# OrangeEarth15/3dgrut

Measured on AMD Instinct MI355X. Metric: train-step images/sec + render ms/frame, MipNeRF360 bicycle @1/2/4/8 GPU, higher is better.
Workload: dtype f32; 1 GPU; bicycle_like_6M_1237x822; num_gaussians=6000000, sh_degree=3, parallelism=per-view dp1, exchanged_records_last_step=0, loss=0.8*L1+0.2*(1-SSIM) (HIP fused SSIM), optimizer=HIP fused SH-gradient+Adam, all 59 params/Gaussian, trainer=native, optimizer_state=synthetic mid-training state: non-zero Adam moments on every row, storage_order=morton, optimizer_overlap=True, lazy_moment_decay=True, densification_statistics=False, warmup_extended_by=6

## Files before the change

3dgrut_amd/_capi.py:

```python
import ctypes as C
import os

HERE = os.path.dirname(os.path.abspath(__file__))
LIB_PATH = os.environ.get("GUT_HIP_LIB", os.path.join(HERE, "libgut_hip.so"))

GUT_ABI_VERSION = 6
GUT_NUM_KERNEL_TIMERS = 11
BWD_RAW_PARAMETER_GRADS = 1
BWD_COMPACT_RADIANCE_GRADS = 2
BWD_SKIP_EPILOGUE = 4
OPT_LAZY_TILE_ORDER = 1
ADAM_CLEAR_CONSUMED_GRADS = 1
GRADIENT_RECORD_FLOATS = 16
OPT_SORTED_REFERENCE_BACKWARD = 2
OPT_EARLY_EXTRA_PERCENT = 3
OPT_FORWARD_TILE_ORDER = 4
OPT_KERNEL_TIMING_SET = 5
OPT_DEBUG_REPLACE_SCRATCH = 100
KERNEL_TIMER_NAMES = ("project", "scan", "expand", "sort", "ranges", "render", "render_bwd", "project_bwd", "optimizer",
                      "optimizer_early", "optimizer_early_2")

SHUTTER_GLOBAL = 4
CAMERA_PINHOLE, CAMERA_FISHEYE = 0, 1

# ... 13 lines not shown


class GutConfig(C.Structure):
    _fields_ = [
        ("abi_version", C.c_int32), ("enable_kernel_timings", C.c_int32), ("particle_radiance_sph_degree", C.c_int32),
        ("particle_kernel_degree", C.c_int32), ("k_buffer_size", C.c_int32), ("global_z_order", C.c_int32),
        ("n_rolling_shutter_iterations", C.c_int32), ("ut_require_all_sigma_points", C.c_int32),
        ("rect_bounding", C.c_int32), ("tight_opacity_bounding", C.c_int32), ("tile_based_culling", C.c_int32),
        ("enable_hitcounts", C.c_int32),
        ("particle_kernel_min_response", C.c_float), ("particle_kernel_min_alpha", C.c_float),
        ("particle_kernel_max_alpha", C.c_float), ("min_transmittance", C.c_float),
        ("ut_alpha", C.c_float), ("ut_beta", C.c_float), ("ut_kappa", C.c_float), ("ut_in_image_margin_factor", C.c_float),
    ]


class GutStats(C.Structure):
    _fields_ = [
        ("num_particles", C.c_uint64), ("num_visible", C.c_uint64), ("num_intersections", C.c_uint64),
        ("num_tiles", C.c_uint64), ("num_pixels", C.c_uint64), ("traversed_fwd", C.c_uint64),
        ("traversed_bwd", C.c_uint64), ("sort_end_bit", C.c_uint32), ("binning_overflows", C.c_uint32),
        ("side_stream_rows", C.c_uint64), ("side_stream_rows_first_launch", C.c_uint64),
    ]


class GutLazyMoments(C.Structure):
    _fields_ = [("d_wave_step", C.c_void_p), ("d_pow_beta1", C.c_void_p), ("d_pow_beta2", C.c_void_p), ("table_len", C.c_uint32),
                ("d_overrun", C.c_void_p)]


class GutRegularisation(C.Structure):
    _fields_ = [("density_coeff", C.c_float), ("scale_coeff", C.c_float), ("d_partials", C.c_void_p)]


EXPORTS = ("gut_default_config", "gut_create", "gut_destroy", "gut_trace", "gut_trace_bwd", "gut_collect_times",
           "gut_get_stats", "gut_debug_buffer", "gut_debug_copy", "gut_kernel_times", "gut_kernel_times_mean", "gut_last_error", "gut_abi_version",
           "gut_ssim_workspace_bytes", "gut_ssim_forward", "gut_ssim_backward",
           "gut_photometric_workspace_bytes", "gut_photometric_loss", "gut_optimize_after_bwd", "gut_set_option",
           "gut_trace_bwd_ex", "gut_optimize_rows_without_gradient", "gut_compact_gradient_rows", "gut_scatter_gradient_records",
           "gut_sh_adam_step_ex", "gut_mark_walked_waves", "gut_adam_unwalked_waves", "gut_activate_pack", "gut_adam_step", "gut_sh_adam_step", "gut_mcmc_relocation",
           "gut_optimize_finish_without_gradient", "gut_scatter_gradient_records_dev", "gut_adam_unwalked_waves_ex", "gut_sync_moments", "gut_trace_fields", "gut_trace_bwd_fields", "gut_selective_adam",
           "gut_trace_model_fields", "gut_trace_bwd_model_fields", "gut_position_gradient_statistics",
           "gut_set_position_gradient_statistics", "gut_mcmc_perturb", "gut_trace_raw_model_fields", "gut_set_regularisation",
           "gut_sh_adam_step_regularised", "gut_adam_unwalked_waves_regularised", "gut_sync_moments_ex", "gut_regularisation_gradient",
           "gut_regularisation_loss", "gut_image_metrics_workspace_bytes", "gut_image_metrics")

_lib = None


def load():
    global _lib
    if _lib is not None:
        return _lib
    path = os.environ.get("GUT_HIP_LIBRARY") or LIB_PATH
    if not os.path.exists(path):
        raise RuntimeError(
            f"{path} is missing: the 3DGUT HIP extension is not built. Run `python -c 'import __graft_entry__ as g; "
            "g.build()'` (needs hipcc). There is no CPU fallback in the product path.")
    lib = C.CDLL(path)
    vp, u32, i32, f_p = C.c_void_p, C.c_uint32, C.c_int32, C.c_void_p
    lib.gut_last_error.restype = C.c_char_p
    lib.gut_abi_version.restype = C.c_int
    lib.gut_default_config.argtypes = [C.POINTER(GutConfig)]
    lib.gut_default_config.restype = None
    lib.gut_create.argtypes = [C.POINTER(GutConfig), C.c_int, C.POINTER(vp)]
    lib.gut_destroy.argtypes = [vp]
    lib.gut_destroy.restype = None
    lib.gut_trace.argtypes = [vp, vp, u32, i32, u32, f_p, f_p, i32, i32, f_p, f_p, C.POINTER(GutCamera), f_p, f_p, f_p, f_p]
    lib.gut_trace_bwd.argtypes = [vp, vp, u32, i32, u32, f_p, f_p, i32, i32, f_p, f_p, C.POINTER(GutCamera),
                                  f_p, f_p, f_p, f_p, f_p, f_p]
    lib.gut_trace_fields.argtypes = [vp, vp, u32, i32, u32, f_p, f_p, f_p, f_p, f_p, i32, i32, f_p, f_p, C.POINTER(GutCamera), f_p, f_p, f_p, f_p]
    lib.gut_trace_bwd_fields.argtypes = [vp, vp, u32, i32, u32, f_p, i32, i32, f_p, f_p, C.POINTER(GutCamera), f_p, f_p, f_p, f_p,
                                         f_p, f_p, f_p, f_p, f_p]
    lib.gut_trace_model_fields.argtypes = [vp, vp, u32, i32, u32, f_p, f_p, f_p, f_p, f_p, f_p, i32, i32, f_p, f_p, C.POINTER(GutCamera),
                                           f_p, f_p, f_p, f_p]
    lib.gut_trace_raw_model_fields.argtypes = lib.gut_trace_model_fields.argtypes
    lib.gut_trace_bwd_model_fields.argtypes = [vp, vp, u32, i32, u32, i32, i32, f_p, f_p, C.POINTER(GutCamera), f_p, f_p, f_p, f_p,
                                               f_p, f_p, f_p, f_p, f_p, f_p]
# ... 16 lines not shown
    lib.gut_photometric_loss.argtypes = [vp, i32, i32, vp, vp, C.c_float, C.c_float, C.c_float, vp, vp, vp]
    lib.gut_image_metrics_workspace_bytes.argtypes = [i32, i32]
    lib.gut_image_metrics_workspace_bytes.restype = C.c_size_t
    lib.gut_image_metrics.argtypes = [vp, i32, i32, vp, vp, C.c_float, vp, vp]
    lib.gut_trace_bwd_ex.argtypes = [vp, vp, u32, i32, u32, f_p, f_p, i32, i32, f_p, f_p, C.POINTER(GutCamera),
                                     f_p, f_p, f_p, f_p, f_p, f_p, u32]
    lib.gut_activate_pack.argtypes = [vp, u32, vp, vp]
    lib.gut_adam_step.argtypes = [vp, C.c_uint64, u32, vp, vp, vp, vp, C.POINTER(C.c_float), C.c_float, C.c_float,
                                  C.c_float, u32, vp]
    fptr = C.POINTER(C.c_float)
    lazy_p = C.POINTER(GutLazyMoments)
    lib.gut_optimize_after_bwd.argtypes = [vp, vp, i32, vp, vp, vp, vp, vp, vp, vp, fptr, fptr, C.c_float, C.c_float, C.c_float, u32,
                                           vp, vp, lazy_p]
    lib.gut_optimize_rows_without_gradient.argtypes = [vp, vp, vp, vp, vp, vp, vp, vp, fptr, fptr, C.c_float, C.c_float, C.c_float,
                                                       u32, vp, lazy_p]
    lib.gut_sync_moments.argtypes = [vp, u32, vp, vp, vp, vp, lazy_p, u32]
    lib.gut_optimize_finish_without_gradient.argtypes = [vp, vp]
    lib.gut_selective_adam.argtypes = [vp, C.c_uint64, u32, vp, vp, vp, vp, vp, C.c_float, C.c_float, C.c_float, C.c_float]
    lib.gut_set_option.argtypes = [vp, i32, i32]
    lib.gut_mcmc_relocation.argtypes = [vp, i32, vp, vp, vp, vp, i32, vp, vp]
    lib.gut_sh_adam_step.argtypes = [vp, u32, i32, u32, vp, vp, vp, C.c_float, vp, vp, vp, vp, vp, vp, fptr, fptr,
                                     C.c_float, C.c_float, C.c_float, u32, vp, vp, u32]
    lib.gut_sh_adam_step_ex.argtypes = lib.gut_sh_adam_step.argtypes + [u32, vp, lazy_p]
    lib.gut_mark_walked_waves.argtypes = [vp, vp, vp]
    lib.gut_adam_unwalked_waves.argtypes = [vp, u32, vp, vp, vp, vp, vp, vp, vp, fptr, fptr, C.c_float, C.c_float, C.c_float, u32, vp]
    lib.gut_adam_unwalked_waves_ex.argtypes = lib.gut_adam_unwalked_waves.argtypes + [lazy_p]
    reg_p = C.POINTER(GutRegularisation)
    lib.gut_set_regularisation.argtypes = [vp, reg_p]
    lib.gut_sh_adam_step_regularised.argtypes = lib.gut_sh_adam_step_ex.argtypes + [reg_p]
    lib.gut_adam_unwalked_waves_regularised.argtypes = lib.gut_adam_unwalked_waves_ex.argtypes + [reg_p]
    lib.gut_sync_moments_ex.argtypes = lib.gut_sync_moments.argtypes + [reg_p]
    lib.gut_regularisation_gradient.argtypes = [vp, u32, vp, vp, reg_p]
    lib.gut_regularisation_loss.argtypes = [vp, u32, vp, C.c_float, C.c_float, vp, vp, vp]
    lib.gut_compact_gradient_rows.argtypes = [vp, vp, vp, vp, u32, vp]
    lib.gut_scatter_gradient_records.argtypes = [vp, vp, u32, u32, vp, vp]
    lib.gut_scatter_gradient_records_dev.argtypes = [vp, vp, vp, u32, u32, vp, vp]
    if lib.gut_abi_version() != GUT_ABI_VERSION:
        raise RuntimeError("libgut_hip.so ABI version mismatch; rebuild")
    _lib = lib
    return lib


def check(rc, what):
    if rc != 0:
        msg = load().gut_last_error()
        raise RuntimeError(f"[3dgut] {what}: {msg.decode() if msg else 'unknown error'}")
```

3dgrut_amd/build.py:

```python
import os
import subprocess
import sys

HERE = os.path.dirname(os.path.abspath(__file__))
CSRC = os.path.join(HERE, "csrc")
OUT = os.path.join(HERE, "libgut_hip.so")
OBJ_DIR = os.path.join(HERE, "csrc", "_obj")

ARCH = "gfx950"
COMMON = ["--offload-arch=" + ARCH, "-O3", "-fPIC", "-std=c++17", "-Wall", "-Wno-unused-function"]
UNITS = [
    ("gut_project.hip", ["-ffp-contract=off"]),
    ("gut_render.hip", ["-ffp-contract=fast", "-munsafe-fp-atomics", "-fno-slp-vectorize"]),
    ("gut_render_general.hip", ["-ffp-contract=fast", "-munsafe-fp-atomics", "-fno-slp-vectorize"]),
    ("gut_render_sorted.hip", ["-ffp-contract=fast", "-munsafe-fp-atomics", "-fno-slp-vectorize"]),
    ("gut_sort.hip", ["-Wno-unused-parameter"]),
    ("gut_ssim.hip", ["-ffp-contract=fast"]),
    ("gut_train.hip", ["-ffp-contract=fast"]),
    ("gut_api.cpp", ["-x", "hip", "-ffp-contract=off"]),
]


def _stale(target, sources):
    if not os.path.exists(target):
        return True
    t = os.path.getmtime(target)
    return any(os.path.getmtime(s) > t for s in sources)


def build_diagnostic(out, defines, verbose=False):
    hipcc = os.environ.get("HIPCC", "/opt/rocm/bin/hipcc")
    obj_dir = out + ".obj"
    os.makedirs(obj_dir, exist_ok=True)
    objs = []
    for src, extra in UNITS:
        o = os.path.join(obj_dir, src + ".o")
        objs.append(o)
        cmd = [hipcc] + COMMON + extra + ["-D" + d for d in defines] + ["-c", os.path.join(CSRC, src), "-o", o]
        if verbose:
            print(" ".join(cmd), flush=True)
        subprocess.check_call(cmd)
    subprocess.check_call([hipcc, "--offload-arch=" + ARCH, "-shared", "-fPIC", "-o", out] + objs)
    return out


def build(force=False, verbose=False):
    hipcc = os.environ.get("HIPCC", "/opt/rocm/bin/hipcc")
    os.makedirs(OBJ_DIR, exist_ok=True)
    headers = [os.path.join(CSRC, "gut_internal.h"), os.path.join(CSRC, "gut_render_common.h"), os.path.join(CSRC, "gut_render.hip"),
               os.path.join(HERE, "..", "include", "gut_hip.h")]
    objs = []
    for src, extra in UNITS:
        s = os.path.join(CSRC, src)
        o = os.path.join(OBJ_DIR, src + ".o")
        objs.append(o)
        if force or _stale(o, [s] + headers):
            cmd = [hipcc] + COMMON + extra + ["-c", s, "-o", o]
            if verbose:
                print(" ".join(cmd), flush=True)
            subprocess.check_call(cmd)
    if force or _stale(OUT, objs):
        cmd = [hipcc, "--offload-arch=" + ARCH, "-shared", "-fPIC", "-o", OUT] + objs
        if verbose:
            print(" ".join(cmd), flush=True)
        subprocess.check_call(cmd)
    return OUT


if __name__ == "__main__":
    print(build(force="--force" in sys.argv, verbose=True))
```

3dgrut_amd/csrc/gut_api.cpp:

```cpp
#include <hip/hip_runtime.h>

#include <cmath>
#include <cstdarg>
#include <cstdio>
#include <cstdlib>
#include <cstring>
#include <deque>
#include <mutex>
#include <new>
#include <string>

#include "gut_internal.h"

namespace {

thread_local std::string g_last_error;

int fail(const char* fmt, ...) {
    char buf[512];
    va_list ap;
    va_start(ap, fmt);
    vsnprintf(buf, sizeof(buf), fmt, ap);
    va_end(ap);
    g_last_error = buf;
// ... 70 lines not shown
        for (int i = 0; i < 4; ++i) qb[i] = -qb[i];
        cos_t = -cos_t;
    }
    float q[4];
    if (cos_t > 1.0f - 1.1920929e-07f) {
        for (int i = 0; i < 4; ++i) q[i] = qa[i] * (1.0f - t) + qb[i] * t;
    } else {
        const float ang = acosf(cos_t);
        const float s0 = sinf((1.0f - t) * ang), s1 = sinf(t * ang), sd = sinf(ang);
        for (int i = 0; i < 4; ++i) q[i] = (s0 * qa[i] + s1 * qb[i]) / sd;
    }
    for (int i = 0; i < 3; ++i) out[i] = a[i] * (1.0f - t) + b[i] * t;
    out[3] = q[1]; out[4] = q[2]; out[5] = q[3]; out[6] = q[0];
}

uint32_t bit_width_u32(uint32_t n) {
    uint32_t w = 0;
    while (n) { ++w; n >>= 1; }
    return w;
}

}

struct gut_context {
    int device = 0;
    GutConfig cfg{};
    gut::RenderConsts consts{};
    std::mutex mu;

    DevBuf tiles_count, tiles_offset, proj_pos, conic_opacity, extent, depth, feat, grad16, scan_temp;
    float* stat_accum = nullptr;
    int32_t* stat_denom = nullptr;
    GutRegularisation reg{};
    DevBuf cam_pos;
    DevBuf wave_sums, block_prefix, scan_total;
    bool timing_main_stream = true, timing_side_stream = true;
    bool dbg_offset_valid = false;
    DevBuf sph_widened, sph_grad_wide;
    DevBuf packed12;
    bool packed_valid = false;
    bool packed_raw = false;
    DevBuf keys_unsorted, keys_sorted, ids_unsorted, ids_sorted, sort_temp;
    DevBuf ids_ordered, dbg_keys_sorted, dbg_ids_sorted;
    DevBuf tile_entries, tile_start, tile_cursor;
    uint32_t tile_entries_zeroed = 0;
    bool dbg_unsorted_valid = false;
    bool lazy_enabled = true;
    bool sorted_reference_bwd = true;
    bool lazy_order = false;
    bool dbg_sorted_valid = false;
    DevBuf ranges, trav_fwd, trav_bwd, tile_order;
    DevBuf counters;
    uint32_t* host_count = nullptr;
    uint32_t* host_count_dev = nullptr;
    hipEvent_t count_event = nullptr;
    hipStream_t side_stream = nullptr;
    hipEvent_t ev_projected = nullptr, ev_early_done = nullptr;
    struct EarlyArgs {
        float *raw12, *raw_m, *raw_v, *sh48, *sh_m, *sh_v, *act12;
        float lr12[12], lr48[48];
        float beta1, beta2, eps;
        uint32_t step, block_begin, block_end;
        uint32_t extra_end;
        GutLazyMoments lazy;
        GutRegularisation reg;
    } early_args{};
    bool marks_valid = false;
    DevBuf wave_walked;
    int early_extra_percent = 100;
    bool stats_early = false;
    uint32_t stats_split = 0, stats_extra_end = 0;
    bool early_part2_pending = false;
    hipEvent_t ev_bwd_start = nullptr;
    bool early_ran = false;
    bool early_wait_pending = false;
    bool grad16_zero = false;
    uint32_t m_capacity = 0, m_peak = 0, sort_n = 0;
    uint64_t overflows = 0;
    DevBuf zero_word, tile_ordered, walk_sums;
    bool fwd_longest_first = false;
    int fwd_order_mode = -1;
    bool dbg_ordered_valid = false;

    bool have_forward = false;
    hipStream_t fwd_stream = nullptr;
    uint32_t n = 0, m = 0;
    int width = 0, height = 0, tiles = 0, sh_degree = 0, end_bit = 0;
    gut::ViewParams view{};
    bool have_backward = false;

    std::deque<EventPair> fwd_timers, bwd_timers;
    float last_fwd_ms = -1.f, last_bwd_ms = -1.f;
    static constexpr int kRing = 64;
    struct KevSet {
        hipEvent_t e[16] = {};
        bool fwd = false, bwd = false, opt = false, early = false, early2 = false;
    };
    KevSet ring[kRing];
// ... 82 lines not shown
        if (old.a) (void)hipEventDestroy(old.a);
        if (old.b) (void)hipEventDestroy(old.b);
    }
    EventPair p;
    if (hipEventCreateWithFlags(&p.a, kTimingEvent) != hipSuccess || hipEventCreateWithFlags(&p.b, kTimingEvent) != hipSuccess) return nullptr;
    (void)hipEventRecord(p.a, s);
    q.push_back(p);
    return &q.back();
}

float drain_timers(std::deque<EventPair>& q) {
    if (q.empty()) return -1.f;
    float sum = 0.f;
    int cnt = 0;
    for (auto& p : q) {
        if (p.armed && hipEventSynchronize(p.b) == hipSuccess) {
            float ms = 0.f;
            if (hipEventElapsedTime(&ms, p.a, p.b) == hipSuccess) {
                sum += ms;
                cnt++;
            }
        }
        if (p.a) (void)hipEventDestroy(p.a);
        if (p.b) (void)hipEventDestroy(p.b);
    }
    q.clear();
    return cnt ? sum / (float)cnt : -1.f;
}

}

static int launch_early_part2(gut_context* h, hipStream_t s);
gut::LazyMoments gut_make_lazy(const GutLazyMoments* lazy, uint32_t step);
gut::Regularisation gut_make_reg(const GutRegularisation* reg);

extern "C" {

const char* gut_last_error(void) { return g_last_error.c_str(); }
int gut_abi_version(void) { return GUT_ABI_VERSION; }

void gut_default_config(GutConfig* cfg) {
    memset(cfg, 0, sizeof(*cfg));
    cfg->abi_version = GUT_ABI_VERSION;
    cfg->enable_kernel_timings = 0;
    cfg->particle_radiance_sph_degree = 3;
    cfg->particle_kernel_degree = 2;
    cfg->k_buffer_size = 0;
    cfg->global_z_order = 1;
    cfg->n_rolling_shutter_iterations = 5;
    cfg->ut_require_all_sigma_points = 0;
    cfg->rect_bounding = 1;
    cfg->tight_opacity_bounding = 1;
    cfg->tile_based_culling = 1;
    cfg->enable_hitcounts = 1;
    cfg->particle_kernel_min_response = 0.0113f;
    cfg->particle_kernel_min_alpha = 1.0f / 255.0f;
    cfg->particle_kernel_max_alpha = 0.99f;
    cfg->min_transmittance = 0.0001f;
    cfg->ut_alpha = 1.0f;
    cfg->ut_beta = 2.0f;
    cfg->ut_kappa = 0.0f;
    cfg->ut_in_image_margin_factor = 0.1f;
}

int gut_create(const GutConfig* cfg, int device_index, gut_handle* out) {
    if (!cfg || !out) return fail("gut_create: null argument");
// ... 165 lines not shown

    gut::FrameClears clears;
    clears.ranges = h->ranges.as<uint2>();
    clears.trav_bwd = h->trav_bwd.as<uint32_t>();
    clears.tiles = (uint32_t)tiles;
    if (n) {
        HIP_TRY(h->wave_walked.ensure(((size_t)n + gut::kBlock - 1) / gut::kBlock * (gut::kBlock / 64) + 64));
        clears.wave_walked = h->wave_walked.as<uint8_t>();
        HIP_TRY(h->cam_pos.ensure(64));
        clears.cam_pos = h->cam_pos.as<float>();
        if (h->lazy_enabled && h->cfg.k_buffer_size == 0) {
            const void* before = h->tile_entries.p;
            HIP_TRY(h->tile_entries.ensure(sizeof(uint32_t) * (size_t)tiles));
            HIP_TRY(h->tile_start.ensure(sizeof(uint32_t) * ((size_t)tiles + 1)));
            HIP_TRY(h->tile_cursor.ensure(sizeof(uint32_t) * (size_t)tiles));
            if (h->tile_entries.p != before) h->tile_entries_zeroed = 0;
            if (h->tile_entries_zeroed < (uint32_t)tiles) {
                HIP_TRY(hipMemsetAsync(h->tile_entries.p, 0, h->tile_entries.cap, s));
                h->tile_entries_zeroed = (uint32_t)(h->tile_entries.cap / sizeof(uint32_t));
            }
            clears.tile_entries = h->tile_entries.as<uint32_t>();
        }
    } else {
        HIP_TRY(hipMemsetAsync(h->trav_bwd.p, 0, sizeof(uint32_t) * (size_t)tiles, s));
        HIP_TRY(hipMemsetAsync(h->ranges.p, 0, sizeof(uint32_t) * 2 * (size_t)tiles, s));
    }
    mark(0);
    if (h->cfg.particle_radiance_sph_degree != 3 && n) {
        const uint32_t w = 3u * (uint32_t)((h->cfg.particle_radiance_sph_degree + 1) * (h->cfg.particle_radiance_sph_degree + 1));
        HIP_TRY(h->sph_widened.ensure(sizeof(float) * 48 * (size_t)n));
        gut::launch_resize_sph_rows(s, n, w, 48u, d_particle_radiance, h->sph_widened.as<float>());
        d_particle_radiance = h->sph_widened.as<float>();
    }
    gut::launch_project(s, v, h->consts, n, num_active_features, d_particle_density, d_particle_radiance,
                        h->tiles_count.as<uint32_t>(), h->proj_pos.as<float>(), h->conic_opacity.as<float>(),
                        h->extent.as<float>(), h->depth.as<float>(), h->feat.as<float>(), d_particle_visibility,
                        h->wave_sums.as<uint32_t>(), d_features_albedo, clears);
    mark(1);
    static const bool early_after_project = getenv("GUT_EARLY_AFTER_PROJECT") != nullptr;
    if (early_after_project) {
        if (!h->ev_projected) HIP_TRY(hipEventCreateWithFlags(&h->ev_projected, kOrderingEvent));
        HIP_TRY(hipEventRecord(h->ev_projected, s));
    }
    const int end_bit = 32 + (int)bit_width_u32((uint32_t)tiles);
    h->dbg_sorted_valid = false;
    h->dbg_unsorted_valid = false;
    h->dbg_ordered_valid = false;
    const uint32_t* d_count = n ? h->scan_total.as<uint32_t>() : h->zero_word.as<uint32_t>();
    h->dbg_offset_valid = false;
    uint32_t m = 0;
    bool count_pending = false;
    if (n) {
        gut::launch_scan_wave_sums(s, n, h->wave_sums.as<uint32_t>(), h->block_prefix.as<uint32_t>(), h->scan_total.as<uint32_t>(),
                                   h->host_count_dev, h->walk_sums.as<uint32_t>(), clears.tile_entries, (uint32_t)tiles,
                                   h->tile_start.as<uint32_t>(), h->tile_cursor.as<uint32_t>());
        if (!h->count_event) HIP_TRY(hipEventCreateWithFlags(&h->count_event, kOrderingEvent));
        HIP_TRY(hipEventRecord(h->count_event, s));
        count_pending = true;
    }
    mark(2);
    auto bin_and_render = [&](uint32_t sort_n, bool lazy) -> int {
        h->lazy_order = lazy;
        if (sort_n && lazy) {
            HIP_TRY(h->keys_sorted.ensure(sizeof(uint64_t) * (size_t)sort_n));
            HIP_TRY(h->ids_ordered.ensure(sizeof(uint32_t) * (size_t)sort_n));
            gut::launch_expand_grouped(s, v, h->consts, n, h->proj_pos.as<float>(), h->conic_opacity.as<float>(), h->extent.as<float>(),
                                       h->depth.as<float>(), (uint32_t)tiles, h->tile_start.as<uint32_t>(), h->tile_cursor.as<uint32_t>(),
                                       h->ranges.as<uint32_t>(), h->keys_sorted.as<uint64_t>(), sort_n);
            mark(3);
            mark(4);
// ... 361 lines not shown
        (void)hipEventRecord(total->b, s);
        total->armed = true;
    }
    h->kev_bwd_valid = timing;
    if (timing) h->ring[h->ring_cur].bwd = true;
    h->have_backward = true;
    return 0;
}

int gut_optimize_after_bwd(gut_handle h, void* stream_, int32_t num_active_features, const float* d_camera_position,
                           float* d_raw12, float* d_raw_m, float* d_raw_v, float* d_sh48, float* d_sh_m, float* d_sh_v,
                           const float* lr12, const float* lr48, float beta1, float beta2, float eps, uint32_t step,
                           const float* d_visibility, float* d_act12_out, const GutLazyMoments* lazy) {
    if (!h) return fail("gut_optimize_after_bwd: null handle");
    if (h->cfg.particle_radiance_sph_degree != 3)
        return fail("gut_optimize_after_bwd: the fused optimiser is built for particle_radiance_sph_degree=3 (59 parameters per Gaussian), this handle has %d", h->cfg.particle_radiance_sph_degree);
    std::lock_guard<std::mutex> lock(h->mu);
    hipStream_t s = static_cast<hipStream_t>(stream_);
    if (!h->have_backward || h->fwd_stream != s)
        return fail("gut_optimize_after_bwd: no backward context on this stream (call gut_trace_bwd_ex(..., GUT_BWD_SKIP_EPILOGUE) first)");
    if (num_active_features != h->sh_degree) return fail("gut_optimize_after_bwd: sh degree differs from the cached forward");
    if (h->n == 0) return 0;
    if (!d_raw12 || !d_raw_m || !d_raw_v || !d_sh48 || !d_sh_m || !d_sh_v || !lr12 || !lr48)
        return fail("gut_optimize_after_bwd: null pointer argument");
    if (!d_camera_position) d_camera_position = h->cam_pos.as<float>();
    if (h->early_ran && d_visibility)
        return fail("gut_optimize_after_bwd: a visibility mask cannot follow gut_optimize_rows_without_gradient");
    DeviceGuard dev_guard;
    HIP_TRY(dev_guard.set(h->device));
    if (lazy && d_visibility) return fail("gut_optimize_after_bwd: lazy moment decay cannot be combined with a visibility mask");
    if (h->early_ran && ((lazy && lazy->d_wave_step) != (h->early_args.lazy.d_wave_step != nullptr)))
        return fail("gut_optimize_after_bwd: lazy moment decay must be the same as in gut_optimize_rows_without_gradient");
    if (launch_early_part2(h, s)) return 1;
    const gut::LazyMoments lz = gut_make_lazy(lazy, step);
    const gut::Regularisation reg = gut_make_reg(h->early_ran ? &h->early_args.reg : &h->reg);
    h->reg = GutRegularisation{};
    if (lz.wave_step && h->cfg.k_buffer_size == 0 && h->m && !h->marks_valid) {
        gut::launch_mark_walked_waves(s, h->n, (uint32_t)h->tiles, h->ranges.as<uint32_t>(), h->trav_fwd.as<uint32_t>(),
                                      (h->lazy_order ? h->ids_ordered : h->ids_sorted).as<uint32_t>(), h->wave_walked.as<uint8_t>());
        h->marks_valid = true;
    }
    const bool timing = h->cfg.enable_kernel_timings != 0 && h->timing_main_stream && h->kev[12] && h->kev[13];
    if (timing) (void)hipEventRecord(h->kev[12], s);
    gut::launch_sh_adam_from_scratch(s, h->n, h->sh_degree, d_camera_position, h->grad16.as<float>(), h->tiles_count.as<uint32_t>(),
                                     h->feat.as<float>(), d_raw12, d_raw_m, d_raw_v, d_sh48, d_sh_m, d_sh_v, lr12, lr48, beta1, beta2,
                                     eps, step, d_visibility, d_act12_out, h->early_ran,
                                     (h->early_ran && h->early_args.extra_end) ? h->wave_walked.as<uint8_t>() : nullptr,
                                     h->early_args.block_begin, h->early_ran ? h->early_args.extra_end : 0u, lz,
                                     (lz.wave_step && h->marks_valid) ? h->wave_walked.as<uint8_t>() : nullptr,
                                     h->stat_accum, h->stat_denom, reg);
    h->stat_accum = nullptr;
    h->stat_denom = nullptr;
    HIP_TRY(hipGetLastError());
    if (timing) {
        (void)hipEventRecord(h->kev[13], s);
        h->ring[h->ring_cur].opt = true;
    }
    if (h->early_wait_pending) {
        HIP_TRY(hipStreamWaitEvent(s, h->ev_early_done, 0));
        h->early_wait_pending = false;
    }
    h->stats_early = h->early_ran;
    h->stats_split = h->early_args.block_begin;
    h->stats_extra_end = h->early_ran ? h->early_args.extra_end : 0u;
    h->early_ran = false;
    h->have_backward = false;
    h->grad16_zero = true;
    return 0;
}

int gut_set_position_gradient_statistics(gut_handle h, float* d_norm_accum, int32_t* d_norm_denom) {
    if (!h) return fail("gut_set_position_gradient_statistics: null handle");
    if ((d_norm_accum == nullptr) != (d_norm_denom == nullptr))
        return fail("gut_set_position_gradient_statistics: both buffers or neither");
    std::lock_guard<std::mutex> lock(h->mu);
    h->stat_accum = d_norm_accum;
    h->stat_denom = d_norm_denom;
    return 0;
}

int gut_set_regularisation(gut_handle h, const GutRegularisation* reg) {
    if (!h) return fail("gut_set_regularisation: null handle");
    if (reg && !(reg->density_coeff >= 0.0f && reg->scale_coeff >= 0.0f && reg->density_coeff < INFINITY && reg->scale_coeff < INFINITY))
        return fail("gut_set_regularisation: coefficients must be finite and >= 0");
    std::lock_guard<std::mutex> lock(h->mu);
    h->reg = reg ? *reg : GutRegularisation{};
    return 0;
}

int gut_optimize_finish_without_gradient(gut_handle h, void* stream_) {
    if (!h) return fail("gut_optimize_finish_without_gradient: null handle");
    std::lock_guard<std::mutex> lock(h->mu);
    if (!h->early_ran) return 0;
    hipStream_t s = static_cast<hipStream_t>(stream_);
    if (h->fwd_stream != s) return fail("gut_optimize_finish_without_gradient: not the stream of the forward");
    DeviceGuard dev_guard;
    HIP_TRY(dev_guard.set(h->device));
    const gut_context::EarlyArgs ea = h->early_args;
    h->stat_accum = nullptr;
    h->stat_denom = nullptr;
    h->reg = GutRegularisation{};
    HIP_TRY(h->grad16.ensure(sizeof(float) * 16 * (size_t)h->n));
    HIP_TRY(hipMemsetAsync(h->grad16.p, 0, h->grad16.cap, s));
    if (launch_early_part2(h, s)) return 1;
    gut::launch_sh_adam_from_scratch(s, h->n, h->sh_degree, h->zero_word.as<float>() ,
                                     h->grad16.as<float>(), h->tiles_count.as<uint32_t>(), h->feat.as<float>(), ea.raw12, ea.raw_m,
                                     ea.raw_v, ea.sh48, ea.sh_m, ea.sh_v, ea.lr12, ea.lr48, ea.beta1, ea.beta2, ea.eps, ea.step, nullptr,
                                     ea.act12, true, ea.extra_end ? h->wave_walked.as<uint8_t>() : nullptr, ea.block_begin, ea.extra_end,
                                     gut_make_lazy(&ea.lazy, ea.step), h->marks_valid ? h->wave_walked.as<uint8_t>() : nullptr,
                                     nullptr, nullptr, gut_make_reg(&ea.reg));
    HIP_TRY(hipGetLastError());
    if (h->early_wait_pending) {
        HIP_TRY(hipStreamWaitEvent(s, h->ev_early_done, 0));
        h->early_wait_pending = false;
    }
    h->stats_early = true;
    h->stats_split = ea.block_begin;
    h->stats_extra_end = ea.extra_end;
    h->early_ran = false;
    h->have_backward = false;
    h->grad16_zero = true;
    return 0;
}

int gut_mark_walked_waves(gut_handle h, void* stream_, uint8_t* d_wave_flags) {
    if (!h) return fail("gut_mark_walked_waves: null handle");
    std::lock_guard<std::mutex> lock(h->mu);
    hipStream_t s = static_cast<hipStream_t>(stream_);
    if (!h->have_forward || h->fwd_stream != s)
        return fail("gut_mark_walked_waves: no forward context on this stream (call gut_trace first, same stream)");
    if (h->n == 0) return 0;
    if (!d_wave_flags) return fail("gut_mark_walked_waves: null pointer argument");
    DeviceGuard dev_guard;
    HIP_TRY(dev_guard.set(h->device));
    HIP_TRY(hipMemsetAsync(d_wave_flags, 0, ((size_t)h->n + 63) / 64, s));
    if (h->m == 0) return 0;
    if (h->cfg.k_buffer_size > 0)
        gut::launch_mark_waves_with_tiles(s, h->n, h->tiles_count.as<uint32_t>(), d_wave_flags);
    else
        gut::launch_mark_walked_waves(s, h->n, (uint32_t)h->tiles, h->ranges.as<uint32_t>(), h->trav_fwd.as<uint32_t>(),
                                      (h->lazy_order ? h->ids_ordered : h->ids_sorted).as<uint32_t>(), d_wave_flags);
    HIP_TRY(hipGetLastError());
    return 0;
}

int gut_compact_gradient_rows(gut_handle h, void* stream_, const float* d_particle_density, float* d_records, uint32_t capacity,
                              uint32_t* d_count) {
    if (!h) return fail("gut_compact_gradient_rows: null handle");
    std::lock_guard<std::mutex> lock(h->mu);
    hipStream_t s = static_cast<hipStream_t>(stream_);
    if (!h->have_backward || h->fwd_stream != s)
        return fail("gut_compact_gradient_rows: no backward context on this stream (call gut_trace_bwd_ex(..., GUT_BWD_SKIP_EPILOGUE) first)");
    if (h->early_ran) return fail("gut_compact_gradient_rows: cannot follow gut_optimize_rows_without_gradient");
    if (!d_count || (h->n && (!d_particle_density || !d_records))) return fail("gut_compact_gradient_rows: null pointer argument");
    if (capacity < h->n) return fail("gut_compact_gradient_rows: the record buffer must hold one record per particle");
    DeviceGuard dev_guard;
    HIP_TRY(dev_guard.set(h->device));
    HIP_TRY(hipMemsetAsync(d_count, 0, sizeof(uint32_t), s));
    gut::launch_compact_gradient_rows(s, h->n, d_particle_density, h->tiles_count.as<uint32_t>(), h->feat.as<float>(),
                                      h->grad16.as<float>(), d_records, capacity, d_count);
    HIP_TRY(hipGetLastError());
    h->have_backward = false;
    h->grad16_zero = true;
    return 0;
}

int gut_optimize_rows_without_gradient(gut_handle h, void* stream_, float* d_raw12, float* d_raw_m, float* d_raw_v, float* d_sh48,
                                       float* d_sh_m, float* d_sh_v, const float* lr12, const float* lr48, float beta1, float beta2,
                                       float eps, uint32_t step, float* d_act12_out, const GutLazyMoments* lazy) {
    if (!h) return fail("gut_optimize_rows_without_gradient: null handle");
    if (h->cfg.particle_radiance_sph_degree != 3)
        return fail("gut_optimize_rows_without_gradient: the fused optimiser is built for particle_radiance_sph_degree=3 (59 parameters per Gaussian), this handle has %d", h->cfg.particle_radiance_sph_degree);
    std::lock_guard<std::mutex> lock(h->mu);
    hipStream_t s = static_cast<hipStream_t>(stream_);
    if (!h->have_forward || h->fwd_stream != s)
        return fail("gut_optimize_rows_without_gradient: no forward context on this stream (call gut_trace first, same stream)");
    if (h->early_ran) return fail("gut_optimize_rows_without_gradient: already called for this forward");
    if (h->have_backward) return fail("gut_optimize_rows_without_gradient: call it between gut_trace and gut_trace_bwd_ex");
    if (h->n == 0) return 0;
    if (!d_raw12 || !d_raw_m || !d_raw_v || !d_sh48 || !d_sh_m || !d_sh_v || !lr12 || !lr48)
        return fail("gut_optimize_rows_without_gradient: null pointer argument");
    DeviceGuard dev_guard;
    HIP_TRY(dev_guard.set(h->device));
    if (!h->side_stream) {
        int least = 0, greatest = 0;
        HIP_TRY(hipDeviceGetStreamPriorityRange(&least, &greatest));
        const char* pe = getenv("GUT_SIDE_STREAM_PRIORITY");
        int prio = 0;
        if (pe && pe[0] == 'l') prio = least;
        if (pe && pe[0] == 'h') prio = greatest;
        HIP_TRY(hipStreamCreateWithPriority(&h->side_stream, hipStreamNonBlocking, prio));
    }
    if (!h->ev_early_done) HIP_TRY(hipEventCreateWithFlags(&h->ev_early_done, kOrderingEvent));
    HIP_TRY(hipStreamWaitEvent(h->side_stream, h->ev_projected, 0));
    const bool timing = h->cfg.enable_kernel_timings != 0 && h->timing_side_stream && h->kev[14] && h->kev[15];
    if (timing) (void)hipEventRecord(h->kev[14], h->side_stream);
    static int split_percent = -1;
    if (split_percent < 0) {
        const char* e = getenv("GUT_EARLY_SPLIT");
        split_percent = e ? atoi(e) : -1;
        if (split_percent > 100) split_percent = -1;
    }
    const uint32_t nblocks = (h->n + gut::kBlock - 1) / gut::kBlock;
    const gut::Regularisation reg = gut_make_reg(&h->reg);
    const uint32_t percent = split_percent >= 0 ? (uint32_t)split_percent : ((lazy && lazy->d_wave_step && !reg.on()) ? 60u : 25u);
    const uint32_t first = (uint32_t)((uint64_t)nblocks * percent / 100u);
    gut::launch_adam_rows_without_gradient(h->side_stream, h->n, h->tiles_count.as<uint32_t>(), d_raw12, d_raw_m, d_raw_v, d_sh48,
                                           d_sh_m, d_sh_v, lr12, lr48, beta1, beta2, eps, step, d_act12_out, 0, first, nullptr, first, 0,
                                           false, gut_make_lazy(lazy, step), reg);
    HIP_TRY(hipGetLastError());
    gut_context::EarlyArgs& ea = h->early_args;
    ea.raw12 = d_raw12; ea.raw_m = d_raw_m; ea.raw_v = d_raw_v; ea.sh48 = d_sh48; ea.sh_m = d_sh_m; ea.sh_v = d_sh_v;
    ea.act12 = d_act12_out;
    memcpy(ea.lr12, lr12, sizeof(ea.lr12));
    memcpy(ea.lr48, lr48, sizeof(ea.lr48));
    ea.beta1 = beta1; ea.beta2 = beta2; ea.eps = eps; ea.step = step; ea.block_begin = first; ea.block_end = nblocks;
    ea.lazy = GutLazyMoments{};
    if (lazy) ea.lazy = *lazy;
    ea.reg = h->reg;
    ea.extra_end = (h->cfg.k_buffer_size == 0 && h->m) ? (uint32_t)((uint64_t)nblocks * (uint32_t)h->early_extra_percent / 100u) : 0u;
    h->early_part2_pending = first < nblocks || ea.extra_end > 0;
    if (timing) {
        (void)hipEventRecord(h->kev[15], h->side_stream);
        h->ring[h->ring_cur].early = true;
    }
    HIP_TRY(hipEventRecord(h->ev_early_done, h->side_stream));
    h->early_ran = true;
    h->early_wait_pending = true;
    return 0;
}

static int launch_early_part2(gut_context* h, hipStream_t s) {
    if (!h->early_part2_pending) return 0;
    h->early_part2_pending = false;
    if (!h->ev_bwd_start) HIP_TRY(hipEventCreateWithFlags(&h->ev_bwd_start, kOrderingEvent));
    const gut_context::EarlyArgs& ea = h->early_args;
    if (ea.extra_end) {
        gut::launch_mark_walked_waves(s, h->n, (uint32_t)h->tiles, h->ranges.as<uint32_t>(), h->trav_fwd.as<uint32_t>(),
                                      (h->lazy_order ? h->ids_ordered : h->ids_sorted).as<uint32_t>(), h->wave_walked.as<uint8_t>());
        h->marks_valid = true;
    }
    HIP_TRY(hipEventRecord(h->ev_bwd_start, s));
    HIP_TRY(hipStreamWaitEvent(h->side_stream, h->ev_bwd_start, 0));
    if (h->cfg.enable_kernel_timings != 0 && h->timing_side_stream && h->kev[7]) (void)hipEventRecord(h->kev[7], h->side_stream);
    gut::launch_adam_rows_without_gradient(h->side_stream, h->n, h->tiles_count.as<uint32_t>(), ea.raw12, ea.raw_m, ea.raw_v, ea.sh48,
                                           ea.sh_m, ea.sh_v, ea.lr12, ea.lr48, ea.beta1, ea.beta2, ea.eps, ea.step, ea.act12,
                                           ea.extra_end ? 0u : ea.block_begin, ea.block_end,
                                           ea.extra_end ? h->wave_walked.as<uint8_t>() : nullptr, ea.block_begin, ea.extra_end, true,
                                           gut_make_lazy(&ea.lazy, ea.step), gut_make_reg(&ea.reg));
    HIP_TRY(hipGetLastError());
    const bool timing = h->cfg.enable_kernel_timings != 0 && h->timing_side_stream && h->kev[14] && h->kev[15];
    if (timing) {
        (void)hipEventRecord(h->kev[15], h->side_stream);
        h->ring[h->ring_cur].early2 = h->kev[7] != nullptr;
    }
    HIP_TRY(hipEventRecord(h->ev_early_done, h->side_stream));
    return 0;
}

int gut_set_option(gut_handle h, int32_t option, int32_t value) {
    if (!h) return fail("gut_set_option: null handle");
    std::lock_guard<std::mutex> lock(h->mu);
    switch (option) {
    case GUT_OPT_LAZY_TILE_ORDER: h->lazy_enabled = value != 0; return 0;
    case GUT_OPT_SORTED_REFERENCE_BACKWARD: h->sorted_reference_bwd = value != 0; return 0;
    case GUT_OPT_KERNEL_TIMING_SET:
        if (value < 0 || value > 2) return fail("gut_set_option: GUT_OPT_KERNEL_TIMING_SET takes 0, 1 or 2");
        h->timing_main_stream = value == 0;
        h->timing_side_stream = value != 2;
        return 0;
    case GUT_OPT_FORWARD_TILE_ORDER:
        if (value < -1 || value > 1) return fail("gut_set_option: GUT_OPT_FORWARD_TILE_ORDER takes -1, 0 or 1");
        h->fwd_order_mode = value;
        return 0;
    case GUT_OPT_EARLY_EXTRA_PERCENT:
        if (value < 0 || value > 100) return fail("gut_set_option: GUT_OPT_EARLY_EXTRA_PERCENT takes 0..100");
        h->early_extra_percent = value;
        return 0;
    case GUT_OPT_DEBUG_REPLACE_SCRATCH: {
        DevBuf* bufs[] = {&h->tiles_count, &h->tiles_offset, &h->proj_pos, &h->conic_opacity, &h->extent, &h->depth, &h->feat,
                          &h->grad16, &h->scan_temp, &h->keys_unsorted, &h->keys_sorted, &h->ids_unsorted, &h->ids_sorted,
                          &h->sort_temp, &h->ids_ordered, &h->ranges, &h->trav_fwd, &h->trav_bwd, &h->tile_order, &h->tile_ordered};
// ... 219 lines not shown
```

3dgrut_amd/csrc/gut_internal.h:

```cpp
#pragma once
#include <hip/hip_runtime.h>
#include <math.h>
#include <stdint.h>

#include "../../include/gut_hip.h"

namespace gut {

constexpr int kTile = 16;
constexpr int kBlock = 256;
constexpr uint32_t kInvalid = 0xFFFFFFFFu;

struct Affine {
    float r[3][3];
    float t[3];
};

struct ViewParams {
    Affine w2s_end;
    float pose_start[7], pose_end[7];
    int32_t shutter;
    Affine w2s_start;
    Affine w2s_mid;
    Affine s2w;
// ... 10 lines not shown
};

struct RenderConsts {
    float alpha_threshold, max_alpha, min_response, min_transmittance;
    float min_sensor_z, cov_dilation;
    float ut_delta, ut_w0_mean, ut_wi, ut_w0_cov, ut_margin;
    int32_t rect_bounding, tight_opacity_bounding, tile_culling, global_z_order;
    float max_d2;
};

__host__ __device__ inline float kernel_cutoff_d2(int degree, float r) {
    float s, n;
    switch (degree) {
    case 8: s = 0.000685871056241f; n = 8.0f; break;
    case 5: s = 0.0185185185185f; n = 5.0f; break;
    case 4: s = 0.0555555555556f; n = 4.0f; break;
    case 3: s = 0.166666666667f; n = 3.0f; break;
    case 1: s = 1.5f; n = 1.0f; break;
    case 0: { const float t = (1.0f - r) / 0.329630334487f; return t * t; }
    default: return -2.0f * logf(r);
    }
    return powf(-logf(r) / s, 2.0f / n);
}

struct Counters {
    unsigned long long visible;
    unsigned long long traversed_fwd;
    unsigned long long traversed_bwd;
    unsigned long long side_stream_rows;
    unsigned long long side_stream_rows_first;
    unsigned long long pad[3];
};

struct LazyMoments {
    uint32_t* wave_step = nullptr;
    const float* pow1 = nullptr;
    const float* pow2 = nullptr;
    uint32_t len = 0;
    uint32_t t = 0;
    uint32_t* overrun = nullptr;
};

struct Regularisation {
    float density_coeff = 0.0f;
    float scale_coeff = 0.0f;
    float2* partials = nullptr;
    __host__ __device__ bool on() const { return density_coeff != 0.0f || scale_coeff != 0.0f; }
};

struct FrameClears {
    uint2* ranges = nullptr;
    uint32_t* trav_bwd = nullptr;
    uint8_t* wave_walked = nullptr;
    uint32_t tiles = 0;
    float* cam_pos = nullptr;
    uint32_t* tile_entries = nullptr;
};

void launch_project(hipStream_t s, const ViewParams& v, const RenderConsts& c, uint32_t n, int sh_degree,
                    const float* density12, const float* sph48, uint32_t* tiles_count, float* proj_pos,
                    float* conic_opacity, float* extent, float* depth, float* feat, float* visibility,
                    uint32_t* wave_sums , const float* sph_albedo ,
                    const FrameClears& clears);
void launch_scan_wave_sums(hipStream_t s, uint32_t n, const uint32_t* wave_sums, uint32_t* block_prefix, uint32_t* total,
                           uint32_t* host_out , const uint32_t* walk_sums ,
                           uint32_t* tile_entries, uint32_t tiles, uint32_t* tile_start, uint32_t* tile_cursor);
void launch_expand_grouped(hipStream_t s, const ViewParams& v, const RenderConsts& c, uint32_t n, const float* proj_pos,
                           const float* conic_opacity, const float* extent, const float* depth, uint32_t tiles,
                           const uint32_t* tile_start, uint32_t* tile_cursor, uint32_t* ranges, uint64_t* entries, uint32_t capacity);
void launch_expand(hipStream_t s, const ViewParams& v, const RenderConsts& c, uint32_t n, const uint32_t* tiles_count,
                   const uint32_t* wave_sums, const uint32_t* block_prefix, const uint32_t* total , const float* proj_pos, const float* conic_opacity, const float* extent, const float* depth,
                   uint64_t* keys, uint32_t* ids, uint32_t capacity);
void launch_pad_keys(hipStream_t s, const uint32_t* count, uint32_t sort_n, uint64_t* keys, uint32_t* ids);
void launch_mask_unordered(hipStream_t s, uint32_t tiles, const uint32_t* ranges, const uint32_t* tile_ordered, uint32_t* ordered_ids);
void launch_tile_ranges(hipStream_t s, uint32_t m, const uint64_t* sorted_keys, uint32_t* ranges);
struct GradFields {
    float* pos = nullptr;
    float* dns = nullptr;
    float* rot = nullptr;
    float* scl = nullptr;
    float* alb = nullptr;
    float* spec = nullptr;
};
void launch_project_bwd(hipStream_t s, const ViewParams& v, uint32_t n, int sh_degree, const float* density12,
                        const uint32_t* tiles_count, const float* feat, float* grad16 ,
                        float* density_grad12, float* sph_grad48, bool raw_grads, const GradFields& fields = GradFields());
void launch_pack_fields(hipStream_t s, uint32_t n, const float* pos, const float* dns, const float* rot, const float* scl,
                        float* density12);
void launch_resize_sph_rows(hipStream_t s, uint32_t n, uint32_t in_width, uint32_t out_width, const float* in, float* out);
void launch_pack_activate_fields(hipStream_t s, uint32_t n, const float* pos, const float* dns_logit, const float* rot_raw,
                                 const float* log_scl, float* act12);

void launch_render(hipStream_t s, const ViewParams& v, const RenderConsts& c, const float* density12,
                   const float* feat, const float* ray_ori, const float* ray_dir, const uint32_t* ranges,
                   const uint32_t* sorted_ids, const uint32_t* d_num_intersections, float* rgba, float* dist, float* hits,
                   uint32_t* tile_traversed, const uint64_t* tile_keys , uint32_t* ordered_ids ,
// ... 61 lines not shown
```

3dgrut_amd/csrc/gut_project.hip:

```cpp
#include "gut_internal.h"

namespace gut {

__device__ __forceinline__ uint32_t f2u(float f) { return __float_as_uint(f); }
__device__ __forceinline__ float u2f(uint32_t u) { return __uint_as_float(u); }

__device__ float det_logf(float x) {
    uint32_t ix = f2u(x);
    int k = 0;
    if (ix >= 0x7f800000u) return x;
    if (ix < 0x00800000u) {
        if (ix == 0) return -__builtin_inff();
        x = x * 33554432.0f;
        ix = f2u(x);
        k -= 25;
    }
    k += (int)(ix >> 23) - 127;
    ix &= 0x007fffffu;
    const uint32_t i = (ix + (0x95f64u << 3)) & 0x800000u;
    x = u2f(ix | (i ^ 0x3f800000u));
    k += (int)(i >> 23);
    const float f = x - 1.0f;
    const float s = f / (2.0f + f);
    const float dk = (float)k;
    const float z = s * s;
    const float w = z * z;
    const float t1 = w * (0.40000972152f + w * 0.24279078841f);
    const float t2 = z * (0.66666662693f + w * 0.28498786688f);
    const float R = t2 + t1;
    const float hfsq = (0.5f * f) * f;
    return dk * 6.9313812256e-01f - ((hfsq - (s * (hfsq + R) + dk * 9.0580006145e-06f)) - f);
}

// ... 280 lines not shown
    }
    if ((tid & 63u) == 0u) {
        red[4 * (tid >> 6) + 0] = a;
        red[4 * (tid >> 6) + 1] = b;
        red[4 * (tid >> 6) + 2] = c;
        red[4 * (tid >> 6) + 3] = d;
    }
    __syncthreads();
    a = __builtin_amdgcn_readfirstlane(min(min(red[0], red[4]), min(red[8], red[12])));
    b = __builtin_amdgcn_readfirstlane(min(min(red[1], red[5]), min(red[9], red[13])));
    c = __builtin_amdgcn_readfirstlane(min(min(red[2], red[6]), min(red[10], red[14])));
    d = __builtin_amdgcn_readfirstlane(min(min(red[3], red[7]), min(red[11], red[15])));
    TileWindow W = {0, 0, 0, 0};
    if (a != kNone && (-c - a) * (-d - b) <= kBinWindow) W = TileWindow{a, b, -c - a, -d - b};
    for (int k = (int)tid; k < W.w * W.h; k += kBlock) bins[k] = 0u;
    __syncthreads();
    return W;
}

__device__ __forceinline__ bool in_window(const TileWindow& W, int x, int y, uint32_t& bin) {
    const uint32_t bx = (uint32_t)(x - W.x0), by = (uint32_t)(y - W.y0);
    bin = by * (uint32_t)W.w + bx;
    return bx < (uint32_t)W.w && by < (uint32_t)W.h;
}

__device__ __forceinline__ uint32_t window_tile(const TileWindow& W, int grid_x, uint32_t bin) {
    const uint32_t by = bin / (uint32_t)W.w;
    return (uint32_t)(W.y0 + (int)by) * (uint32_t)grid_x + (uint32_t)W.x0 + (bin - by * (uint32_t)W.w);
}

__device__ __forceinline__ float bcast(float v, int src_lane) { return __shfl(v, src_lane); }
__device__ __forceinline__ int bcast(int v, int src_lane) { return __shfl(v, src_lane); }

template <int kVariant, bool kRolling, bool kSplitSH>
__global__ __launch_bounds__(kBlock, 5) void k_project_on_tiles(ViewParams v, RenderConsts c, uint32_t n, int sh_degree,
                                                            const float4* __restrict__ density12,
                                                            const float* __restrict__ sph48,
                                                            const float* __restrict__ sph_albedo,
                                                            uint32_t* __restrict__ tiles_count, float2* __restrict__ proj_pos,
                                                            float4* __restrict__ conic_opacity, float2* __restrict__ extent,
                                                            float* __restrict__ depth, float* __restrict__ feat,
                                                            float* __restrict__ visibility, uint32_t* __restrict__ wave_sums,
                                                            FrameClears clr) {
    __shared__ float sh_lds[(kBlock / 64) * 32 * kShRow];
    __shared__ uint32_t s_bins[kBinWindow];
    __shared__ int s_red[16];
    const uint32_t i = blockIdx.x * kBlock + threadIdx.x;
    const int lane = (int)(threadIdx.x & 63);
    const int wave = (int)(threadIdx.x >> 6);
    for (uint32_t t = i; t < clr.tiles; t += gridDim.x * kBlock) {
        clr.ranges[t] = make_uint2(0u, 0u);
        clr.trav_bwd[t] = 0u;
    }
    if (lane == 0 && clr.wave_walked) clr.wave_walked[blockIdx.x * (kBlock / 64) + (uint32_t)wave] = 0;
    if (i == 0 && clr.cam_pos) {
        clr.cam_pos[0] = v.s2w.t[0]; clr.cam_pos[1] = v.s2w.t[1]; clr.cam_pos[2] = v.s2w.t[2];
    }
    uint32_t cnt = 0;
    bool conic_ok = false, ok = false;
    float cx = 0.f, cy = 0.f, con0 = 0.f, con1 = 0.f, con2 = 0.f, con3 = 0.f, ex = 0.f, ey = 0.f, zkey = 0.f;
    float f0 = 0.f, f1 = 0.f, f2 = 0.f, max_power = 0.f, zcam = 0.f;
    float4 a = make_float4(0.f, 0.f, 0.f, 0.f);
    const uint32_t wave_first = blockIdx.x * kBlock + (uint32_t)wave * 64u;
    const uint32_t rows_here = wave_first < n ? min(64u, n - wave_first) : 0u;
    if (i < n) {
        a = density12[3 * (size_t)i + 0];
        const float4 b = density12[3 * (size_t)i + 1];
        const float4 d = density12[3 * (size_t)i + 2];
        const float opacity_in = a.w;
        const Affine& m = v.w2s_mid;
        zcam = a.x * m.r[2][0] + a.y * m.r[2][1] + a.z * m.r[2][2] + m.t[2];
        ok = !(opacity_in < c.alpha_threshold) && !(zcam < c.min_sensor_z);
        if (ok) {
            float rows[3][3];
            quat_rows(b.x, b.y, b.z, b.w, rows);
            const float scl[3] = {d.x, d.y, d.z};
// ... 104 lines not shown
            const int jx0 = bcast(bb.x0, j), jy0 = bcast(bb.y0, j), jw = bcast(bb.x1 - bb.x0, j), jarea = bcast(area, j);
            const float j0 = bcast(con0, j), j1 = bcast(con1, j), j2 = bcast(con2, j), jcx = bcast(cx, j), jcy = bcast(cy, j),
                        jmp = bcast(max_power, j);
            uint32_t total = 0;
            for (int base = 0; base < jarea; base += 64) {
                const int t = base + lane;
                bool pass = false;
                if (t < jarea) {
                    const int ty = t / jw;
                    const int tx = t - ty * jw;
                    pass = tile_min_power((float)(jx0 + tx), (float)(jy0 + ty), j0, j1, j2, jcx, jcy) < jmp;
                    if (pass) count_entry(jx0 + tx, jy0 + ty);
                }
                total += (uint32_t)__popcll(__ballot(pass));
            }
            if (lane == j) cnt = total;
        }
    }
    if (tile_entries) {
        __syncthreads();
        for (int k = (int)threadIdx.x; k < W.w * W.h; k += kBlock) {
            const uint32_t b = s_bins[k];
            if (b) atomicAdd(&tile_entries[window_tile(W, v.grid_x, (uint32_t)k)], b);
        }
    }

    const bool vis = cnt != 0;
    const unsigned long long vis_mask = __ballot(vis);
    if (vis_mask != 0ull) {
        float* wl = sh_lds + wave * 32 * kShRow;
        const float4* src = reinterpret_cast<const float4*>(sph48 + (size_t)wave_first * 48);
        float Y[16];
        float inv_dist = 0.f, dist = 0.f;
        if (vis) {
            const float rx = a.x - v.s2w.t[0], ry = a.y - v.s2w.t[1], rz = a.z - v.s2w.t[2];
            dist = sqrtf(rx * rx + ry * ry + rz * rz);
            inv_dist = 1.0f / dist;
            sh_basis(sh_degree, rx * inv_dist, ry * inv_dist, rz * inv_dist, Y);
        }
        const int ncoef = (sh_degree + 1) * (sh_degree + 1);
        float4 shq[12];
        float alb0 = 0.f, alb1 = 0.f, alb2 = 0.f;
        if (kSplitSH) {
            const float* spec = sph48 + (size_t)wave_first * 45;
            const uint32_t lim = rows_here * 45u;
            if (vis) {
                alb0 = sph_albedo[3 * (size_t)i + 0];
                alb1 = sph_albedo[3 * (size_t)i + 1];
                alb2 = sph_albedo[3 * (size_t)i + 2];
            }
#pragma unroll
            for (int it = 0; it < 12; ++it) {
                const uint32_t ql = (uint32_t)(it % 6) * 64u + (uint32_t)lane;
                const uint32_t f = 4u * ((uint32_t)(it / 6) * 360u + ql);
                const uint32_t r0 = min(f / 45u, 63u), r1 = min((f + 3u) / 45u, 63u);
                const bool wanted = (ql < 360u) && (f < lim) && (sh_degree > 0) && (((vis_mask >> r0) | (vis_mask >> r1)) & 1ull);
                float4 val = make_float4(0.f, 0.f, 0.f, 0.f);
                if (wanted) {
                    if (f + 3u < lim) {
                        val = *reinterpret_cast<const float4*>(spec + f);
                    } else {
                        val.x = spec[f];
                        if (f + 1u < lim) val.y = spec[f + 1u];
                        if (f + 2u < lim) val.z = spec[f + 2u];
                    }
                }
                shq[it] = val;
            }
        } else {
#pragma unroll
            for (int it = 0; it < 12; ++it) {
                const uint32_t q = (uint32_t)it * 64u + (uint32_t)lane;
                const bool wanted = (q < rows_here * 12u) && ((vis_mask >> (q / 12u)) & 1ull);
                shq[it] = wanted ? src[q] : make_float4(0.f, 0.f, 0.f, 0.f);
            }
        }
#pragma unroll
        for (int half = 0; half < 2; ++half) {
            if (kSplitSH) {
#pragma unroll
                for (int it6 = 0; it6 < 6; ++it6) {
                    const uint32_t ql = (uint32_t)it6 * 64u + (uint32_t)lane;
                    if (ql < 360u) {
                        const uint32_t f = 4u * ql;
                        const uint32_t row = f / 45u, col = f - row * 45u;
                        const float4 val = shq[half * 6 + it6];
                        const float vals[4] = {val.x, val.y, val.z, val.w};
#pragma unroll
                        for (uint32_t j = 0; j < 4u; ++j) {
                            const uint32_t cj = col + j;
                            const uint32_t rj = cj >= 45u ? row + 1u : row;
                            if (rj < 32u) wl[rj * kShRow + 3u + (cj >= 45u ? cj - 45u : cj)] = vals[j];
                        }
                    }
                }
                if ((lane >> 5) == half) {
                    float* own = wl + (lane & 31) * kShRow;
                    own[0] = alb0; own[1] = alb1; own[2] = alb2;
                }
            } else {
#pragma unroll
                for (int it6 = 0; it6 < 6; ++it6) {
                    const uint32_t q = (uint32_t)it6 * 64u + (uint32_t)lane;
                    const uint32_t row = q / 12u, col = (q - row * 12u) * 4u;
                    float* dst = wl + row * kShRow + col;
                    const float4 val = shq[half * 6 + it6];
                    dst[0] = val.x; dst[1] = val.y; dst[2] = val.z; dst[3] = val.w;
                }
            }
// ... 515 lines not shown
}

__global__ __launch_bounds__(kBlock) void k_stats_reduce(uint32_t n, const uint32_t* __restrict__ tiles_count, uint32_t t,
                                                        const uint32_t* __restrict__ trav_fwd,
                                                        const uint32_t* __restrict__ trav_bwd, Counters* __restrict__ out) {
    unsigned long long v = 0, ef = 0, eb = 0;
    for (uint32_t i = blockIdx.x * kBlock + threadIdx.x; i < n; i += gridDim.x * kBlock) v += tiles_count[i] != 0;
    for (uint32_t i = blockIdx.x * kBlock + threadIdx.x; i < t; i += gridDim.x * kBlock) {
        ef += trav_fwd[i];
        eb += trav_bwd[i];
    }
    for (int m = 32; m >= 1; m >>= 1) {
        v += __shfl_xor(v, m);
        ef += __shfl_xor(ef, m);
        eb += __shfl_xor(eb, m);
    }
    if ((threadIdx.x & 63) == 0) {
        if (v) atomicAdd(&out->visible, v);
        if (ef) atomicAdd(&out->traversed_fwd, ef);
        if (eb) atomicAdd(&out->traversed_bwd, eb);
    }
}

void launch_stats_reduce(hipStream_t s, uint32_t n, const uint32_t* tiles_count, uint32_t t, const uint32_t* trav_fwd,
                         const uint32_t* trav_bwd, Counters* out) {
    hipLaunchKernelGGL(k_stats_reduce, dim3(256), dim3(kBlock), 0, s, n, tiles_count, t, trav_fwd, trav_bwd, out);
}

static inline uint32_t blocks_for(uint32_t n) { return (n + kBlock - 1) / kBlock; }

void launch_project(hipStream_t s, const ViewParams& v, const RenderConsts& c, uint32_t n, int sh_degree,
                    const float* density12, const float* sph48, uint32_t* tiles_count, float* proj_pos,
                    float* conic_opacity, float* extent, float* depth, float* feat, float* visibility,
                    uint32_t* wave_sums, const float* sph_albedo, const FrameClears& clears) {
    if (n == 0) return;
    bool distorted = false;
    for (float k : v.radial) distorted |= (k != 0.0f);
    for (float k : v.tangential) distorted |= (k != 0.0f);
    for (float k : v.thin_prism) distorted |= (k != 0.0f);
    const int variant = v.model == GUT_CAMERA_OPENCV_FISHEYE ? 2 : (distorted ? 1 : 0);
    const bool rolling = v.shutter != GUT_SHUTTER_GLOBAL;
    auto kern = rolling ? (variant == 0 ? k_project_on_tiles<0, true, false> : (variant == 1 ? k_project_on_tiles<1, true, false> : k_project_on_tiles<2, true, false>))
                        : (variant == 0 ? k_project_on_tiles<0, false, false> : (variant == 1 ? k_project_on_tiles<1, false, false> : k_project_on_tiles<2, false, false>));
    if (sph_albedo)
        kern = rolling ? (variant == 0 ? k_project_on_tiles<0, true, true> : (variant == 1 ? k_project_on_tiles<1, true, true> : k_project_on_tiles<2, true, true>))
                       : (variant == 0 ? k_project_on_tiles<0, false, true> : (variant == 1 ? k_project_on_tiles<1, false, true> : k_project_on_tiles<2, false, true>));
    hipLaunchKernelGGL(kern, dim3(blocks_for(n)), dim3(kBlock), 0, s, v, c, n, sh_degree,
                       reinterpret_cast<const float4*>(density12), sph48, sph_albedo, tiles_count, reinterpret_cast<float2*>(proj_pos),
                       reinterpret_cast<float4*>(conic_opacity), reinterpret_cast<float2*>(extent), depth, feat, visibility,
                       wave_sums, clears);
}

void launch_scan_wave_sums(hipStream_t s, uint32_t n, const uint32_t* wave_sums, uint32_t* block_prefix, uint32_t* total,
                           uint32_t* host_out, const uint32_t* walk_sums, uint32_t* tile_entries, uint32_t tiles, uint32_t* tile_start,
                           uint32_t* tile_cursor) {
    if (n == 0) return;
    hipLaunchKernelGGL(k_scan_wave_sums, dim3(1), dim3(1024), 0, s, reinterpret_cast<const uint4*>(wave_sums), blocks_for(n), block_prefix,
                       total, host_out, walk_sums, tile_entries, tiles, tile_start, tile_cursor);
}

void launch_expand_grouped(hipStream_t s, const ViewParams& v, const RenderConsts& c, uint32_t n, const float* proj_pos,
                           const float* conic_opacity, const float* extent, const float* depth, uint32_t tiles,
                           const uint32_t* tile_start, uint32_t* tile_cursor, uint32_t* ranges, uint64_t* entries, uint32_t capacity) {
    if (n == 0) return;
    hipLaunchKernelGGL(k_expand_grouped, dim3(blocks_for(n)), dim3(kBlock), 0, s, v, c, n, reinterpret_cast<const float2*>(proj_pos),
                       reinterpret_cast<const float4*>(conic_opacity), reinterpret_cast<const float2*>(extent), depth, tiles, tile_start,
                       tile_cursor, reinterpret_cast<uint2*>(ranges), reinterpret_cast<uint2*>(entries), capacity);
}

void launch_expand(hipStream_t s, const ViewParams& v, const RenderConsts& c, uint32_t n, const uint32_t* tiles_count,
                   const uint32_t* wave_sums, const uint32_t* block_prefix, const uint32_t* total,
                   const float* proj_pos, const float* conic_opacity, const float* extent, const float* depth,
                   uint64_t* keys, uint32_t* ids, uint32_t capacity) {
    if (n == 0) return;
    hipLaunchKernelGGL(k_expand_tiles, dim3(blocks_for(n)), dim3(kBlock), 0, s, v, c, n, tiles_count,
                       reinterpret_cast<const uint4*>(wave_sums), block_prefix, total,
                       reinterpret_cast<const float2*>(proj_pos), reinterpret_cast<const float4*>(conic_opacity),
                       reinterpret_cast<const float2*>(extent), depth, keys, ids, capacity);
}
// ... 28 lines not shown
```

3dgrut_amd/csrc/gut_train.hip:

```cpp
#include <cstdlib>
#include <type_traits>

#include "gut_internal.h"

namespace gut {

__device__ __forceinline__ float4 activate_position_density(const float4& a) {
    return make_float4(a.x, a.y, a.z, 1.0f / (1.0f + expf(-a.w)));
}
__device__ __forceinline__ float4 activate_quaternion(const float4& q, float* clamped_norm) {
    const float nrm = sqrtf(q.x * q.x + q.y * q.y + q.z * q.z + q.w * q.w);
    const float inv = 1.0f / fmaxf(nrm, 1e-12f);
    *clamped_norm = fmaxf(nrm, 1e-12f);
    return make_float4(q.x * inv, q.y * inv, q.z * inv, q.w * inv);
}
__device__ __forceinline__ float4 activate_scale(const float4& s, float clamped_norm) {
    return make_float4(expf(s.x), expf(s.y), expf(s.z), clamped_norm);
}
__device__ __forceinline__ void activate_row(const float4& a, const float4& q, const float4& s, float4* __restrict__ act_row) {
    float nrm;
    act_row[0] = activate_position_density(a);
    act_row[1] = activate_quaternion(q, &nrm);
    act_row[2] = activate_scale(s, nrm);
}

__global__ __launch_bounds__(kBlock) void k_activate_pack(uint32_t n, const float4* __restrict__ raw, float4* __restrict__ act) {
    const uint32_t i = blockIdx.x * kBlock + threadIdx.x;
    if (i >= n) return;
    activate_row(raw[3 * (size_t)i + 0], raw[3 * (size_t)i + 1], raw[3 * (size_t)i + 2], act + 3 * (size_t)i);
}

__global__ __launch_bounds__(kBlock) void k_pack_activate_fields(uint32_t n, const float* __restrict__ pos, const float* __restrict__ dns,
                                                                const float4* __restrict__ rot, const float* __restrict__ scl,
                                                                float4* __restrict__ act) {
    const uint32_t i = blockIdx.x * kBlock + threadIdx.x;
    if (i >= n) return;
// ... 218 lines not shown
    return tiny ? y * 0x1p-32f : y;
}

__device__ __forceinline__ void adam4(const AdamParams& ap, uint32_t c0, const float4& g, float4& p, float4& m, float4& v) {
#define GUT_ADAM_LANE(X, K)                               \
    m.X = ap.beta1 * m.X + (1.0f - ap.beta1) * g.X;        \
    v.X = ap.beta2 * v.X + (1.0f - ap.beta2) * g.X * g.X;  \
    p.X -= ap.lr[c0 + K] * m.X * __builtin_amdgcn_rcpf(sqrt_approx_pos(v.X) * ap.bias2_sqrt + ap.eps);
    GUT_ADAM_LANE(x, 0)
    GUT_ADAM_LANE(y, 1)
    GUT_ADAM_LANE(z, 2)
    GUT_ADAM_LANE(w, 3)
#undef GUT_ADAM_LANE
}

__device__ __forceinline__ void scale4(float4& a, float f) { a.x *= f; a.y *= f; a.z *= f; a.w *= f; }

__device__ __forceinline__ bool all_zero(const float4& m, const float4& v) {
    return m.x == 0.0f && m.y == 0.0f && m.z == 0.0f && m.w == 0.0f && v.x == 0.0f && v.y == 0.0f && v.z == 0.0f && v.w == 0.0f;
}

__device__ __forceinline__ void adam4_zero_grad(const AdamParams& ap, const float4& lr, float4& p, float4& m, float4& v) {
#define GUT_ADAM_LANE(X)                                   \
    m.X = ap.beta1 * m.X + (1.0f - ap.beta1) * 0.0f;       \
    v.X = ap.beta2 * v.X + (1.0f - ap.beta2) * 0.0f * 0.0f; \
    p.X -= lr.X * m.X * __builtin_amdgcn_rcpf(sqrt_approx_pos(v.X) * ap.bias2_sqrt + ap.eps);
    GUT_ADAM_LANE(x)
    GUT_ADAM_LANE(y)
    GUT_ADAM_LANE(z)
    GUT_ADAM_LANE(w)
#undef GUT_ADAM_LANE
}

struct LazyAdam {
    float c1, c2s, b2s, eps;
};
__device__ __forceinline__ LazyAdam make_lazy_adam(const AdamParams& ap, const float2& dk) {
    LazyAdam la;
    la.c1 = ap.beta1 * dk.x;
    la.c2s = (ap.beta2 * dk.y) * 0x1p+32f;
    la.b2s = ap.bias2_sqrt * 0x1p-16f;
    la.eps = ap.eps;
    return la;
}
__device__ __forceinline__ void adam4_lazy(const LazyAdam& la, const float4& lr, float4& p, const float4& m, const float4& v) {
#define GUT_ADAM_LANE(X) p.X -= lr.X * (la.c1 * m.X) * __builtin_amdgcn_rcpf(__builtin_amdgcn_sqrtf(la.c2s * v.X) * la.b2s + la.eps);
    GUT_ADAM_LANE(x)
    GUT_ADAM_LANE(y)
    GUT_ADAM_LANE(z)
    GUT_ADAM_LANE(w)
#undef GUT_ADAM_LANE
}

__device__ __forceinline__ float reg_sigmoid(float d) { return 1.0f / (1.0f + expf(-d)); }
__device__ __forceinline__ float4 reg_density_grad(const Regularisation& r, float sig) {
    return make_float4(0.0f, 0.0f, 0.0f, r.density_coeff * (sig * (1.0f - sig)));
}
__device__ __forceinline__ float4 reg_scale_grad(const Regularisation& r, float e0, float e1, float e2) {
    return make_float4(r.scale_coeff * e0, r.scale_coeff * e1, r.scale_coeff * e2, 0.0f);
}
__device__ __forceinline__ void reg_wave_partials(const Regularisation& r, float sig, float esum, uint32_t wave_index, uint32_t lane) {
#pragma unroll
    for (int o = 32; o >= 1; o >>= 1) {
        sig += __shfl_xor(sig, o);
        esum += __shfl_xor(esum, o);
    }
    if (r.partials && lane == 0) r.partials[wave_index] = make_float2(sig, esum);
}
__device__ __forceinline__ void reg_adam_raw_row(const Regularisation& r, const AdamParams& a12, float4* __restrict__ p12,
                                                 float4* __restrict__ m12, float4* __restrict__ v12, float4* __restrict__ act12, size_t i,
                                                 float* sig_out, float* esum_out) {
    float4 a = p12[3 * i + 0], m = m12[3 * i + 0], v = v12[3 * i + 0];
    const float sig = reg_sigmoid(a.w);
    adam4(a12, 0, reg_density_grad(r, sig), a, m, v);
    p12[3 * i + 0] = a; m12[3 * i + 0] = m; v12[3 * i + 0] = v;
    float4 b = p12[3 * i + 1];
    m = m12[3 * i + 1]; v = v12[3 * i + 1];
    adam4(a12, 4, make_float4(0.f, 0.f, 0.f, 0.f), b, m, v);
    p12[3 * i + 1] = b; m12[3 * i + 1] = m; v12[3 * i + 1] = v;
    float4 c = p12[3 * i + 2];
    m = m12[3 * i + 2]; v = v12[3 * i + 2];
    const float e0 = expf(c.x), e1 = expf(c.y), e2 = expf(c.z);
    adam4(a12, 8, reg_scale_grad(r, e0, e1, e2), c, m, v);
    p12[3 * i + 2] = c; m12[3 * i + 2] = m; v12[3 * i + 2] = v;
    if (act12) activate_row(a, b, c, act12 + 3 * i);
    *sig_out = sig;
    *esum_out = (e0 + e1) + e2;
}

template <bool kScratch, bool kReg>
__global__ __launch_bounds__(kBlock) void k_sh_adam(std::conditional_t<kReg, ShAdamParamsReg, ShAdamParams> sp, float* __restrict__ mrgb,
                                                   float4* __restrict__ grad12, float4* __restrict__ p12,
                                                   float4* __restrict__ m12, float4* __restrict__ v12, float4* __restrict__ p48,
                                                   float4* __restrict__ m48, float4* __restrict__ v48,
                                                   const float* __restrict__ visibility, float4* __restrict__ act12,
                                                   const uint32_t* __restrict__ tiles_count, const float* __restrict__ feat) {
    constexpr int kRow = 49;
    __shared__ float tile[(kBlock / 64) * 64 * kRow];
    const uint32_t i = blockIdx.x * kBlock + threadIdx.x;
    const uint32_t lane = threadIdx.x & 63, wave = threadIdx.x >> 6;
    float* wl = tile + wave * 64 * kRow;
    const uint32_t wave_first = blockIdx.x * kBlock + wave * 64u;
    const uint32_t rows_here = wave_first < sp.n ? min(64u, sp.n - wave_first) : 0u;
    if (kScratch && sp.rows_with_tiles_only &&
        side_stream_owns_wave(sp.own, __ballot(i < sp.n && tiles_count[i] != 0) != 0ull, wave_first >> 6, blockIdx.x))
        return;
    if (!kScratch && sp.own.walked && wave_first < sp.n && sp.own.walked[wave_first >> 6] == 0) return;
    const uint32_t wave_index = wave_first >> 6;
    bool lazy_wave = false;
    float2 dk = make_float2(1.0f, 1.0f);
    if (sp.lazy.wave_step && wave_first < sp.n) {
        dk = missed_decay(sp.lazy, wave_index);
        if (kScratch) {
            const bool has_tiles = __ballot(i < sp.n && tiles_count[i] != 0) != 0ull;
            lazy_wave = !has_tiles || (sp.rule_walked && sp.rule_walked[wave_index] == 0);
        }
    }
    if constexpr (kReg) {
        float sig = 0.0f, esum = 0.0f;
        if (i < sp.n) {
            const float4 a = p12[3 * (size_t)i + 0], c = p12[3 * (size_t)i + 2];
            sig = reg_sigmoid(a.w);
            esum = (expf(c.x) + expf(c.y)) + expf(c.z);
        }
        if (wave_first < sp.n) reg_wave_partials(sp.reg, sig, esum, wave_index, lane);
    }
    if (kScratch && lazy_wave) {
        const LazyAdam l12 = make_lazy_adam(sp.a12, dk), l48 = make_lazy_adam(sp.a48, dk);
        if constexpr (kReg) {
            if (i < sp.n) {
                float sig, esum;
                reg_adam_raw_row(sp.reg, sp.a12, p12, m12, v12, act12, i, &sig, &esum);
            }
        } else if (i < sp.n) {
            float4 a = p12[3 * (size_t)i + 0], b = p12[3 * (size_t)i + 1], c = p12[3 * (size_t)i + 2];
            adam4_lazy(l12, make_float4(sp.a12.lr[0], sp.a12.lr[1], sp.a12.lr[2], sp.a12.lr[3]), a, m12[3 * (size_t)i + 0], v12[3 * (size_t)i + 0]);
            adam4_lazy(l12, make_float4(sp.a12.lr[4], sp.a12.lr[5], sp.a12.lr[6], sp.a12.lr[7]), b, m12[3 * (size_t)i + 1], v12[3 * (size_t)i + 1]);
            adam4_lazy(l12, make_float4(sp.a12.lr[8], sp.a12.lr[9], sp.a12.lr[10], sp.a12.lr[11]), c, m12[3 * (size_t)i + 2], v12[3 * (size_t)i + 2]);
            p12[3 * (size_t)i + 0] = a; p12[3 * (size_t)i + 1] = b; p12[3 * (size_t)i + 2] = c;
            if (act12) activate_row(a, b, c, act12 + 3 * (size_t)i);
        }
        float4* bp = p48 + (size_t)wave_first * 12;
        const float4* bm = m48 + (size_t)wave_first * 12;
        const float4* bv = v48 + (size_t)wave_first * 12;
#pragma unroll 4
        for (int it = 0; it < 12; ++it) {
            const uint32_t q = (uint32_t)it * 64u + lane;
            if (q >= rows_here * 12u) continue;
            const uint32_t row = q / 12u, col = (q - row * 12u) * 4u;
            float4 pp = bp[q];
            adam4_lazy(l48, make_float4(sp.a48.lr[col], sp.a48.lr[col + 1], sp.a48.lr[col + 2], sp.a48.lr[col + 3]), pp, bm[q], bv[q]);
            bp[q] = pp;
        }
        return;
    }
    float G[48];
#pragma unroll
    for (int k = 0; k < 48; ++k) G[k] = 0.0f;
    bool active = false;
    if (i < sp.n) {
        active = !(visibility && !(visibility[i] != 0.0f));
        if (active) {
            float4 a = p12[3 * (size_t)i + 0];
            const float px = a.x, py = a.y, pz = a.z;
            float4 b = p12[3 * (size_t)i + 1], c = p12[3 * (size_t)i + 2];
            float4 g0, g1, g2;
            float own_r = 0.f, own_g = 0.f, own_b = 0.f;
            const float gs = sp.grad_scale;
            if (kScratch) {
                g0 = make_float4(0.f, 0.f, 0.f, 0.f); g1 = g0; g2 = g0;
                if (tiles_count[i] != 0) {
                    g0 = grad12[4 * (size_t)i + 0];
                    g1 = grad12[4 * (size_t)i + 1];
                    g2 = grad12[4 * (size_t)i + 2];
                    const float4 g3 = grad12[4 * (size_t)i + 3];
                    grad12[4 * (size_t)i + 0] = make_float4(0.f, 0.f, 0.f, 0.f);
                    grad12[4 * (size_t)i + 1] = make_float4(0.f, 0.f, 0.f, 0.f);
                    grad12[4 * (size_t)i + 2] = make_float4(0.f, 0.f, 0.f, 0.f);
                    grad12[4 * (size_t)i + 3] = make_float4(0.f, 0.f, 0.f, 0.f);
                    own_r = feat[3 * (size_t)i + 0] > 0.0f ? g2.w : 0.0f;
                    own_g = feat[3 * (size_t)i + 1] > 0.0f ? g3.x : 0.0f;
                    own_b = feat[3 * (size_t)i + 2] > 0.0f ? g3.y : 0.0f;
                    if (sp.stat_accum && (g0.x != 0.0f || g0.y != 0.0f || g0.z != 0.0f))
                        position_gradient_statistic(g0.x, g0.y, g0.z, px, py, pz, sp.cam, sp.stat_accum + i, sp.stat_denom + i);
                    float4 act[3];
                    activate_row(a, b, c, act);
// ... 53 lines not shown
                for (int k = 0; k < 16; ++k) {
                    G[3 * k + 0] += Y[k] * r;
                    G[3 * k + 1] += Y[k] * g;
                    G[3 * k + 2] += Y[k] * bl;
                }
            }
        }
    }
    if (__ballot(active) == 0ull) return;
#pragma unroll
    for (int k = 0; k < 48; ++k) wl[lane * kRow + k] = G[k];
    wl[lane * kRow + 48] = active ? 1.0f : 0.0f;
    __builtin_amdgcn_fence(__ATOMIC_RELEASE, "wavefront");
    __builtin_amdgcn_wave_barrier();
    __builtin_amdgcn_fence(__ATOMIC_ACQUIRE, "wavefront");
    float4* bp = p48 + (size_t)wave_first * 12;
    float4* bm = m48 + (size_t)wave_first * 12;
    float4* bv = v48 + (size_t)wave_first * 12;
#pragma unroll 4
    for (int it = 0; it < 12; ++it) {
        const uint32_t q = (uint32_t)it * 64u + lane;
        if (q >= rows_here * 12u) continue;
        const uint32_t row = q / 12u, col = (q - row * 12u) * 4u;
        if (wl[row * kRow + 48] == 0.0f) continue;
        const float* gsrc = wl + row * kRow + col;
        const float4 g = make_float4(gsrc[0], gsrc[1], gsrc[2], gsrc[3]);
        float4 pp = bp[q], mm = bm[q], vv = bv[q];
        scale4(mm, dk.x); scale4(vv, dk.y);
        adam4(sp.a48, col, g, pp, mm, vv);
        bp[q] = pp;
        if (!lazy_wave) { bm[q] = mm; bv[q] = vv; }
    }
    if (sp.lazy.wave_step && !lazy_wave && lane == 0 && rows_here) sp.lazy.wave_step[wave_index] = sp.lazy.t;
}

template <bool kLazy, bool kReg, typename... Reg>
__global__ __launch_bounds__(kBlock, 4) void k_adam_rows_without_gradient(AdamParams a12, AdamParams a48, uint32_t n,
                                                                          const uint32_t* __restrict__ tiles_count,
                                                                          float4* __restrict__ p12, float4* __restrict__ m12,
                                                                          float4* __restrict__ v12, float4* __restrict__ p48,
                                                                          float4* __restrict__ m48, float4* __restrict__ v48,
                                                                          float4* __restrict__ act12, uint32_t block_begin,
                                                                          uint32_t block_end, EarlyOwnership own,
                                                                          uint32_t second_launch, LazyMoments lazy, Reg... reg_arg) {
    const uint32_t lane = threadIdx.x & 63, wave = threadIdx.x >> 6;
    const float4 zero = make_float4(0.f, 0.f, 0.f, 0.f);
    __builtin_amdgcn_s_setprio(1);
    __shared__ float4 s_lr48[12];
    if (threadIdx.x < 12) s_lr48[threadIdx.x] = make_float4(a48.lr[4 * threadIdx.x], a48.lr[4 * threadIdx.x + 1], a48.lr[4 * threadIdx.x + 2],
                                                           a48.lr[4 * threadIdx.x + 3]);
    __syncthreads();
    for (uint32_t blk = block_begin + blockIdx.x; blk < block_end; blk += gridDim.x) {
        const uint32_t i = blk * kBlock + threadIdx.x;
        const uint32_t wave_first = blk * kBlock + wave * 64u;
        const uint32_t rows_here = wave_first < n ? min(64u, n - wave_first) : 0u;
        const bool mine = i < n;
        if (wave_first >= n) continue;
        const bool has_tiles = tiles_count ? (__ballot(i < n && tiles_count[i] != 0) != 0ull) : true;
        if (!side_stream_owns_wave(own, has_tiles, wave_first >> 6, blk, second_launch != 0u)) continue;
        const float2 dk = missed_decay(lazy, wave_first >> 6);
        const bool store_mv = kLazy ? false : (lazy.wave_step == nullptr);
        if constexpr (kReg) {
            const Regularisation reg = (reg_arg, ...);
            float sig = 0.0f, esum = 0.0f;
            if (mine) reg_adam_raw_row(reg, a12, p12, m12, v12, act12, i, &sig, &esum);
            reg_wave_partials(reg, sig, esum, wave_first >> 6, lane);
// ... 1 lines not shown
            float4* bm = m48 + (size_t)wave_first * 12;
            float4* bv = v48 + (size_t)wave_first * 12;
            const LazyAdam l48 = make_lazy_adam(a48, dk);
#pragma unroll 4
            for (int it = 0; it < 12; ++it) {
                const uint32_t q = (uint32_t)it * 64u + lane;
                if (q >= rows_here * 12u) continue;
                const uint32_t row = q / 12u, col = (q - row * 12u) * 4u;
                float4 pp = bp[q];
                if (kLazy) {
                    adam4_lazy(l48, s_lr48[col >> 2], pp, bm[q], bv[q]);
                } else {
                    float4 mm = bm[q], vv = bv[q];
                    scale4(mm, dk.x); scale4(vv, dk.y);
                    adam4_zero_grad(a48, s_lr48[col >> 2], pp, mm, vv);
                    bm[q] = mm; bv[q] = vv;
                }
                bp[q] = pp;
            }
            continue;
        }
        if (kLazy) {
            const LazyAdam l12 = make_lazy_adam(a12, dk), l48 = make_lazy_adam(a48, dk);
            if (mine) {
                float4 a = p12[3 * (size_t)i + 0], b = p12[3 * (size_t)i + 1], c = p12[3 * (size_t)i + 2];
                adam4_lazy(l12, make_float4(a12.lr[0], a12.lr[1], a12.lr[2], a12.lr[3]), a, m12[3 * (size_t)i + 0], v12[3 * (size_t)i + 0]);
                p12[3 * (size_t)i + 0] = a;
                adam4_lazy(l12, make_float4(a12.lr[4], a12.lr[5], a12.lr[6], a12.lr[7]), b, m12[3 * (size_t)i + 1], v12[3 * (size_t)i + 1]);
                p12[3 * (size_t)i + 1] = b;
                adam4_lazy(l12, make_float4(a12.lr[8], a12.lr[9], a12.lr[10], a12.lr[11]), c, m12[3 * (size_t)i + 2], v12[3 * (size_t)i + 2]);
                p12[3 * (size_t)i + 2] = c;
                if (act12) activate_row(a, b, c, act12 + 3 * (size_t)i);
            }
            float4* bp = p48 + (size_t)wave_first * 12;
            const float4* bm = m48 + (size_t)wave_first * 12;
            const float4* bv = v48 + (size_t)wave_first * 12;
#pragma unroll 4
            for (int it = 0; it < 12; ++it) {
                const uint32_t q = (uint32_t)it * 64u + lane;
                if (q >= rows_here * 12u) continue;
                const uint32_t row = q / 12u, col = (q - row * 12u) * 4u;
                float4 pp = bp[q];
                adam4_lazy(l48, s_lr48[col >> 2], pp, bm[q], bv[q]);
                bp[q] = pp;
            }
            continue;
        }
        if (mine) {
            float4 a = p12[3 * (size_t)i + 0], m = m12[3 * (size_t)i + 0], v = v12[3 * (size_t)i + 0];
            scale4(m, dk.x); scale4(v, dk.y);
            adam4(a12, 0, zero, a, m, v);
            p12[3 * (size_t)i + 0] = a;
            if (store_mv) { m12[3 * (size_t)i + 0] = m; v12[3 * (size_t)i + 0] = v; }
            float4 b = p12[3 * (size_t)i + 1];
            m = m12[3 * (size_t)i + 1]; v = v12[3 * (size_t)i + 1];
            scale4(m, dk.x); scale4(v, dk.y);
            adam4(a12, 4, zero, b, m, v);
            p12[3 * (size_t)i + 1] = b;
            if (store_mv) { m12[3 * (size_t)i + 1] = m; v12[3 * (size_t)i + 1] = v; }
            float4 c = p12[3 * (size_t)i + 2];
            m = m12[3 * (size_t)i + 2]; v = v12[3 * (size_t)i + 2];
            scale4(m, dk.x); scale4(v, dk.y);
            adam4(a12, 8, zero, c, m, v);
            p12[3 * (size_t)i + 2] = c;
            if (store_mv) { m12[3 * (size_t)i + 2] = m; v12[3 * (size_t)i + 2] = v; }
            if (act12) activate_row(a, b, c, act12 + 3 * (size_t)i);
        }
        float4* bp = p48 + (size_t)wave_first * 12;
        float4* bm = m48 + (size_t)wave_first * 12;
        float4* bv = v48 + (size_t)wave_first * 12;
#pragma unroll 4
        for (int it = 0; it < 12; ++it) {
            const uint32_t q = (uint32_t)it * 64u + lane;
            if (q >= rows_here * 12u) continue;
            const uint32_t row = q / 12u, col = (q - row * 12u) * 4u;
            float4 pp = bp[q], mm = bm[q], vv = bv[q];
            scale4(mm, dk.x); scale4(vv, dk.y);
            adam4_zero_grad(a48, s_lr48[col >> 2], pp, mm, vv);
            bp[q] = pp;
            if (store_mv) { bm[q] = mm; bv[q] = vv; }
        }
    }
}

#ifndef GUT_NARROW_REGULARISED
#define GUT_NARROW_REGULARISED 0
#endif
template <bool kReg, typename... Reg>
__global__ __launch_bounds__(kBlock) __attribute__((amdgpu_num_vgpr(16))) void k_adam_rows_without_gradient_narrow(
    AdamParams a12, AdamParams a48, uint32_t n, const uint32_t* __restrict__ tiles_count, float4* __restrict__ p12,
    float4* __restrict__ m12, float4* __restrict__ v12, float4* __restrict__ p48, float4* __restrict__ m48,
    float4* __restrict__ v48, float4* __restrict__ act12, uint32_t block_begin, uint32_t block_end, EarlyOwnership own,
    uint32_t second_launch, LazyMoments lazy, Reg... reg_arg) {
    const uint32_t lane = threadIdx.x & 63;
    const uint32_t wave = (uint32_t)__builtin_amdgcn_readfirstlane((int)(threadIdx.x >> 6));
    __builtin_amdgcn_s_setprio(1);
    __shared__ float4 s_lr48[12];
    if (threadIdx.x < 12) s_lr48[threadIdx.x] = make_float4(a48.lr[4 * threadIdx.x], a48.lr[4 * threadIdx.x + 1], a48.lr[4 * threadIdx.x + 2],
                                                           a48.lr[4 * threadIdx.x + 3]);
    __syncthreads();
    for (uint32_t blk = block_begin + blockIdx.x; blk < block_end; blk += gridDim.x) {
        const uint32_t wave_first = blk * kBlock + wave * 64u;
        if (wave_first >= n) continue;
        const uint32_t rows_here = min(64u, n - wave_first);
        const bool has_tiles = tiles_count ? (__ballot(lane < rows_here && tiles_count[wave_first + lane] != 0) != 0ull) : true;
        if (!side_stream_owns_wave(own, has_tiles, wave_first >> 6, blk, second_launch != 0u)) continue;
        const float2 dk = missed_decay(lazy, wave_first >> 6);
        const LazyAdam l12 = make_lazy_adam(a12, dk), l48 = make_lazy_adam(a48, dk);
        if constexpr (kReg) {
            const Regularisation reg = (reg_arg, ...);
            float sig = 0.0f, esum = 0.0f;
            if (lane < rows_here) {
                float4* rp = p12 + 3 * (size_t)wave_first;
                float4* rm = m12 + 3 * (size_t)wave_first;
                float4* rv = v12 + 3 * (size_t)wave_first;
                float4* ra = act12 + 3 * (size_t)wave_first;
                uint32_t o = 3u * lane;
                asm volatile("" : "+v"(o));
                float4 x = rp[o], m = rm[o], v = rv[o];
                sig = reg_sigmoid(x.w);
                adam4(a12, 0, reg_density_grad(reg, sig), x, m, v);
// ... 9 lines not shown
                x = rp[o + 2]; m = rm[o + 2]; v = rv[o + 2];
                const float e0 = expf(x.x), e1 = expf(x.y), e2 = expf(x.z);
                adam4(a12, 8, reg_scale_grad(reg, e0, e1, e2), x, m, v);
                esum = (e0 + e1) + e2;
                rp[o + 2] = x; rm[o + 2] = m; rv[o + 2] = v;
                if (act12) ra[o + 2] = activate_scale(x, nrm);
                __builtin_amdgcn_sched_barrier(0);
            }
            reg_wave_partials(reg, sig, esum, wave_first >> 6, lane);
        } else if (lane < rows_here) {
            float4* rp = p12 + 3 * (size_t)wave_first;
            const float4* rm = m12 + 3 * (size_t)wave_first;
            const float4* rv = v12 + 3 * (size_t)wave_first;
            float4* ra = act12 + 3 * (size_t)wave_first;
            uint32_t o = 3u * lane;
            asm volatile("" : "+v"(o));
            float4 x = rp[o];
            adam4_lazy(l12, make_float4(a12.lr[0], a12.lr[1], a12.lr[2], a12.lr[3]), x, rm[o], rv[o]);
            rp[o] = x;
            if (act12) ra[o] = activate_position_density(x);
            __builtin_amdgcn_sched_barrier(0);
            x = rp[o + 1];
            adam4_lazy(l12, make_float4(a12.lr[4], a12.lr[5], a12.lr[6], a12.lr[7]), x, rm[o + 1], rv[o + 1]);
            rp[o + 1] = x;
            float nrm = 0.0f;
            if (act12) ra[o + 1] = activate_quaternion(x, &nrm);
            __builtin_amdgcn_sched_barrier(0);
            x = rp[o + 2];
            adam4_lazy(l12, make_float4(a12.lr[8], a12.lr[9], a12.lr[10], a12.lr[11]), x, rm[o + 2], rv[o + 2]);
            rp[o + 2] = x;
            if (act12) ra[o + 2] = activate_scale(x, nrm);
            __builtin_amdgcn_sched_barrier(0);
        }
        float4* bp = p48 + (size_t)wave_first * 12;
        const float4* bm = m48 + (size_t)wave_first * 12;
        const float4* bv = v48 + (size_t)wave_first * 12;
        uint32_t q0 = lane;
        asm volatile("" : "+v"(q0));
#pragma unroll 1
        for (uint32_t q = q0; q < rows_here * 12u; q += 64u) {
            const uint32_t col4 = q % 12u;
            float4 pp = bp[q];
            adam4_lazy(l48, s_lr48[col4], pp, bm[q], bv[q]);
            bp[q] = pp;
        }
    }
}

__device__ __forceinline__ bool any_bits(const float4& a) {
    return ((__float_as_uint(a.x) | __float_as_uint(a.y) | __float_as_uint(a.z) | __float_as_uint(a.w)) & 0x7fffffffu) != 0u;
}

__global__ __launch_bounds__(kBlock) void k_compact_gradient_rows(uint32_t n, const float4* __restrict__ act12,
                                                                 const uint32_t* __restrict__ tiles_count,
                                                                 const float* __restrict__ feat, float4* __restrict__ grad16,
                                                                 float4* __restrict__ records, uint32_t capacity,
                                                                 uint32_t* __restrict__ count) {
    const uint32_t i = blockIdx.x * kBlock + threadIdx.x;
    const uint32_t lane = threadIdx.x & 63;
    float4 g0, g1, g2, g3;
    bool have = false;
    if (i < n && tiles_count[i] != 0) {
        g0 = grad16[4 * (size_t)i + 0];
        g1 = grad16[4 * (size_t)i + 1];
        g2 = grad16[4 * (size_t)i + 2];
        g3 = grad16[4 * (size_t)i + 3];
// ... 102 lines not shown
                                       bool second_launch, const LazyMoments& lazy, const Regularisation& reg) {
    if (n == 0 || block_end <= block_begin) return;
    EarlyOwnership own;
    own.walked = wave_walked; own.split_block = split_block; own.extra_end = extra_end;
    AdamParams a12, a48;
    fill_adam(a12, lr12, 12, beta1, beta2, eps, step);
    fill_adam(a48, lr48, 48, beta1, beta2, eps, step);
    static int num_cus = 0;
    if (num_cus == 0) {
        int dev = 0;
        hipDeviceProp_t prop;
        if (hipGetDevice(&dev) == hipSuccess && hipGetDeviceProperties(&prop, dev) == hipSuccess) num_cus = prop.multiProcessorCount;
        if (num_cus <= 0) num_cus = 256;
    }
    const uint32_t nblocks = block_end - block_begin;
    static int wgs_per_cu = 0, wgs_per_cu2 = 0;
    if (wgs_per_cu == 0) {
        const char* e = getenv("GUT_EARLY_WGS_PER_CU");
        wgs_per_cu = e ? atoi(e) : 1;
        if (wgs_per_cu < 1 || wgs_per_cu > 8) wgs_per_cu = 1;
        const char* e2 = getenv("GUT_EARLY_WGS_PER_CU2");
        wgs_per_cu2 = e2 ? atoi(e2) : (e ? wgs_per_cu : 2);
        if (wgs_per_cu2 < 1 || wgs_per_cu2 > 8) wgs_per_cu2 = wgs_per_cu;
    }
    const uint32_t cap = (uint32_t)(second_launch ? wgs_per_cu2 : wgs_per_cu) * (uint32_t)num_cus;
    const uint32_t grid = nblocks < cap ? nblocks : cap;
    static int narrow_first = -1;
    if (narrow_first < 0) {
        const char* e = getenv("GUT_EARLY_NARROW");
        narrow_first = e ? atoi(e) : 1;
    }
    if (reg.on()) {
#if GUT_NARROW_REGULARISED
        auto kern = lazy.wave_step ? ((narrow_first && !second_launch) ? k_adam_rows_without_gradient_narrow<true, Regularisation>
                                                                       : k_adam_rows_without_gradient<true, true, Regularisation>)
                                   : k_adam_rows_without_gradient<false, true, Regularisation>;
#else
        auto kern = lazy.wave_step ? k_adam_rows_without_gradient<true, true, Regularisation>
                                   : k_adam_rows_without_gradient<false, true, Regularisation>;
#endif
        hipLaunchKernelGGL(kern, dim3(grid), dim3(kBlock), 0, s, a12, a48, n, tiles_count,
                           reinterpret_cast<float4*>(raw12), reinterpret_cast<float4*>(raw_m), reinterpret_cast<float4*>(raw_v),
                           reinterpret_cast<float4*>(sh48), reinterpret_cast<float4*>(sh_m), reinterpret_cast<float4*>(sh_v),
                           reinterpret_cast<float4*>(act12_out), block_begin, block_end, own, second_launch ? 1u : 0u, lazy, reg);
        return;
    }
    if (lazy.wave_step && narrow_first && !second_launch) {
        hipLaunchKernelGGL(k_adam_rows_without_gradient_narrow<false>, dim3(grid), dim3(kBlock), 0, s, a12, a48, n, tiles_count,
                           reinterpret_cast<float4*>(raw12), reinterpret_cast<float4*>(raw_m), reinterpret_cast<float4*>(raw_v),
                           reinterpret_cast<float4*>(sh48), reinterpret_cast<float4*>(sh_m), reinterpret_cast<float4*>(sh_v),
                           reinterpret_cast<float4*>(act12_out), block_begin, block_end, own, second_launch ? 1u : 0u, lazy);
        return;
    }
    auto kern = lazy.wave_step ? k_adam_rows_without_gradient<true, false> : k_adam_rows_without_gradient<false, false>;
    hipLaunchKernelGGL(kern, dim3(grid), dim3(kBlock), 0, s, a12, a48, n, tiles_count,
                       reinterpret_cast<float4*>(raw12), reinterpret_cast<float4*>(raw_m), reinterpret_cast<float4*>(raw_v),
                       reinterpret_cast<float4*>(sh48), reinterpret_cast<float4*>(sh_m), reinterpret_cast<float4*>(sh_v),
                       reinterpret_cast<float4*>(act12_out), block_begin, block_end, own, second_launch ? 1u : 0u, lazy);
}

constexpr uint32_t kRegLossThreads = 1024;
__global__ __launch_bounds__(kRegLossThreads) void k_regularisation_loss(uint32_t n, const float2* __restrict__ partials, float lambda_opacity,
                                                                        float lambda_scale, float* __restrict__ out_opacity,
                                                                        float* __restrict__ out_scale, float* __restrict__ loss) {
    __shared__ double s_sig[kRegLossThreads], s_exp[kRegLossThreads];
    const uint32_t waves = (n + 63u) / 64u;
    double a = 0.0, b = 0.0;
#pragma unroll 8
    for (uint32_t w = threadIdx.x; w < waves; w += kRegLossThreads) {
        const float2 p = partials[w];
        a += (double)p.x;
        b += (double)p.y;
    }
    s_sig[threadIdx.x] = a;
    s_exp[threadIdx.x] = b;
    __syncthreads();
    for (uint32_t h = kRegLossThreads / 2; h > 0; h >>= 1) {
        if (threadIdx.x < h) {
            s_sig[threadIdx.x] += s_sig[threadIdx.x + h];
            s_exp[threadIdx.x] += s_exp[threadIdx.x + h];
        }
// ... 77 lines not shown
    if (n == 0 || tiles == 0) return;
    hipLaunchKernelGGL(k_mark_walked_waves, dim3(tiles), dim3(kBlock), 0, s, n, reinterpret_cast<const uint2*>(ranges), tile_walked,
                       ids, wave_walked);
}
}

namespace gut {
template <bool kRawEager>
__global__ __launch_bounds__(kBlock) void k_sync_moments(uint32_t n, float4* __restrict__ m12, float4* __restrict__ v12,
                                                        float4* __restrict__ m48, float4* __restrict__ v48, LazyMoments lz) {
    const uint32_t wave = blockIdx.x * (kBlock / 64) + (threadIdx.x >> 6), lane = threadIdx.x & 63;
    const uint32_t wave_first = wave * 64u;
    if (wave_first >= n) return;
    const uint32_t seen = lz.wave_step[wave];
    if (seen >= lz.t) return;
    const uint32_t d = lz.t - seen;
    const uint32_t k = d < lz.len ? d : lz.len - 1u;
    if (d >= lz.len && lz.overrun && lane == 0) *lz.overrun = 1u;
    const float f1 = lz.pow1[k], f2 = lz.pow2[k];
    const uint32_t rows_here = min(64u, n - wave_first);
    for (uint32_t q = lane; !kRawEager && q < rows_here * 3u; q += 64u) {
        float4 a = m12[(size_t)wave_first * 3 + q], b = v12[(size_t)wave_first * 3 + q];
        scale4(a, f1); scale4(b, f2);
        m12[(size_t)wave_first * 3 + q] = a; v12[(size_t)wave_first * 3 + q] = b;
    }
    for (uint32_t q = lane; q < rows_here * 12u; q += 64u) {
        float4 a = m48[(size_t)wave_first * 12 + q], b = v48[(size_t)wave_first * 12 + q];
        scale4(a, f1); scale4(b, f2);
        m48[(size_t)wave_first * 12 + q] = a; v48[(size_t)wave_first * 12 + q] = b;
    }
    __builtin_amdgcn_fence(__ATOMIC_RELEASE, "wavefront");
    if (lane == 0) lz.wave_step[wave] = lz.t;
}
}

namespace gut {
__global__ __launch_bounds__(256) void k_resize_sph_rows(uint32_t n, uint32_t in_width, uint32_t out_width, const float* __restrict__ in,
                                                         float* __restrict__ out) {
    const size_t idx = (size_t)blockIdx.x * 256u + threadIdx.x;
    if (idx >= (size_t)n * out_width) return;
    const uint32_t row = (uint32_t)(idx / out_width), col = (uint32_t)(idx - (size_t)row * out_width);
    out[idx] = col < in_width ? in[(size_t)row * in_width + col] : 0.0f;
}

void launch_resize_sph_rows(hipStream_t s, uint32_t n, uint32_t in_width, uint32_t out_width, const float* in, float* out) {
    const size_t total = (size_t)n * out_width;
    if (total == 0) return;
    hipLaunchKernelGGL(k_resize_sph_rows, dim3((unsigned)((total + 255) / 256)), dim3(256), 0, s, n, in_width, out_width, in, out);
}

void launch_pack_activate_fields(hipStream_t s, uint32_t n, const float* pos, const float* dns, const float* rot, const float* scl,
                                 float* act12) {
    if (n == 0) return;
    hipLaunchKernelGGL(k_pack_activate_fields, dim3((n + kBlock - 1) / kBlock), dim3(kBlock), 0, s, n, pos, dns,
                       reinterpret_cast<const float4*>(rot), scl, reinterpret_cast<float4*>(act12));
}
}

gut::LazyMoments gut_make_lazy(const GutLazyMoments* lazy, uint32_t step) {
    gut::LazyMoments lz;
    if (lazy && lazy->d_wave_step && lazy->d_pow_beta1 && lazy->d_pow_beta2 && lazy->table_len >= 2 && step >= 1) {
        lz.wave_step = lazy->d_wave_step; lz.pow1 = lazy->d_pow_beta1; lz.pow2 = lazy->d_pow_beta2; lz.len = lazy->table_len; lz.t = step;
        lz.overrun = lazy->d_overrun;
    }
    return lz;
}

gut::Regularisation gut_make_reg(const GutRegularisation* reg) {
    gut::Regularisation r;
    if (reg && (reg->density_coeff != 0.0f || reg->scale_coeff != 0.0f)) {
        r.density_coeff = reg->density_coeff;
        r.scale_coeff = reg->scale_coeff;
        r.partials = reinterpret_cast<float2*>(reg->d_partials);
    }
    return r;
}

extern "C" {

int gut_sync_moments_ex(void* stream, uint32_t num_particles, float* d_raw_m, float* d_raw_v, float* d_sh_m, float* d_sh_v,
                        const GutLazyMoments* lazy, uint32_t step, const GutRegularisation* reg) {
    if (num_particles == 0) return 0;
    if (!d_raw_m || !d_raw_v || !d_sh_m || !d_sh_v || !lazy) return 1;
    gut::LazyMoments lz = gut_make_lazy(lazy, step ? step : 1u);
    if (!lz.wave_step) return 3;
    lz.t = step;
    const uint32_t waves = (num_particles + 63u) / 64u;
    auto kern = gut_make_reg(reg).on() ? gut::k_sync_moments<true> : gut::k_sync_moments<false>;
    hipLaunchKernelGGL(kern, dim3((waves + 3u) / 4u), dim3(gut::kBlock), 0, static_cast<hipStream_t>(stream), num_particles,
                       reinterpret_cast<float4*>(d_raw_m), reinterpret_cast<float4*>(d_raw_v), reinterpret_cast<float4*>(d_sh_m),
                       reinterpret_cast<float4*>(d_sh_v), lz);
    return hipGetLastError() == hipSuccess ? 0 : 2;
}

int gut_sync_moments(void* stream, uint32_t num_particles, float* d_raw_m, float* d_raw_v, float* d_sh_m, float* d_sh_v,
                     const GutLazyMoments* lazy, uint32_t step) {
    return gut_sync_moments_ex(stream, num_particles, d_raw_m, d_raw_v, d_sh_m, d_sh_v, lazy, step, nullptr);
}

int gut_regularisation_loss(void* stream, uint32_t num_particles, const float* d_partials, float lambda_opacity, float lambda_scale,
                            float* d_opacity_loss, float* d_scale_loss, float* d_loss) {
    if (!d_opacity_loss || !d_scale_loss) return 1;
    if (num_particles && !d_partials) return 1;
    hipLaunchKernelGGL(gut::k_regularisation_loss, dim3(1), dim3(gut::kRegLossThreads), 0, static_cast<hipStream_t>(stream), num_particles,
                       reinterpret_cast<const float2*>(d_partials), lambda_opacity, lambda_scale, d_opacity_loss, d_scale_loss, d_loss);
    return hipGetLastError() == hipSuccess ? 0 : 2;
}

int gut_regularisation_gradient(void* stream, uint32_t num_particles, const float* d_raw12, float* d_raw_grad12,
                                const GutRegularisation* reg) {
    if (num_particles == 0) return 0;
    if (!d_raw12 || !d_raw_grad12) return 1;
    const gut::Regularisation r = gut_make_reg(reg);
    if (!r.on()) return 0;
    hipLaunchKernelGGL(gut::k_add_regularisation_gradient, dim3((num_particles + gut::kBlock - 1) / gut::kBlock), dim3(gut::kBlock), 0,
                       static_cast<hipStream_t>(stream), num_particles, reinterpret_cast<const float4*>(d_raw12),
                       reinterpret_cast<float4*>(d_raw_grad12), r);
    return hipGetLastError() == hipSuccess ? 0 : 2;
}

int gut_activate_pack(void* stream, uint32_t num_particles, const float* d_raw12, float* d_act12) {
    if (num_particles == 0) return 0;
    if (!d_raw12 || !d_act12) return 1;
    hipLaunchKernelGGL(gut::k_activate_pack, dim3((num_particles + gut::kBlock - 1) / gut::kBlock), dim3(gut::kBlock), 0,
// ... 184 lines not shown
```

3dgrut_amd/native.py:

```python
import ctypes as C
import os
import math

import numpy as np
import torch

from . import _capi
from .dp import (RecordExchange, allgather_rows_, allgather_rows_async, allreduce_max_, allreduce_max_async, allreduce_mean_, allreduce_sum_async,
                 assert_replicas_identical)
from .losses import photometric_loss
from .tracer import SplatRaster, Tracer

RAW_COLS = dict(positions=slice(0, 3), density=slice(3, 4), rotation=slice(4, 8), scale=slice(8, 11))
_RAW_MOMENTS_EAGER = _capi.GutRegularisation(1.0, 1.0, None)


def spatial_permutation(positions: torch.Tensor, bits: int = 10) -> torch.Tensor:
    p = positions.detach().to(torch.float64)
    lo, hi = p.min(0).values, p.max(0).values
    q = ((p - lo) / (hi - lo).clamp_min(1e-12) * ((1 << bits) - 1)).to(torch.int64).clamp_(0, (1 << bits) - 1)

    def spread(v):
        v = (v | (v << 16)) & 0x030000FF
        v = (v | (v << 8)) & 0x0300F00F
        v = (v | (v << 4)) & 0x030C30C3
        v = (v | (v << 2)) & 0x09249249
        return v

    code = spread(q[:, 0]) | (spread(q[:, 1]) << 1) | (spread(q[:, 2]) << 2)
    return torch.argsort(code, stable=True)


class NativeGaussianModel:

    def __init__(self, scene: dict, device="cuda", sh_degree=3, background_color="black", spatial_order=False):
        n = scene["positions"].shape[0]
        self.spatial_order = bool(spatial_order)
        self.permutation = None
        if self.spatial_order and n:
            perm = spatial_permutation(torch.as_tensor(np.ascontiguousarray(scene["positions"], np.float32))).numpy()
            scene = {k: np.asarray(v)[perm] for k, v in scene.items()}
            self.permutation = torch.as_tensor(perm, device=device)
        dens = np.clip(np.asarray(scene["density"], np.float64), 1e-6, 1 - 1e-6)
        raw = np.zeros((n, 12), np.float32)
        raw[:, 0:3] = scene["positions"]
        raw[:, 3:4] = np.log(dens / (1 - dens))
        raw[:, 4:8] = scene["rotation"]
        raw[:, 8:11] = np.log(np.asarray(scene["scale"], np.float64))
        self.raw = torch.as_tensor(raw, device=device)
        self.features = torch.as_tensor(np.ascontiguousarray(scene["features"], np.float32), device=device)
        self.n_active_features = int(sh_degree)
        self.max_n_features = 3
        self.background_color = background_color
        self.device = device

    @classmethod
    def from_tensors(cls, raw, features, sh_degree=3, background_color="black", spatial_order=False, permutation=None):
        m = cls.__new__(cls)
        if raw.dim() != 2 or raw.shape[1] != 12 or features.shape != (raw.shape[0], 48):
            raise ValueError("from_tensors: raw must be [N,12] and features [N,48]")
        m.raw, m.features = raw.contiguous(), features.contiguous()
        m.spatial_order, m.permutation = bool(spatial_order), permutation
        m.n_active_features, m.max_n_features = int(sh_degree), 3
        m.background_color, m.device = background_color, raw.device
        return m

    @property
    def num_gaussians(self):
        return self.raw.shape[0]

    @property
    def positions(self):
        return self.raw[:, 0:3]

    def get_rotation(self):
        return torch.nn.functional.normalize(self.raw[:, 4:8], dim=1)

    def get_scale(self):
        return torch.exp(self.raw[:, 8:11])

    def get_density(self):
        return torch.sigmoid(self.raw[:, 3:4])

    def get_features(self):
        return self.features

    def background(self, T_to_world, rays_d, rgb, opacity, train=False):
        if self.background_color == "white":
            rgb = rgb + (1.0 - opacity)
        elif self.background_color == "random" and train:
            rgb = rgb + torch.rand_like(rays_d) * (1.0 - opacity)
        return rgb, opacity


class NativeTrainStep:
    OVERLAP_MIN_GAUSSIANS = 1_000_000
    PROBE_FIRST, PROBE_LAST = 2, 9

    def __init__(self, model: NativeGaussianModel, tracer: Tracer, scene_extent=1.0, world_size=1, selective=False,
                 betas=(0.9, 0.999), eps=1e-15, fused_sh_adam=True, rank=0, fused_loss=True, lambda_l1=0.8, lambda_ssim=0.2,
                 dp_chunks=4, dp_chunk_min_rows=1 << 20, fuse_epilogue=True, schedule=None,
                 overlap_optimizer=None, dp_exchange="sparse", dp_side_stream=True, lazy_moments=True, lambda_opacity=0.0,
                 lambda_scale=0.0):
        self.model = model
        self.tracer = tracer
        self.raster: SplatRaster = tracer.tracer_wrapper
        self.world_size = world_size
        self.selective = selective
        self.betas, self.eps = betas, eps
        self._lib = _capi.load()
        dev = model.raw.device
        n = model.num_gaussians
        lr12 = np.zeros(12, np.float32)
        lr12[0:3] = 1.6e-4 * scene_extent
        lr12[3] = 0.05
        lr12[4:8] = 0.001
        lr12[8:11] = 0.005
        lr48 = np.full(48, 0.000125, np.float32)
        lr48[0:3] = 0.0025
        self.lr12, self.lr48 = lr12, lr48
        self.schedule = schedule
        if schedule is not None:
            self.lr12[0:3] = schedule.position_lr
            model.n_active_features = schedule.n_active_features
        z = lambda c: torch.zeros((n, c), dtype=torch.float32, device=dev)
        self.m12, self.v12, self.m48, self.v48 = z(12), z(12), z(48), z(48)
        self.fused = bool(fused_sh_adam)
        self.lazy_moments = bool(lazy_moments) and self.fused and not selective
        self.LAZY_TABLE = 1024
        k = np.arange(self.LAZY_TABLE, dtype=np.float64)
        self._pow1 = torch.as_tensor((float(np.float32(betas[0])) ** k).astype(np.float32), device=dev)
        self._pow2 = torch.as_tensor((float(np.float32(betas[1])) ** k).astype(np.float32), device=dev)
        self.wave_step = None
        self._lazy_overrun = torch.zeros(1, dtype=torch.int32, device=dev)
        self._step_id = 0
        self.fused_loss = bool(fused_loss)
        self.fuse_epilogue = bool(fuse_epilogue)
        self.overlap_optimizer = (bool(getattr(model, "spatial_order", False)) and model.num_gaussians >= self.OVERLAP_MIN_GAUSSIANS) \
            if overlap_optimizer is None else bool(overlap_optimizer)
        self._overlap_probe = dict(on=[], off=[], done=False) if (overlap_optimizer is None and self.overlap_optimizer) else None
        self.dp_chunks, self.dp_chunk_min_rows = max(1, int(dp_chunks)), int(dp_chunk_min_rows)
        if dp_exchange not in ("sparse", "dense"):
            raise ValueError("dp_exchange must be 'sparse' or 'dense'")
        self.dp_exchange = dp_exchange
        self.dp_side_stream = bool(dp_side_stream) and not selective
        self._side = None
        self.lambda_l1, self.lambda_ssim = float(lambda_l1), float(lambda_ssim)
        self.lambda_opacity, self.lambda_scale = float(lambda_opacity), float(lambda_scale)
        self._raw_eager = self._regularised()
        self._reg_partials = None
        self._loss_ws = None
        self._loss3 = None
        self._cam_ring = None
        self._cam_dev = None
        self._act_key = None
        self.rank = int(rank)
        self.force_exchange = os.environ.get("GUT_DP_FORCE_COLLECTIVES") == "1"
        self._exchange = RecordExchange(max(1, world_size))
        self.replica_check_every = 500
        self.post_backward_hook = None
        self.fused_statistics = None
        self.row_listeners = []
        self.resize_workspace()
        self.phase_timing = False
        self._phase_events = []

    @property
    def probe_pending(self):
        p = self._overlap_probe
        one_pass = self.fused and self.world_size <= 1 and not self.force_exchange and self.fuse_epilogue \
            and (self.post_backward_hook is None or self.fused_statistics is not None)
        return p is not None and not p["done"] and one_pass and not self.selective

    def resize_workspace(self):
        n = self.model.num_gaussians
        dev = self.model.raw.device
        self._act_key = None
        if getattr(self, "lazy_moments", False):
            self.wave_step = torch.full(((n + 63) // 64,), int(getattr(self, "step_id", 0)), dtype=torch.int32, device=dev)
        self.act = torch.empty((n, 12), dtype=torch.float32, device=dev)
        self.g12 = torch.empty((n, 12), dtype=torch.float32, device=dev)
        self._reg_partials = torch.empty((max(1, (n + 63) // 64), 2), dtype=torch.float32, device=dev)
        if self.fused:
            w = max(1, self.world_size)
            nchunks = 1
            sparse = getattr(self, "dp_exchange", "dense") == "sparse"
            if (w > 1 or getattr(self, "force_exchange", False)) and n >= self.dp_chunk_min_rows and not sparse:
                nchunks = self.dp_chunks
            rows = (((n + nchunks - 1) // nchunks) + 255) // 256 * 256 if n else 0
            self.chunks = [(r0, min(n, r0 + rows)) for r0 in range(0, n, rows)] if n else []
            if sparse:
                self.g12.zero_()
                self.mrgb = [torch.zeros((w, r1 - r0, 3), dtype=torch.float32, device=dev) for r0, r1 in self.chunks]
                self.records = torch.empty((max(n, 1), _capi.GRADIENT_RECORD_FLOATS), dtype=torch.float32, device=dev)
                self.rec_count = torch.zeros(1, dtype=torch.int32, device=dev)
                if getattr(self, "_exchange", None) is not None:
                    self._exchange.reset()
                self.wave_flags = torch.zeros(((n + 63) // 64,), dtype=torch.uint8, device=dev)
                self.exchanged_records = 0
            else:
                self.mrgb = [torch.empty((w, r1 - r0, 3), dtype=torch.float32, device=dev) for r0, r1 in self.chunks]
            self.mrgb_local = torch.empty((n, 3), dtype=torch.float32, device=dev)
            self.cams = torch.zeros((w, 3), dtype=torch.float32, device=dev)
            self.g48 = None
        else:
            self.g48 = torch.empty((n, 48), dtype=torch.float32, device=dev)

    def _regularised(self):
        return self.lambda_opacity != 0.0 or self.lambda_scale != 0.0

    def _regularisation(self, row0=0):
        n = self.model.num_gaussians
        if not self._regularised() or n == 0:
            return None
        return _capi.GutRegularisation(self.lambda_opacity / n, self.lambda_scale / (3 * n), self._reg_partials.data_ptr() + 8 * (row0 // 64))

    def _regularisation_losses(self, loss_buffer=None):
        out = torch.empty((2,), dtype=torch.float32, device=self.model.raw.device)
        st = torch.cuda.current_stream(out.device).cuda_stream
        rc = self._lib.gut_regularisation_loss(C.c_void_p(st), self.model.num_gaussians, self._reg_partials.data_ptr(), self.lambda_opacity,
                                              self.lambda_scale, out.data_ptr(), out.data_ptr() + 4,
                                              None if loss_buffer is None else loss_buffer.data_ptr())
        if rc:
            raise RuntimeError(f"[3dgut] regularisation_loss failed ({rc})")
        return out[0], out[1]

    def _lazy(self):
        if not self.lazy_moments or self.wave_step is None:
            return None
        return _capi.GutLazyMoments(self.wave_step.data_ptr(), self._pow1.data_ptr(), self._pow2.data_ptr(), self.LAZY_TABLE,
                                    self._lazy_overrun.data_ptr())

    @property
    def step_id(self):
        return self._step_id

    @step_id.setter
    def step_id(self, value):
        self.set_step(value)

    def set_step(self, step):
        step = int(step)
        if step < 0:
            raise ValueError("step must be >= 0")
        if step != self._step_id:
            self.sync_moments()
            self._step_id = step
            if self.wave_step is not None:
                self.wave_step.fill_(step)

    def state_dict(self):
        self.sync_moments()
        return dict(step=int(self._step_id), exp_avg_raw=self.m12.clone(), exp_avg_sq_raw=self.v12.clone(),
                    exp_avg_features=self.m48.clone(), exp_avg_sq_features=self.v48.clone(), lr_raw=self.lr12.copy())

    def load_state_dict(self, state):
        n = self.model.num_gaussians
        for key, dst in (("exp_avg_raw", self.m12), ("exp_avg_sq_raw", self.v12), ("exp_avg_features", self.m48), ("exp_avg_sq_features", self.v48)):
            src = state[key]
            if tuple(src.shape) != tuple(dst.shape):
                raise ValueError(f"load_state_dict: {key} has shape {tuple(src.shape)}, the trainer holds {n} Gaussians ({tuple(dst.shape)})")
            dst.copy_(src)
        if "lr_raw" in state:
            self.lr12[:] = np.asarray(state["lr_raw"], np.float32)
        self._step_id = int(state["step"])
        if self.wave_step is not None:
            self.wave_step.fill_(self._step_id)

    def sync_moments(self):
        lz = self._lazy()
        if lz is None or self.model.num_gaussians == 0 or not self.model.raw.is_cuda:
            return
        st = torch.cuda.current_stream(self.model.raw.device).cuda_stream
        eager = _RAW_MOMENTS_EAGER if self._raw_eager else None
        with torch.cuda.device(self.model.raw.device):
            rc = self._lib.gut_sync_moments_ex(C.c_void_p(st), self.model.num_gaussians, self.m12.data_ptr(), self.v12.data_ptr(),
                                               self.m48.data_ptr(), self.v48.data_ptr(), C.byref(lz), int(self.step_id),
                                               None if eager is None else C.byref(eager))
        if rc:
            raise RuntimeError(f"[3dgut] sync_moments failed ({rc})")
        if int(self._lazy_overrun.item()):
            self._lazy_overrun.zero_()
            raise RuntimeError(f"[3dgut] lazy moment decay: a wave's stored Adam moments had missed {self.LAZY_TABLE} or more steps "
                               "(wave_step does not belong to step_id: use set_step() / load_state_dict() to resume, never a bare "
                               "assignment of wave_step or of the moments)")

    def reorder(self, perm: torch.Tensor):
        self.sync_moments()
        m = self.model
        perm = perm.to(m.raw.device)
        m.raw = m.raw[perm].contiguous()
        m.features = m.features[perm].contiguous()
        self.m12, self.v12 = self.m12[perm].contiguous(), self.v12[perm].contiguous()
        self.m48, self.v48 = self.m48[perm].contiguous(), self.v48[perm].contiguous()
        if m.permutation is not None:
            m.permutation = m.permutation[perm]
        for fn in self.row_listeners:
            fn(perm)
        self.resize_workspace()

    def tune_placement(self, attempts=4):
        m = self.model
# ... 50 lines not shown
        del held
        self._act_key = None
        torch.cuda.empty_cache()
        self.placement_trials_ms = times
        return times

    def restore_spatial_order(self):
        m = self.model
        if m.permutation is None:
            m.permutation = torch.arange(m.num_gaussians, device=m.raw.device)
        self.reorder(spatial_permutation(m.raw[:, 0:3]))
        m.spatial_order = True

    def activate(self):
        raw = self.model.raw
        if self._act_key == (raw.data_ptr(), raw._version, raw.shape[0]):
            return self.act
        st = torch.cuda.current_stream(self.model.raw.device).cuda_stream
        rc = self._lib.gut_activate_pack(C.c_void_p(st), self.model.num_gaussians, self.model.raw.data_ptr(), self.act.data_ptr())
        if rc:
            raise RuntimeError(f"[3dgut] activate_pack failed ({rc})")
        return self.act

    def _adam(self, p, g, m, v, lr, vis):
        st = torch.cuda.current_stream(p.device).cuda_stream
        lr_arr = (C.c_float * len(lr))(*[float(x) for x in lr])
        rc = self._lib.gut_adam_step(C.c_void_p(st), p.shape[0], p.shape[1], p.data_ptr(), g.data_ptr(), m.data_ptr(),
                                     v.data_ptr(), lr_arr, self.betas[0], self.betas[1], self.eps,
                                     0 if self.selective else self.step_id + 1,
                                     None if vis is None else vis.data_ptr())
        if rc:
            raise RuntimeError(f"[3dgut] adam_step failed ({rc})")

    def forward(self, batch, train=True):
        m = self.model
        act = self.activate()
        sensor, poses = Tracer.create_camera_parameters(batch)
        rgba, dist_, hits, vis = self.raster.trace(self.step_id, m.n_active_features, act, m.features, batch.rays_ori.contiguous(),
                                                  batch.rays_dir.contiguous(), None, sensor, poses.timestamps_us[0],
                                                  poses.timestamps_us[1], poses.T_world_sensors[0], poses.T_world_sensors[1])
        self._ctx = (batch, sensor, poses, rgba, dist_)
        return rgba, dist_, hits, vis

    def _sensor_position(self, batch):
        t = batch.T_to_world.reshape(4, 4)[:3, 3].to(torch.float32)
        if t.is_cuda:
            return t.contiguous()
        if self._cam_ring is None:
            self._cam_ring = [torch.empty(3, dtype=torch.float32).pin_memory() for _ in range(8)]
            self._cam_dev = [torch.empty(3, dtype=torch.float32, device=self.model.raw.device) for _ in range(8)]
        k = self.step_id % len(self._cam_ring)
        self._cam_ring[k].copy_(t)
        self._cam_dev[k].copy_(self._cam_ring[k], non_blocking=True)
        return self._cam_dev[k]

    def _mark(self, evs):
        if evs is not None:
            e = torch.cuda.Event(enable_timing=True)
            e.record()
            evs.append(e)

    def phase_times_mean(self, reset=True):
        names = ("forward", "loss", "backward", "update")
        if not self._phase_events:
            return {}
        torch.cuda.synchronize(self.model.raw.device)
        acc = [0.0] * len(names)
        for evs in self._phase_events:
            for k in range(len(names)):
                acc[k] += evs[k].elapsed_time(evs[k + 1])
        n = len(self._phase_events)
        spans = sorted(evs[0].elapsed_time(evs[len(names)]) for evs in self._phase_events)
        self.last_step_spans_ms = dict(min=spans[0], median=spans[len(spans) // 2], max=spans[-1])
        if os.environ.get("GUT_STEP_SPANS") == "1":
            self.last_step_spans_ms["all"] = [[round(evs[k].elapsed_time(evs[k + 1]), 3) for k in range(len(names))] for evs in self._phase_events]
        if spans[-1] > 3.0 * spans[len(spans) // 2]:
            worst = max(range(n), key=lambda i: self._phase_events[i][0].elapsed_time(self._phase_events[i][len(names)]))
            evs = self._phase_events[worst]
            self.last_step_spans_ms["slowest"] = dict(index=worst, **{names[k]: evs[k].elapsed_time(evs[k + 1]) for k in range(len(names))})
        if reset:
            self._phase_events = []
        return {names[k]: acc[k] / n for k in range(len(names))}

    def step(self, batch):
        try:
            return self._step(batch)
        except Exception as err:
            if getattr(self, "_reg_set", False):
                self._reg_set = False
                self.raster.set_regularisation(None)
            if getattr(self, "_early_queued", False):
                self._early_queued = False
                try:
                    self.raster.finish_optimizer_step_without_gradient()
                except Exception as finish_err:
                    raise RuntimeError(f"[3dgut] the optimiser step begun on the side stream could not be finished after "
                                       f"{type(err).__name__}: {err}; the trainer's state is not usable: {finish_err}") from err
                self._act_key = None
                self._probe_evs = None
                self._end_of_step(None)
            raise

    def _step(self, batch):
        m = self.model
        if self.world_size > 1 and self.replica_check_every and not getattr(self, "_replicas_checked_at_start", False):
            self._replicas_checked_at_start = True
            assert_replicas_identical([self.model.raw, self.model.features, self.m12, self.v12, self.m48, self.v48], self.world_size,
                                      what=f"before the first step (step counter {self.step_id})")
        evs = [] if self.phase_timing else None
        self._mark(evs)
        if self._regularised() != self._raw_eager:
            self.sync_moments()
            self._raw_eager = self._regularised()
        reg = self._regularisation()
        one_pass = self.fused and self.world_size <= 1 and not self.force_exchange and self.fuse_epilogue \
            and (self.post_backward_hook is None or self.fused_statistics is not None)
        use_overlap, probe_evs = self.overlap_optimizer, None
        probe = self._overlap_probe
        if probe is not None and one_pass and not self.selective:
            if self.PROBE_FIRST <= self.step_id <= self.PROBE_LAST:
                use_overlap = (self.step_id % 2) == 1
                probe_evs = (torch.cuda.Event(enable_timing=True), torch.cuda.Event(enable_timing=True))
                probe_evs[0].record()
                probe["on" if use_overlap else "off"].append(probe_evs)
            elif self.step_id > self.PROBE_LAST and not probe["done"] and all(e[1].query() for e in probe["on"] + probe["off"]):
                t_on = min((a.elapsed_time(b) for a, b in probe["on"]), default=float("inf"))
                t_off = min((a.elapsed_time(b) for a, b in probe["off"]), default=float("inf"))
                probe.update(done=True, ms_on=t_on, ms_off=t_off)
                if probe["on"] and probe["off"]:
                    self.overlap_optimizer = use_overlap = t_on <= t_off
        early = one_pass and use_overlap and not self.selective
        self._probe_evs = probe_evs
        rgba, dist_, hits, vis = self.forward(batch)
        if one_pass and reg is not None:
            self.raster.set_regularisation(reg)
            self._reg_set = True
        if early:
            self.raster.optimize_rows_without_gradient(m.raw, self.m12, self.v12, m.features, self.m48, self.v48, self.lr12,
                                                       self.lr48, self.betas, self.eps, self.step_id + 1, self.act, lazy=self._lazy())
            self._early_queued = True
        self._mark(evs)
        gt = batch.rgb_gt
        if self.fused_loss and m.background_color in ("black", "white") and gt.dtype == torch.float32 and gt.is_contiguous() \
                and gt.numel() == rgba.shape[0] * rgba.shape[1] * 3:
            H, W = rgba.shape[0], rgba.shape[1]
            need = self._lib.gut_photometric_workspace_bytes(H, W)
            if self._loss_ws is None or self._loss_ws.numel() * 4 < need:
                self._loss_ws = torch.empty(((need + 3) // 4,), dtype=torch.float32, device=rgba.device)
            self._loss3 = torch.empty((3,), dtype=torch.float32, device=rgba.device)
            rgba_grad = torch.empty_like(rgba)
            st = torch.cuda.current_stream(rgba.device).cuda_stream
            rc = self._lib.gut_photometric_loss(C.c_void_p(st), H, W, rgba.data_ptr(), gt.data_ptr(),
                                                1.0 if m.background_color == "white" else 0.0, self.lambda_l1, self.lambda_ssim,
                                                self._loss_ws.data_ptr(), self._loss3.data_ptr(), rgba_grad.data_ptr())
            if rc:
                raise RuntimeError(f"[3dgut] photometric_loss failed ({rc})")
            loss = self._loss3[0]
            pred_rgb = rgba[..., :3].unsqueeze(0)
            if m.background_color == "white":
                pred_rgb = pred_rgb + (1.0 - rgba[..., 3:].unsqueeze(0))
        else:
            rgba_leaf = rgba.detach().requires_grad_(True)
            pred_rgb = rgba_leaf[..., :3].unsqueeze(0)
            pred_opacity = rgba_leaf[..., 3:].unsqueeze(0)
            pred_rgb, pred_opacity = m.background(batch.T_to_world, batch.rays_dir, pred_rgb, pred_opacity, True)
            loss = photometric_loss(pred_rgb, gt, self.lambda_l1, self.lambda_ssim)
            loss.backward()
            rgba_grad = rgba_leaf.grad
        self._mark(evs)
        _, sensor, poses, _, _ = self._ctx
        bwd_args = (self.step_id, m.n_active_features, self.act, m.features, batch.rays_ori.contiguous(),
                    batch.rays_dir.contiguous(), None, sensor, poses.timestamps_us[0], poses.timestamps_us[1],
                    poses.T_world_sensors[0], poses.T_world_sensors[1], rgba, rgba_grad, dist_, None)
        vmask = None
        if self.fused:
            w = max(1, self.world_size)
            exchange = w > 1 or self.force_exchange
            if one_pass:
                self.raster.trace_bwd(*bwd_args, skip_epilogue=True)
                self._mark(evs)
                vmask = vis.reshape(-1) if self.selective else None
                stats = self.fused_statistics() if self.fused_statistics is not None else None
                if stats is not None:
                    self.raster.set_position_gradient_statistics(*stats)
                self.raster.optimize_after_bwd(m.n_active_features, None, m.raw, self.m12, self.v12, m.features,
                                               self.m48, self.v48, self.lr12, self.lr48, self.betas, self.eps,
                                               0 if self.selective else self.step_id + 1, vmask, self.act, lazy=self._lazy())
                self._reg_set = False
                self._act_key = (m.raw.data_ptr(), m.raw._version, m.raw.shape[0])
                return self._finish_step(evs, loss, pred_rgb, vis, hits, reg)
            if self.dp_exchange == "sparse":
                self._sparse_exchange_and_update(batch, bwd_args, vis, evs, w, exchange, reg)
                return self._finish_step(evs, loss, pred_rgb, vis, hits, reg)
            local_mrgb = self.mrgb_local if exchange else self.mrgb[0][0]
            self.raster.trace_bwd(*bwd_args, raw_parameter_grads=True, compact_radiance_grads=True, out=(self.g12, local_mrgb))
            self._mark(evs)
            cam_local = self._sensor_position(batch)
            if self.post_backward_hook is not None:
                self.post_backward_hook(self.g12[:, 0:3], cam_local)
            works = []
            if exchange:
                allgather_rows_(self.cams, cam_local, w)
                if self.selective:
                    allreduce_max_(vis, w)
                for (r0, r1), gathered in zip(self.chunks, self.mrgb):
                    works.append((allreduce_sum_async(self.g12[r0:r1], w),
                                  allgather_rows_async(gathered, self.mrgb_local[r0:r1], w)))
            else:
                self.cams[0].copy_(cam_local)
            if self.selective:
                vmask = vis.reshape(-1)
            st = torch.cuda.current_stream(m.raw.device).cuda_stream
            f32p = C.POINTER(C.c_float)
            for k, ((r0, r1), gathered) in enumerate(zip(self.chunks, self.mrgb)):
                if works:
                    works[k][0].wait()
                    works[k][1].wait()
                lz = self._lazy()
                if lz is not None:
                    lz = _capi.GutLazyMoments(self.wave_step.data_ptr() + 4 * (r0 // 64), self._pow1.data_ptr(), self._pow2.data_ptr(), self.LAZY_TABLE)
                reg_c = self._regularisation(r0)
# ... 106 lines not shown
                mine = torch.cat([mine, tail[0][r, :tail[1][r]]])
            pg = torch.zeros((n, 3), dtype=torch.float32, device=m.raw.device)
            pg[mine[:, 11].contiguous().view(torch.int32).long()] = mine[:, 0:3]
            self.post_backward_hook(pg, cam_local)
        vmask = vis.reshape(-1) if self.selective else None
        rc = self._lib.gut_sh_adam_step_regularised(
            C.c_void_p(st), n, m.n_active_features, w, self.cams.data_ptr(), slabs.data_ptr(), self.g12.data_ptr(), 1.0 / w,
            m.raw.data_ptr(), self.m12.data_ptr(), self.v12.data_ptr(), m.features.data_ptr(), self.m48.data_ptr(),
            self.v48.data_ptr(), self.lr12.ctypes.data_as(f32p), self.lr48.ctypes.data_as(f32p), self.betas[0], self.betas[1],
            self.eps, 0 if self.selective else self.step_id + 1, None if vmask is None else vmask.data_ptr(), self.act.data_ptr(),
            n, _capi.ADAM_CLEAR_CONSUMED_GRADS, self.wave_flags.data_ptr() if side_on else None,
            None if self._lazy() is None else C.byref(self._lazy()), None if reg is None else C.byref(reg))
        if rc:
            raise RuntimeError(f"[3dgut] sh_adam_step failed ({rc})")
        if side_on:
            main.wait_stream(self._side)
        self._act_key = (m.raw.data_ptr(), m.raw._version, m.raw.shape[0])

    def _end_of_step(self, evs):
        self._early_queued = False
        if self.world_size > 1 and self.replica_check_every and self.step_id % self.replica_check_every == 0:
            assert_replicas_identical([self.model.raw, self.model.features, self.m12, self.v12, self.m48, self.v48], self.world_size,
                                      what=f"after step {self.step_id}")
        if getattr(self, "_probe_evs", None) is not None:
            self._probe_evs[1].record()
            self._probe_evs = None
        if evs is not None:
            self._phase_events.append(evs)
        if self.schedule is not None:
            lr, deg = self.schedule.after_optimizer_step(self.step_id)
            self.lr12[0:3] = lr
            self.model.n_active_features = deg
        self._step_id += 1
        if self.lazy_moments and self._step_id % (self.LAZY_TABLE // 2) == 0:
            self.sync_moments()

    def render(self, batch, train=False):
        return self.tracer.render(self.model, batch, train=train, frame_id=self.step_id)
```

3dgrut_amd/tracer.py:

```python
import ctypes as C
import enum
import math
import os

import numpy as np
import torch

from . import _capi
from .cameras import ShutterType as DatasetShutterType
from .pose import SensorPose3D, sensor_pose_from_c2w


class ShutterType(enum.IntEnum):
    ROLLING_TOP_TO_BOTTOM = 0
    ROLLING_LEFT_TO_RIGHT = 1
    ROLLING_BOTTOM_TO_TOP = 2
    ROLLING_RIGHT_TO_LEFT = 3
    GLOBAL = 4


SHUTTER_TYPE_MAP = {d: ShutterType[d.name] for d in DatasetShutterType}


def plugin_shutter_type(value):
# ... 333 lines not shown
        dist_g = None if ray_hit_distance_grd is None else _check_f32_cuda(ray_hit_distance_grd, "rayHitDistanceGradient")
        opts = dict(dtype=torch.float32, device=dev)
        if out is not None:
            pos_g, dns_g, rot_g, scl_g, alb_g, spec_g = (_check_f32_cuda(t, "gradient output", (c,)) for t, c in zip(out, (3, 1, 4, 3, 3, 45)))
            if any(t.shape[0] != n or not o.is_contiguous() for t, o in zip((pos_g, dns_g, rot_g, scl_g, alb_g, spec_g), out)):
                raise RuntimeError("[3dgut] gradient outputs must be contiguous [N,c] tensors with the forward's number of rows")
        else:
            pos_g, dns_g, rot_g, scl_g, alb_g, spec_g = (torch.empty((n, c), **opts) for c in (3, 1, 4, 3, 3, 45))
        cam = self._camera(sensor_params, ts_start, ts_end, pose_start, pose_end)
        stream = torch.cuda.current_stream(dev).cuda_stream
        ptr = lambda t: t.data_ptr() if n else None
        with torch.cuda.device(dev):
            rc = self._lib.gut_trace_bwd_model_fields(self._handle, C.c_void_p(stream), int(frame_number) & 0xFFFFFFFF, int(num_active_features),
                                                      n, W, H, ray_ori.data_ptr(), ray_dir.data_ptr(), C.byref(cam), rgba.data_ptr(),
                                                      rgba_g.data_ptr(), dist.data_ptr(), None if dist_g is None else dist_g.data_ptr(),
                                                      ptr(pos_g), ptr(dns_g), ptr(rot_g), ptr(scl_g), ptr(alb_g), ptr(spec_g))
        _capi.check(rc, "trace_bwd_model_fields")
        return pos_g, dns_g, rot_g, scl_g, alb_g, spec_g

    def set_position_gradient_statistics(self, norm_accum, norm_denom):
        if norm_accum is None:
            _capi.check(self._lib.gut_set_position_gradient_statistics(self._handle, None, None), "set_position_gradient_statistics")
            return
        if not (norm_accum.is_cuda and norm_accum.dtype == torch.float32 and norm_accum.is_contiguous()
                and norm_denom.is_cuda and norm_denom.dtype == torch.int32 and norm_denom.is_contiguous()
                and norm_accum.numel() == norm_denom.numel()):
            raise RuntimeError("[3dgut] statistics buffers: contiguous GPU tensors, float32 accum and int32 denom of equal length")
        self._stat_rows = int(norm_accum.numel())
        _capi.check(self._lib.gut_set_position_gradient_statistics(self._handle, norm_accum.data_ptr(), norm_denom.data_ptr()),
                    "set_position_gradient_statistics")

    def set_regularisation(self, reg):
        _capi.check(self._lib.gut_set_regularisation(self._handle, None if reg is None else C.byref(reg)), "set_regularisation")

    def optimize_after_bwd(self, num_active_features, camera_position, raw12, raw_m, raw_v, sh48, sh_m, sh_v, lr12, lr48, betas, eps,
                           step, visibility=None, act_out=None, lazy=None):
        f32p = C.POINTER(C.c_float)
        stream = torch.cuda.current_stream(raw12.device).cuda_stream
        with torch.cuda.device(raw12.device):
            rc = self._lib.gut_optimize_after_bwd(self._handle, C.c_void_p(stream), int(num_active_features),
                                                  None if camera_position is None else camera_position.data_ptr(),
                                                  raw12.data_ptr(), raw_m.data_ptr(), raw_v.data_ptr(), sh48.data_ptr(), sh_m.data_ptr(),
                                                  sh_v.data_ptr(), lr12.ctypes.data_as(f32p), lr48.ctypes.data_as(f32p), betas[0],
                                                  betas[1], eps, int(step), None if visibility is None else visibility.data_ptr(),
                                                  None if act_out is None else act_out.data_ptr(), None if lazy is None else C.byref(lazy))
        _capi.check(rc, "optimize_after_bwd")

    def optimize_rows_without_gradient(self, raw12, raw_m, raw_v, sh48, sh_m, sh_v, lr12, lr48, betas, eps, step, act_out=None, lazy=None):
        f32p = C.POINTER(C.c_float)
        stream = torch.cuda.current_stream(raw12.device).cuda_stream
        with torch.cuda.device(raw12.device):
            rc = self._lib.gut_optimize_rows_without_gradient(
                self._handle, C.c_void_p(stream), raw12.data_ptr(), raw_m.data_ptr(), raw_v.data_ptr(), sh48.data_ptr(),
                sh_m.data_ptr(), sh_v.data_ptr(), lr12.ctypes.data_as(f32p), lr48.ctypes.data_as(f32p), betas[0], betas[1], eps,
                int(step), None if act_out is None else act_out.data_ptr(), None if lazy is None else C.byref(lazy))
        _capi.check(rc, "optimize_rows_without_gradient")

    def finish_optimizer_step_without_gradient(self):
        dev = torch.device("cuda", self.device_index)
        with torch.cuda.device(dev):
            rc = self._lib.gut_optimize_finish_without_gradient(self._handle, C.c_void_p(torch.cuda.current_stream(dev).cuda_stream))
        _capi.check(rc, "optimize_finish_without_gradient")

    def compact_gradient_rows(self, act12, records, count):
        if records.shape[0] < act12.shape[0] or records.shape[1] != _capi.GRADIENT_RECORD_FLOATS or not records.is_contiguous():
            raise ValueError("records must be a contiguous [>= num_particles, 16] float32 tensor")
# ... 222 lines not shown
```

include/gut_hip.h:

```cpp
#ifndef GUT_HIP_H
#define GUT_HIP_H

#include <stddef.h>
#include <stdint.h>

#ifdef __cplusplus
extern "C" {
#endif

#define GUT_ABI_VERSION 6

typedef struct gut_context* gut_handle;

enum { GUT_SHUTTER_ROLLING_TOP_TO_BOTTOM = 0, GUT_SHUTTER_ROLLING_LEFT_TO_RIGHT = 1,
       GUT_SHUTTER_ROLLING_BOTTOM_TO_TOP = 2, GUT_SHUTTER_ROLLING_RIGHT_TO_LEFT = 3, GUT_SHUTTER_GLOBAL = 4 };
enum { GUT_CAMERA_OPENCV_PINHOLE = 0, GUT_CAMERA_OPENCV_FISHEYE = 1 };

typedef struct GutCamera {
    int32_t model;
    int32_t shutter;
    float principal_point[2];
    float focal_length[2];
    float radial_coeffs[6];
    float tangential_coeffs[2];
// ... 207 lines not shown
                        const GutLazyMoments* lazy );

int gut_mark_walked_waves(gut_handle h, void* stream, uint8_t* d_wave_flags);
int gut_adam_unwalked_waves(void* stream, uint32_t num_particles, const uint8_t* d_wave_flags, float* d_raw12, float* d_raw_m,
                            float* d_raw_v, float* d_sh48, float* d_sh_m, float* d_sh_v, const float* lr12, const float* lr48,
                            float beta1, float beta2, float eps, uint32_t step, float* d_act12_out);
int gut_adam_unwalked_waves_ex(void* stream, uint32_t num_particles, const uint8_t* d_wave_flags, float* d_raw12, float* d_raw_m,
                               float* d_raw_v, float* d_sh48, float* d_sh_m, float* d_sh_v, const float* lr12, const float* lr48,
                               float beta1, float beta2, float eps, uint32_t step, float* d_act12_out, const GutLazyMoments* lazy);

typedef struct GutRegularisation {
    float density_coeff;
    float scale_coeff;
    float* d_partials;
} GutRegularisation;
int gut_set_regularisation(gut_handle h, const GutRegularisation* reg);
int gut_sh_adam_step_regularised(void* stream, uint32_t num_particles, int32_t sh_degree, uint32_t num_views,
                                 const float* d_camera_positions, float* d_mrgb, float* d_raw_grad12, float grad_scale,
                                 float* d_raw12, float* d_raw_m, float* d_raw_v, float* d_sh48, float* d_sh_m, float* d_sh_v,
                                 const float* lr12, const float* lr48, float beta1, float beta2, float eps, uint32_t step,
                                 const float* d_visibility, float* d_act12_out, uint32_t mrgb_view_stride, uint32_t flags,
                                 const uint8_t* d_wave_flags, const GutLazyMoments* lazy, const GutRegularisation* reg);
int gut_adam_unwalked_waves_regularised(void* stream, uint32_t num_particles, const uint8_t* d_wave_flags, float* d_raw12,
                                        float* d_raw_m, float* d_raw_v, float* d_sh48, float* d_sh_m, float* d_sh_v, const float* lr12,
                                        const float* lr48, float beta1, float beta2, float eps, uint32_t step, float* d_act12_out,
                                        const GutLazyMoments* lazy, const GutRegularisation* reg);
int gut_sync_moments_ex(void* stream, uint32_t num_particles, float* d_raw_m, float* d_raw_v, float* d_sh_m, float* d_sh_v,
                        const GutLazyMoments* lazy, uint32_t step, const GutRegularisation* reg);
int gut_regularisation_gradient(void* stream, uint32_t num_particles, const float* d_raw12, float* d_raw_grad12,
                                const GutRegularisation* reg);
int gut_regularisation_loss(void* stream, uint32_t num_particles, const float* d_partials, float lambda_opacity, float lambda_scale,
                            float* d_opacity_loss, float* d_scale_loss, float* d_loss);

int gut_position_gradient_statistics(void* stream, uint32_t num_particles, const float* d_position_grad, uint32_t grad_stride,
                                     const float* d_positions, uint32_t position_stride, const float* d_sensor_position,
                                     float* d_norm_accum, int32_t* d_norm_denom);
int gut_set_position_gradient_statistics(gut_handle h, float* d_norm_accum, int32_t* d_norm_denom);

int gut_mcmc_relocation(void* stream, int32_t n, const float* d_opacities, const float* d_scales, const int32_t* d_ratios,
                        const float* d_binoms, int32_t n_max, float* d_new_opacities, float* d_new_scales);

int gut_mcmc_perturb(void* stream, uint32_t num_particles, float* d_raw12, float* d_act12, float noise_scale, uint64_t seed,
                     uint64_t step, const float* d_unit_normals);

const char* gut_last_error(void);
int gut_abi_version(void);

#ifdef __cplusplus
}
#endif
#endif
```

Baseline: 463.8 images/s.

## Defer SH Adam updates for unwalked rows and replay them lazily in projection

```diff
diff --git a/3dgrut_amd/_capi.py b/3dgrut_amd/_capi.py
--- a/3dgrut_amd/_capi.py
+++ b/3dgrut_amd/_capi.py
@@ -69,6 +69,11 @@
     _fields_ = [("density_coeff", C.c_float), ("scale_coeff", C.c_float), ("d_partials", C.c_void_p)]
 
 
+class GutDeferredSh(C.Structure):
+    _fields_ = [("d_sh_step", C.c_void_p), ("d_step_ring", C.c_void_p), ("ring_len", C.c_uint32), ("steps_applied", C.c_uint32),
+                ("d_sh_m", C.c_void_p), ("d_sh_v", C.c_void_p), ("lazy", GutLazyMoments)]
+
+
 EXPORTS = ("gut_default_config", "gut_create", "gut_destroy", "gut_trace", "gut_trace_bwd", "gut_collect_times",
            "gut_get_stats", "gut_debug_buffer", "gut_debug_copy", "gut_kernel_times", "gut_kernel_times_mean", "gut_last_error", "gut_abi_version",
            "gut_ssim_workspace_bytes", "gut_ssim_forward", "gut_ssim_backward",
@@ -79,7 +84,8 @@
            "gut_trace_model_fields", "gut_trace_bwd_model_fields", "gut_position_gradient_statistics",
            "gut_set_position_gradient_statistics", "gut_mcmc_perturb", "gut_trace_raw_model_fields", "gut_set_regularisation",
            "gut_sh_adam_step_regularised", "gut_adam_unwalked_waves_regularised", "gut_sync_moments_ex", "gut_regularisation_gradient",
-           "gut_regularisation_loss", "gut_image_metrics_workspace_bytes", "gut_image_metrics")
+           "gut_regularisation_loss", "gut_image_metrics_workspace_bytes", "gut_image_metrics", "gut_set_deferred_sh",
+           "gut_sync_deferred_sh")
 
 _lib = None
 
@@ -162,6 +168,9 @@
     lib.gut_sync_moments_ex.argtypes = lib.gut_sync_moments.argtypes + [reg_p]
     lib.gut_regularisation_gradient.argtypes = [vp, u32, vp, vp, reg_p]
     lib.gut_regularisation_loss.argtypes = [vp, u32, vp, C.c_float, C.c_float, vp, vp, vp]
+    defer_p = C.POINTER(GutDeferredSh)
+    lib.gut_set_deferred_sh.argtypes = [vp, defer_p]
+    lib.gut_sync_deferred_sh.argtypes = [vp, u32, vp, vp, vp, lazy_p, defer_p, u32]
     lib.gut_compact_gradient_rows.argtypes = [vp, vp, vp, vp, u32, vp]
     lib.gut_scatter_gradient_records.argtypes = [vp, vp, u32, u32, vp, vp]
     lib.gut_scatter_gradient_records_dev.argtypes = [vp, vp, vp, u32, u32, vp, vp]
diff --git a/3dgrut_amd/build.py b/3dgrut_amd/build.py
--- a/3dgrut_amd/build.py
+++ b/3dgrut_amd/build.py
@@ -47,7 +47,7 @@
 def build(force=False, verbose=False):
     hipcc = os.environ.get("HIPCC", "/opt/rocm/bin/hipcc")
     os.makedirs(OBJ_DIR, exist_ok=True)
-    headers = [os.path.join(CSRC, "gut_internal.h"), os.path.join(CSRC, "gut_render_common.h"), os.path.join(CSRC, "gut_render.hip"),
+    headers = [os.path.join(CSRC, "gut_internal.h"), os.path.join(CSRC, "gut_render_common.h"), os.path.join(CSRC, "gut_lazy_adam.h"), os.path.join(CSRC, "gut_render.hip"),
                os.path.join(HERE, "..", "include", "gut_hip.h")]
     objs = []
     for src, extra in UNITS:
diff --git a/3dgrut_amd/csrc/gut_api.cpp b/3dgrut_amd/csrc/gut_api.cpp
--- a/3dgrut_amd/csrc/gut_api.cpp
+++ b/3dgrut_amd/csrc/gut_api.cpp
@@ -126,6 +126,7 @@
     float* stat_accum = nullptr;
     int32_t* stat_denom = nullptr;
     GutRegularisation reg{};
+    GutDeferredSh defer{};
     DevBuf cam_pos;
     DevBuf wave_sums, block_prefix, scan_total;
     bool timing_main_stream = true, timing_side_stream = true;
@@ -158,6 +159,7 @@
         uint32_t extra_end;
         GutLazyMoments lazy;
         GutRegularisation reg;
+        GutDeferredSh defer;
     } early_args{};
     bool marks_valid = false;
     DevBuf wave_walked;
@@ -306,6 +308,7 @@
 
 static int launch_early_part2(gut_context* h, hipStream_t s);
 gut::LazyMoments gut_make_lazy(const GutLazyMoments* lazy, uint32_t step);
+gut::LazyMoments gut_make_lazy(const GutLazyMoments* lazy, uint32_t step, const GutDeferredSh* defer);
 gut::Regularisation gut_make_reg(const GutRegularisation* reg);
 
 extern "C" {
@@ -537,10 +540,26 @@
         gut::launch_resize_sph_rows(s, n, w, 48u, d_particle_radiance, h->sph_widened.as<float>());
         d_particle_radiance = h->sph_widened.as<float>();
     }
+    gut::ShCatchUp catch_up;
+    const bool deferring = h->defer.d_sh_step != nullptr && n != 0;
+    if (deferring) {
+        if (d_features_albedo || h->cfg.particle_radiance_sph_degree != 3)
+            return fail("gut_trace: the deferred SH update takes the concatenated [N,48] radiance of particle_radiance_sph_degree=3");
+        const gut::LazyMoments lz = gut_make_lazy(&h->defer.lazy, h->defer.steps_applied + 1u, &h->defer);
+        if (!lz.defer.sh_step || !h->defer.d_sh_m || !h->defer.d_sh_v)
+            return fail("gut_trace: incomplete GutDeferredSh (stamps, ring, lazy moments and the [N,48] moments are all needed)");
+        catch_up.defer = lz.defer;
+        catch_up.wave_step = lz.wave_step; catch_up.pow1 = lz.pow1; catch_up.pow2 = lz.pow2; catch_up.pow_len = lz.len;
+        catch_up.overrun = lz.overrun;
+        catch_up.steps_applied = h->defer.steps_applied;
+        catch_up.p48 = reinterpret_cast<float4*>(const_cast<float*>(d_particle_radiance));
+        catch_up.m48 = reinterpret_cast<const float4*>(h->defer.d_sh_m);
+        catch_up.v48 = reinterpret_cast<const float4*>(h->defer.d_sh_v);
+    }
     gut::launch_project(s, v, h->consts, n, num_active_features, d_particle_density, d_particle_radiance,
                         h->tiles_count.as<uint32_t>(), h->proj_pos.as<float>(), h->conic_opacity.as<float>(),
                         h->extent.as<float>(), h->depth.as<float>(), h->feat.as<float>(), d_particle_visibility,
-                        h->wave_sums.as<uint32_t>(), d_features_albedo, clears);
+                        h->wave_sums.as<uint32_t>(), d_features_albedo, clears, deferring ? &catch_up : nullptr);
     mark(1);
     static const bool early_after_project = getenv("GUT_EARLY_AFTER_PROJECT") != nullptr;
     if (early_after_project) {
@@ -968,9 +987,14 @@
     if (h->early_ran && ((lazy && lazy->d_wave_step) != (h->early_args.lazy.d_wave_step != nullptr)))
         return fail("gut_optimize_after_bwd: lazy moment decay must be the same as in gut_optimize_rows_without_gradient");
     if (launch_early_part2(h, s)) return 1;
-    const gut::LazyMoments lz = gut_make_lazy(lazy, step);
     const gut::Regularisation reg = gut_make_reg(h->early_ran ? &h->early_args.reg : &h->reg);
     h->reg = GutRegularisation{};
+    const GutDeferredSh defer = h->early_ran ? h->early_args.defer : h->defer;
+    h->defer = GutDeferredSh{};
+    if (defer.d_sh_step && (reg.on() || d_visibility || !lazy || !lazy->d_wave_step || defer.steps_applied + 1u != step))
+        return fail("gut_optimize_after_bwd: the deferred SH update needs lazy moments, no regulariser, no visibility mask, and the "
+                    "step after the one its forward was given (%u + 1, got %u)", defer.steps_applied, step);
+    const gut::LazyMoments lz = gut_make_lazy(lazy, step, &defer);
     if (lz.wave_step && h->cfg.k_buffer_size == 0 && h->m && !h->marks_valid) {
         gut::launch_mark_walked_waves(s, h->n, (uint32_t)h->tiles, h->ranges.as<uint32_t>(), h->trav_fwd.as<uint32_t>(),
                                       (h->lazy_order ? h->ids_ordered : h->ids_sorted).as<uint32_t>(), h->wave_walked.as<uint8_t>());
@@ -1024,6 +1048,18 @@
     return 0;
 }
 
+int gut_set_deferred_sh(gut_handle h, const GutDeferredSh* defer) {
+    if (!h) return fail("gut_set_deferred_sh: null handle");
+    if (defer && defer->d_sh_step &&
+        (!defer->d_step_ring || defer->ring_len < 2 || !defer->d_sh_m || !defer->d_sh_v || !defer->lazy.d_wave_step ||
+         !defer->lazy.d_pow_beta1 || !defer->lazy.d_pow_beta2 || defer->lazy.table_len < 2))
+        return fail("gut_set_deferred_sh: stamps, ring, the [N,48] moments and complete lazy moments are all needed");
+    std::lock_guard<std::mutex> lock(h->mu);
+    if (h->early_ran) return fail("gut_set_deferred_sh: an optimiser step is half applied");
+    h->defer = (defer && defer->d_sh_step) ? *defer : GutDeferredSh{};
+    return 0;
+}
+
 int gut_optimize_finish_without_gradient(gut_handle h, void* stream_) {
     if (!h) return fail("gut_optimize_finish_without_gradient: null handle");
     std::lock_guard<std::mutex> lock(h->mu);
@@ -1036,6 +1072,7 @@
     h->stat_accum = nullptr;
     h->stat_denom = nullptr;
     h->reg = GutRegularisation{};
+    h->defer = GutDeferredSh{};
     HIP_TRY(h->grad16.ensure(sizeof(float) * 16 * (size_t)h->n));
     HIP_TRY(hipMemsetAsync(h->grad16.p, 0, h->grad16.cap, s));
     if (launch_early_part2(h, s)) return 1;
@@ -1043,7 +1080,7 @@
                                      h->grad16.as<float>(), h->tiles_count.as<uint32_t>(), h->feat.as<float>(), ea.raw12, ea.raw_m,
                                      ea.raw_v, ea.sh48, ea.sh_m, ea.sh_v, ea.lr12, ea.lr48, ea.beta1, ea.beta2, ea.eps, ea.step, nullptr,
                                      ea.act12, true, ea.extra_end ? h->wave_walked.as<uint8_t>() : nullptr, ea.block_begin, ea.extra_end,
-                                     gut_make_lazy(&ea.lazy, ea.step), h->marks_valid ? h->wave_walked.as<uint8_t>() : nullptr,
+                                     gut_make_lazy(&ea.lazy, ea.step, &ea.defer), h->marks_valid ? h->wave_walked.as<uint8_t>() : nullptr,
                                      nullptr, nullptr, gut_make_reg(&ea.reg));
     HIP_TRY(hipGetLastError());
     if (h->early_wait_pending) {
@@ -1100,6 +1137,8 @@
     h->grad16_zero = true;
     return 0;
 }
+
+constexpr uint32_t kDeferredFirstShare = 100u;
 
 int gut_optimize_rows_without_gradient(gut_handle h, void* stream_, float* d_raw12, float* d_raw_m, float* d_raw_v, float* d_sh48,
                                        float* d_sh_m, float* d_sh_v, const float* lr12, const float* lr48, float beta1, float beta2,
@@ -1139,11 +1178,16 @@
     }
     const uint32_t nblocks = (h->n + gut::kBlock - 1) / gut::kBlock;
     const gut::Regularisation reg = gut_make_reg(&h->reg);
-    const uint32_t percent = split_percent >= 0 ? (uint32_t)split_percent : ((lazy && lazy->d_wave_step && !reg.on()) ? 60u : 25u);
+    const bool deferring = h->defer.d_sh_step != nullptr;
+    if (deferring && (reg.on() || !lazy || !lazy->d_wave_step || h->defer.steps_applied + 1u != step))
+        return fail("gut_optimize_rows_without_gradient: the deferred SH update needs lazy moments, no regulariser, and the step after "
+                    "the one its forward was given (%u + 1, got %u)", h->defer.steps_applied, step);
+    const uint32_t percent = split_percent >= 0 ? (uint32_t)split_percent
+                                                : (deferring ? kDeferredFirstShare : ((lazy && lazy->d_wave_step && !reg.on()) ? 60u : 25u));
     const uint32_t first = (uint32_t)((uint64_t)nblocks * percent / 100u);
     gut::launch_adam_rows_without_gradient(h->side_stream, h->n, h->tiles_count.as<uint32_t>(), d_raw12, d_raw_m, d_raw_v, d_sh48,
                                            d_sh_m, d_sh_v, lr12, lr48, beta1, beta2, eps, step, d_act12_out, 0, first, nullptr, first, 0,
-                                           false, gut_make_lazy(lazy, step), reg);
+                                           false, gut_make_lazy(lazy, step, &h->defer), reg);
     HIP_TRY(hipGetLastError());
     gut_context::EarlyArgs& ea = h->early_args;
     ea.raw12 = d_raw12; ea.raw_m = d_raw_m; ea.raw_v = d_raw_v; ea.sh48 = d_sh48; ea.sh_m = d_sh_m; ea.sh_v = d_sh_v;
@@ -1154,6 +1198,7 @@
     ea.lazy = GutLazyMoments{};
     if (lazy) ea.lazy = *lazy;
     ea.reg = h->reg;
+    ea.defer = h->defer;
     ea.extra_end = (h->cfg.k_buffer_size == 0 && h->m) ? (uint32_t)((uint64_t)nblocks * (uint32_t)h->early_extra_percent / 100u) : 0u;
     h->early_part2_pending = first < nblocks || ea.extra_end > 0;
     if (timing) {
@@ -1183,7 +1228,7 @@
                                            ea.sh_m, ea.sh_v, ea.lr12, ea.lr48, ea.beta1, ea.beta2, ea.eps, ea.step, ea.act12,
                                            ea.extra_end ? 0u : ea.block_begin, ea.block_end,
                                            ea.extra_end ? h->wave_walked.as<uint8_t>() : nullptr, ea.block_begin, ea.extra_end, true,
-                                           gut_make_lazy(&ea.lazy, ea.step), gut_make_reg(&ea.reg));
+                                           gut_make_lazy(&ea.lazy, ea.step, &ea.defer), gut_make_reg(&ea.reg));
     HIP_TRY(hipGetLastError());
     const bool timing = h->cfg.enable_kernel_timings != 0 && h->timing_side_stream && h->kev[14] && h->kev[15];
     if (timing) {
diff --git a/3dgrut_amd/csrc/gut_internal.h b/3dgrut_amd/csrc/gut_internal.h
--- a/3dgrut_amd/csrc/gut_internal.h
+++ b/3dgrut_amd/csrc/gut_internal.h
@@ -66,6 +66,12 @@
     unsigned long long pad[3];
 };
 
+struct DeferredSh {
+    uint32_t* sh_step = nullptr;
+    float* ring = nullptr;
+    uint32_t ring_len = 0;
+};
+
 struct LazyMoments {
     uint32_t* wave_step = nullptr;
     const float* pow1 = nullptr;
@@ -73,6 +79,20 @@
     uint32_t len = 0;
     uint32_t t = 0;
     uint32_t* overrun = nullptr;
+    DeferredSh defer;
+};
+
+struct ShCatchUp {
+    DeferredSh defer;
+    const uint32_t* wave_step = nullptr;
+    const float* pow1 = nullptr;
+    const float* pow2 = nullptr;
+    uint32_t pow_len = 0;
+    uint32_t steps_applied = 0;
+    uint32_t* overrun = nullptr;
+    float4* p48 = nullptr;
+    const float4* m48 = nullptr;
+    const float4* v48 = nullptr;
 };
 
 struct Regularisation {
@@ -95,7 +115,7 @@
                     const float* density12, const float* sph48, uint32_t* tiles_count, float* proj_pos,
                     float* conic_opacity, float* extent, float* depth, float* feat, float* visibility,
                     uint32_t* wave_sums , const float* sph_albedo ,
-                    const FrameClears& clears);
+                    const FrameClears& clears, const ShCatchUp* catch_up = nullptr );
 void launch_scan_wave_sums(hipStream_t s, uint32_t n, const uint32_t* wave_sums, uint32_t* block_prefix, uint32_t* total,
                            uint32_t* host_out , const uint32_t* walk_sums ,
                            uint32_t* tile_entries, uint32_t tiles, uint32_t* tile_start, uint32_t* tile_cursor);
diff --git a/3dgrut_amd/csrc/gut_lazy_adam.h b/3dgrut_amd/csrc/gut_lazy_adam.h
--- /dev/null
+++ b/3dgrut_amd/csrc/gut_lazy_adam.h
@@ -0,0 +1,57 @@
+#pragma once
+#include "gut_internal.h"
+
+namespace gut {
+
+struct LazyAdam {
+    float c1, c2s, b2s, eps;
+};
+__device__ __forceinline__ LazyAdam make_lazy_adam(float beta1, float beta2, float bias2_sqrt, float eps, const float2& dk) {
+    LazyAdam la;
+    la.c1 = beta1 * dk.x;
+    la.c2s = (beta2 * dk.y) * 0x1p+32f;
+    la.b2s = bias2_sqrt * 0x1p-16f;
+    la.eps = eps;
+    return la;
+}
+__device__ __forceinline__ void adam4_lazy(const LazyAdam& la, const float4& lr, float4& p, const float4& m, const float4& v) {
+#pragma clang fp contract(fast)
+#define GUT_ADAM_LANE(X) p.X -= lr.X * (la.c1 * m.X) * __builtin_amdgcn_rcpf(__builtin_amdgcn_sqrtf(la.c2s * v.X) * la.b2s + la.eps);
+    GUT_ADAM_LANE(x)
+    GUT_ADAM_LANE(y)
+    GUT_ADAM_LANE(z)
+    GUT_ADAM_LANE(w)
+#undef GUT_ADAM_LANE
+}
+
+__device__ __forceinline__ float2 pow_beta(const float* __restrict__ pow1, const float* __restrict__ pow2, uint32_t len, uint32_t* overrun,
+                                           uint32_t d) {
+    const uint32_t k = d < len ? d : len - 1u;
+    if (d >= len && overrun) *overrun = 1u;
+    return make_float2(pow1[k], pow2[k]);
+}
+
+constexpr uint32_t kShRingSlot = 64;
+
+__device__ __forceinline__ void write_sh_ring_slot(float* __restrict__ ring, uint32_t ring_len, uint32_t t, uint32_t lane, float lr,
+                                                   float bias2_sqrt, float eps, float beta1, float beta2) {
+    float* slot = ring + (size_t)(t % ring_len) * kShRingSlot;
+    if (lane < 48u) slot[lane] = lr;
+    else if (lane == 48u) slot[lane] = bias2_sqrt;
+    else if (lane == 49u) slot[lane] = eps;
+    else if (lane == 50u) slot[lane] = beta1;
+    else if (lane == 51u) slot[lane] = beta2;
+}
+
+__device__ __forceinline__ void replay_sh4(const DeferredSh& ds, const float* __restrict__ pow1, const float* __restrict__ pow2,
+                                           uint32_t pow_len, uint32_t* overrun, uint32_t seen, uint32_t from, uint32_t to, uint32_t col4,
+                                           float4& p, const float4& m, const float4& v) {
+    for (uint32_t s = from + 1u; s <= to; ++s) {
+        const float* slot = ds.ring + (size_t)(s % ds.ring_len) * kShRingSlot;
+        const float2 dk = pow_beta(pow1, pow2, pow_len, overrun, s > seen ? s - seen - 1u : 0u);
+        const LazyAdam la = make_lazy_adam(slot[50], slot[51], slot[48], slot[49], dk);
+        adam4_lazy(la, reinterpret_cast<const float4*>(slot)[col4], p, m, v);
+    }
+}
+
+}
diff --git a/3dgrut_amd/csrc/gut_project.hip b/3dgrut_amd/csrc/gut_project.hip
--- a/3dgrut_amd/csrc/gut_project.hip
+++ b/3dgrut_amd/csrc/gut_project.hip
@@ -1,4 +1,5 @@
 #include "gut_internal.h"
+#include "gut_lazy_adam.h"
 
 namespace gut {
 
@@ -345,7 +346,7 @@
 __device__ __forceinline__ float bcast(float v, int src_lane) { return __shfl(v, src_lane); }
 __device__ __forceinline__ int bcast(int v, int src_lane) { return __shfl(v, src_lane); }
 
-template <int kVariant, bool kRolling, bool kSplitSH>
+template <int kVariant, bool kRolling, bool kSplitSH, typename... CatchUp>
 __global__ __launch_bounds__(kBlock, 5) void k_project_on_tiles(ViewParams v, RenderConsts c, uint32_t n, int sh_degree,
                                                             const float4* __restrict__ density12,
                                                             const float* __restrict__ sph48,
@@ -354,7 +355,9 @@
                                                             float4* __restrict__ conic_opacity, float2* __restrict__ extent,
                                                             float* __restrict__ depth, float* __restrict__ feat,
                                                             float* __restrict__ visibility, uint32_t* __restrict__ wave_sums,
-                                                            FrameClears clr) {
+                                                            FrameClears clr, CatchUp... catch_up_arg) {
+    constexpr bool kCatchUp = sizeof...(CatchUp) != 0;
+    static_assert(!(kCatchUp && kSplitSH), "the deferred SH update is built for the concatenated [N,48] tensor");
     __shared__ float sh_lds[(kBlock / 64) * 32 * kShRow];
     __shared__ uint32_t s_bins[kBinWindow];
     __shared__ int s_red[16];
@@ -525,12 +528,13 @@
         const float4* src = reinterpret_cast<const float4*>(sph48 + (size_t)wave_first * 48);
         float Y[16];
         float inv_dist = 0.f, dist = 0.f;
-        if (vis) {
+        auto view_basis = [&]() {
             const float rx = a.x - v.s2w.t[0], ry = a.y - v.s2w.t[1], rz = a.z - v.s2w.t[2];
             dist = sqrtf(rx * rx + ry * ry + rz * rz);
             inv_dist = 1.0f / dist;
             sh_basis(sh_degree, rx * inv_dist, ry * inv_dist, rz * inv_dist, Y);
-        }
+        };
+        if (!kCatchUp && vis) view_basis();
         const int ncoef = (sh_degree + 1) * (sh_degree + 1);
         float4 shq[12];
         float alb0 = 0.f, alb1 = 0.f, alb2 = 0.f;
@@ -560,6 +564,36 @@
                 }
                 shq[it] = val;
             }
+        } else if constexpr (kCatchUp) {
+            const ShCatchUp& cu = (catch_up_arg, ...);
+            float4* blk = cu.p48 + (size_t)wave_first * 12;
+            const uint32_t w = (uint32_t)__builtin_amdgcn_readfirstlane((int)(wave_first >> 6));
+            const uint32_t have = cu.defer.sh_step[w], now = cu.steps_applied;
+            if (have < now) {
+                if (now - have >= cu.defer.ring_len && cu.overrun && lane == 0) *cu.overrun = 1u;
+                const uint32_t seen = cu.wave_step[w];
+                const float4* bm = cu.m48 + (size_t)wave_first * 12;
+                const float4* bv = cu.v48 + (size_t)wave_first * 12;
+#pragma unroll
+                for (int it = 0; it < 12; ++it) {
+                    const uint32_t q = (uint32_t)it * 64u + (uint32_t)lane;
+                    float4 val = make_float4(0.f, 0.f, 0.f, 0.f);
+                    if (q < rows_here * 12u) {
+                        val = blk[q];
+                        replay_sh4(cu.defer, cu.pow1, cu.pow2, cu.pow_len, cu.overrun, seen, have, now, q % 12u, val, bm[q], bv[q]);
+                        blk[q] = val;
+                    }
+                    shq[it] = val;
+                }
+                if (lane == 0) cu.defer.sh_step[w] = now;
+            } else {
+#pragma unroll
+                for (int it = 0; it < 12; ++it) {
+                    const uint32_t q = (uint32_t)it * 64u + (uint32_t)lane;
+                    const bool wanted = (q < rows_here * 12u) && ((vis_mask >> (q / 12u)) & 1ull);
+                    shq[it] = wanted ? blk[q] : make_float4(0.f, 0.f, 0.f, 0.f);
+                }
+            }
         } else {
 #pragma unroll
             for (int it = 0; it < 12; ++it) {
@@ -568,6 +602,7 @@
                 shq[it] = wanted ? src[q] : make_float4(0.f, 0.f, 0.f, 0.f);
             }
         }
+        if (kCatchUp && vis) view_basis();
 #pragma unroll
         for (int half = 0; half < 2; ++half) {
             if (kSplitSH) {
@@ -1149,7 +1184,7 @@
 void launch_project(hipStream_t s, const ViewParams& v, const RenderConsts& c, uint32_t n, int sh_degree,
                     const float* density12, const float* sph48, uint32_t* tiles_count, float* proj_pos,
                     float* conic_opacity, float* extent, float* depth, float* feat, float* visibility,
-                    uint32_t* wave_sums, const float* sph_albedo, const FrameClears& clears) {
+                    uint32_t* wave_sums, const float* sph_albedo, const FrameClears& clears, const ShCatchUp* catch_up) {
     if (n == 0) return;
     bool distorted = false;
     for (float k : v.radial) distorted |= (k != 0.0f);
@@ -1162,6 +1197,17 @@
     if (sph_albedo)
         kern = rolling ? (variant == 0 ? k_project_on_tiles<0, true, true> : (variant == 1 ? k_project_on_tiles<1, true, true> : k_project_on_tiles<2, true, true>))
                        : (variant == 0 ? k_project_on_tiles<0, false, true> : (variant == 1 ? k_project_on_tiles<1, false, true> : k_project_on_tiles<2, false, true>));
+    if (catch_up && !sph_albedo) {
+        auto kern_cu = rolling ? (variant == 0 ? k_project_on_tiles<0, true, false, ShCatchUp>
+                                               : (variant == 1 ? k_project_on_tiles<1, true, false, ShCatchUp> : k_project_on_tiles<2, true, false, ShCatchUp>))
+                               : (variant == 0 ? k_project_on_tiles<0, false, false, ShCatchUp>
+                                               : (variant == 1 ? k_project_on_tiles<1, false, false, ShCatchUp> : k_project_on_tiles<2, false, false, ShCatchUp>));
+        hipLaunchKernelGGL(kern_cu, dim3(blocks_for(n)), dim3(kBlock), 0, s, v, c, n, sh_degree,
+                           reinterpret_cast<const float4*>(density12), sph48, sph_albedo, tiles_count, reinterpret_cast<float2*>(proj_pos),
+                           reinterpret_cast<float4*>(conic_opacity), reinterpret_cast<float2*>(extent), depth, feat, visibility,
+                           wave_sums, clears, *catch_up);
+        return;
+    }
     hipLaunchKernelGGL(kern, dim3(blocks_for(n)), dim3(kBlock), 0, s, v, c, n, sh_degree,
                        reinterpret_cast<const float4*>(density12), sph48, sph_albedo, tiles_count, reinterpret_cast<float2*>(proj_pos),
                        reinterpret_cast<float4*>(conic_opacity), reinterpret_cast<float2*>(extent), depth, feat, visibility,
diff --git a/3dgrut_amd/csrc/gut_train.hip b/3dgrut_amd/csrc/gut_train.hip
--- a/3dgrut_amd/csrc/gut_train.hip
+++ b/3dgrut_amd/csrc/gut_train.hip
@@ -2,6 +2,7 @@
 #include <type_traits>
 
 #include "gut_internal.h"
+#include "gut_lazy_adam.h"
 
 namespace gut {
 
@@ -286,24 +287,8 @@
 #undef GUT_ADAM_LANE
 }
 
-struct LazyAdam {
-    float c1, c2s, b2s, eps;
-};
 __device__ __forceinline__ LazyAdam make_lazy_adam(const AdamParams& ap, const float2& dk) {
-    LazyAdam la;
-    la.c1 = ap.beta1 * dk.x;
-    la.c2s = (ap.beta2 * dk.y) * 0x1p+32f;
-    la.b2s = ap.bias2_sqrt * 0x1p-16f;
-    la.eps = ap.eps;
-    return la;
-}
-__device__ __forceinline__ void adam4_lazy(const LazyAdam& la, const float4& lr, float4& p, const float4& m, const float4& v) {
-#define GUT_ADAM_LANE(X) p.X -= lr.X * (la.c1 * m.X) * __builtin_amdgcn_rcpf(__builtin_amdgcn_sqrtf(la.c2s * v.X) * la.b2s + la.eps);
-    GUT_ADAM_LANE(x)
-    GUT_ADAM_LANE(y)
-    GUT_ADAM_LANE(z)
-    GUT_ADAM_LANE(w)
-#undef GUT_ADAM_LANE
+    return make_lazy_adam(ap.beta1, ap.beta2, ap.bias2_sqrt, ap.eps, dk);
 }
 
 __device__ __forceinline__ float reg_sigmoid(float d) { return 1.0f / (1.0f + expf(-d)); }
@@ -356,20 +341,24 @@
     float* wl = tile + wave * 64 * kRow;
     const uint32_t wave_first = blockIdx.x * kBlock + wave * 64u;
     const uint32_t rows_here = wave_first < sp.n ? min(64u, sp.n - wave_first) : 0u;
+    if (kScratch && !kReg && sp.lazy.defer.ring && blockIdx.x == 0 && threadIdx.x < 64)
+        write_sh_ring_slot(sp.lazy.defer.ring, sp.lazy.defer.ring_len, sp.lazy.t, threadIdx.x, sp.a48.lr[threadIdx.x], sp.a48.bias2_sqrt,
+                           sp.a48.eps, sp.a48.beta1, sp.a48.beta2);
     if (kScratch && sp.rows_with_tiles_only &&
         side_stream_owns_wave(sp.own, __ballot(i < sp.n && tiles_count[i] != 0) != 0ull, wave_first >> 6, blockIdx.x))
         return;
     if (!kScratch && sp.own.walked && wave_first < sp.n && sp.own.walked[wave_first >> 6] == 0) return;
     const uint32_t wave_index = wave_first >> 6;
-    bool lazy_wave = false;
+    bool lazy_wave = false, has_tiles = true;
     float2 dk = make_float2(1.0f, 1.0f);
     if (sp.lazy.wave_step && wave_first < sp.n) {
         dk = missed_decay(sp.lazy, wave_index);
         if (kScratch) {
-            const bool has_tiles = __ballot(i < sp.n && tiles_count[i] != 0) != 0ull;
+            has_tiles = __ballot(i < sp.n && tiles_count[i] != 0) != 0ull;
             lazy_wave = !has_tiles || (sp.rule_walked && sp.rule_walked[wave_index] == 0);
         }
     }
+    uint32_t* const sh_step = kReg ? nullptr : sp.lazy.defer.sh_step;
     if constexpr (kReg) {
         float sig = 0.0f, esum = 0.0f;
         if (i < sp.n) {
@@ -394,6 +383,7 @@
             p12[3 * (size_t)i + 0] = a; p12[3 * (size_t)i + 1] = b; p12[3 * (size_t)i + 2] = c;
             if (act12) activate_row(a, b, c, act12 + 3 * (size_t)i);
         }
+        if (sh_step && !has_tiles) return;
         float4* bp = p48 + (size_t)wave_first * 12;
         const float4* bm = m48 + (size_t)wave_first * 12;
         const float4* bv = v48 + (size_t)wave_first * 12;
@@ -406,6 +396,7 @@
             adam4_lazy(l48, make_float4(sp.a48.lr[col], sp.a48.lr[col + 1], sp.a48.lr[col + 2], sp.a48.lr[col + 3]), pp, bm[q], bv[q]);
             bp[q] = pp;
         }
+        if (sh_step && lane == 0 && rows_here) sh_step[wave_index] = sp.lazy.t;
         return;
     }
     float G[48];
@@ -525,6 +516,7 @@
         if (!lazy_wave) { bm[q] = mm; bv[q] = vv; }
     }
     if (sp.lazy.wave_step && !lazy_wave && lane == 0 && rows_here) sp.lazy.wave_step[wave_index] = sp.lazy.t;
+    if (kScratch && sh_step && lane == 0 && rows_here) sh_step[wave_index] = sp.lazy.t;
 }
 
 template <bool kLazy, bool kReg, typename... Reg>
@@ -592,6 +584,7 @@
                 p12[3 * (size_t)i + 2] = c;
                 if (act12) activate_row(a, b, c, act12 + 3 * (size_t)i);
             }
+            if (lazy.defer.sh_step && !has_tiles) continue;
             float4* bp = p48 + (size_t)wave_first * 12;
             const float4* bm = m48 + (size_t)wave_first * 12;
             const float4* bv = v48 + (size_t)wave_first * 12;
@@ -604,6 +597,7 @@
                 adam4_lazy(l48, s_lr48[col >> 2], pp, bm[q], bv[q]);
                 bp[q] = pp;
             }
+            if (lazy.defer.sh_step && lane == 0) lazy.defer.sh_step[wave_first >> 6] = lazy.t;
             continue;
         }
         if (mine) {
@@ -646,7 +640,7 @@
 #ifndef GUT_NARROW_REGULARISED
 #define GUT_NARROW_REGULARISED 0
 #endif
-template <bool kReg, typename... Reg>
+template <bool kReg, bool kSkipSh, typename... Reg>
 __global__ __launch_bounds__(kBlock) __attribute__((amdgpu_num_vgpr(16))) void k_adam_rows_without_gradient_narrow(
     AdamParams a12, AdamParams a48, uint32_t n, const uint32_t* __restrict__ tiles_count, float4* __restrict__ p12,
     float4* __restrict__ m12, float4* __restrict__ v12, float4* __restrict__ p48, float4* __restrict__ m48,
@@ -722,6 +716,7 @@
             if (act12) ra[o + 2] = activate_scale(x, nrm);
             __builtin_amdgcn_sched_barrier(0);
         }
+        if constexpr (kSkipSh) continue;
         float4* bp = p48 + (size_t)wave_first * 12;
         const float4* bm = m48 + (size_t)wave_first * 12;
         const float4* bv = v48 + (size_t)wave_first * 12;
@@ -890,7 +885,7 @@
     }
     if (reg.on()) {
 #if GUT_NARROW_REGULARISED
-        auto kern = lazy.wave_step ? ((narrow_first && !second_launch) ? k_adam_rows_without_gradient_narrow<true, Regularisation>
+        auto kern = lazy.wave_step ? ((narrow_first && !second_launch) ? k_adam_rows_without_gradient_narrow<true, false, Regularisation>
                                                                        : k_adam_rows_without_gradient<true, true, Regularisation>)
                                    : k_adam_rows_without_gradient<false, true, Regularisation>;
 #else
@@ -903,8 +898,9 @@
                            reinterpret_cast<float4*>(act12_out), block_begin, block_end, own, second_launch ? 1u : 0u, lazy, reg);
         return;
     }
-    if (lazy.wave_step && narrow_first && !second_launch) {
-        hipLaunchKernelGGL(k_adam_rows_without_gradient_narrow<false>, dim3(grid), dim3(kBlock), 0, s, a12, a48, n, tiles_count,
+    if (lazy.wave_step && narrow_first && !second_launch && !(lazy.defer.sh_step && wave_walked)) {
+        auto narrow = lazy.defer.sh_step ? k_adam_rows_without_gradient_narrow<false, true> : k_adam_rows_without_gradient_narrow<false, false>;
+        hipLaunchKernelGGL(narrow, dim3(grid), dim3(kBlock), 0, s, a12, a48, n, tiles_count,
                            reinterpret_cast<float4*>(raw12), reinterpret_cast<float4*>(raw_m), reinterpret_cast<float4*>(raw_v),
                            reinterpret_cast<float4*>(sh48), reinterpret_cast<float4*>(sh_m), reinterpret_cast<float4*>(sh_v),
                            reinterpret_cast<float4*>(act12_out), block_begin, block_end, own, second_launch ? 1u : 0u, lazy);
@@ -1048,6 +1044,26 @@
     __builtin_amdgcn_fence(__ATOMIC_RELEASE, "wavefront");
     if (lane == 0) lz.wave_step[wave] = lz.t;
 }
+
+__global__ __launch_bounds__(kBlock) void k_sync_deferred_sh(uint32_t n, float4* __restrict__ p48, const float4* __restrict__ m48,
+                                                            const float4* __restrict__ v48, LazyMoments lz) {
+    const uint32_t wave = blockIdx.x * (kBlock / 64) + (threadIdx.x >> 6), lane = threadIdx.x & 63;
+    const uint32_t wave_first = wave * 64u;
+    if (wave_first >= n) return;
+    const uint32_t have = lz.defer.sh_step[wave];
+    if (have >= lz.t) return;
+    if (lz.t - have >= lz.defer.ring_len && lz.overrun && lane == 0) *lz.overrun = 1u;
+    const uint32_t seen = lz.wave_step[wave];
+    const uint32_t rows_here = min(64u, n - wave_first);
+    for (uint32_t q = lane; q < rows_here * 12u; q += 64u) {
+        float4 pp = p48[(size_t)wave_first * 12 + q];
+        replay_sh4(lz.defer, lz.pow1, lz.pow2, lz.len, lz.overrun, seen, have, lz.t, q % 12u, pp, m48[(size_t)wave_first * 12 + q],
+                   v48[(size_t)wave_first * 12 + q]);
+        p48[(size_t)wave_first * 12 + q] = pp;
+    }
+    __builtin_amdgcn_fence(__ATOMIC_RELEASE, "wavefront");
+    if (lane == 0) lz.defer.sh_step[wave] = lz.t;
+}
 }
 
 namespace gut {
@@ -1078,6 +1094,14 @@
     if (lazy && lazy->d_wave_step && lazy->d_pow_beta1 && lazy->d_pow_beta2 && lazy->table_len >= 2 && step >= 1) {
         lz.wave_step = lazy->d_wave_step; lz.pow1 = lazy->d_pow_beta1; lz.pow2 = lazy->d_pow_beta2; lz.len = lazy->table_len; lz.t = step;
         lz.overrun = lazy->d_overrun;
+    }
+    return lz;
+}
+
+gut::LazyMoments gut_make_lazy(const GutLazyMoments* lazy, uint32_t step, const GutDeferredSh* defer) {
+    gut::LazyMoments lz = gut_make_lazy(lazy, step);
+    if (lz.wave_step && defer && defer->d_sh_step && defer->d_step_ring && defer->ring_len >= 2) {
+        lz.defer.sh_step = defer->d_sh_step; lz.defer.ring = defer->d_step_ring; lz.defer.ring_len = defer->ring_len;
     }
     return lz;
 }
@@ -1106,6 +1130,19 @@
     hipLaunchKernelGGL(kern, dim3((waves + 3u) / 4u), dim3(gut::kBlock), 0, static_cast<hipStream_t>(stream), num_particles,
                        reinterpret_cast<float4*>(d_raw_m), reinterpret_cast<float4*>(d_raw_v), reinterpret_cast<float4*>(d_sh_m),
                        reinterpret_cast<float4*>(d_sh_v), lz);
+    return hipGetLastError() == hipSuccess ? 0 : 2;
+}
+
+int gut_sync_deferred_sh(void* stream, uint32_t num_particles, float* d_sh48, const float* d_sh_m, const float* d_sh_v,
+                         const GutLazyMoments* lazy, const GutDeferredSh* defer, uint32_t step) {
+    if (num_particles == 0 || step == 0) return 0;
+    if (!d_sh48 || !d_sh_m || !d_sh_v || !lazy || !defer) return 1;
+    const gut::LazyMoments lz = gut_make_lazy(lazy, step, defer);
+    if (!lz.wave_step || !lz.defer.sh_step) return 3;
+    const uint32_t waves = (num_particles + 63u) / 64u;
+    hipLaunchKernelGGL(gut::k_sync_deferred_sh, dim3((waves + 3u) / 4u), dim3(gut::kBlock), 0, static_cast<hipStream_t>(stream),
+                       num_particles, reinterpret_cast<float4*>(d_sh48), reinterpret_cast<const float4*>(d_sh_m),
+                       reinterpret_cast<const float4*>(d_sh_v), lz);
     return hipGetLastError() == hipSuccess ? 0 : 2;
 }
 
diff --git a/3dgrut_amd/native.py b/3dgrut_amd/native.py
--- a/3dgrut_amd/native.py
+++ b/3dgrut_amd/native.py
@@ -48,6 +48,7 @@
         raw[:, 4:8] = scene["rotation"]
         raw[:, 8:11] = np.log(np.asarray(scene["scale"], np.float64))
         self.raw = torch.as_tensor(raw, device=device)
+        self._features_owner = None
         self.features = torch.as_tensor(np.ascontiguousarray(scene["features"], np.float32), device=device)
         self.n_active_features = int(sh_degree)
         self.max_n_features = 3
@@ -59,6 +60,7 @@
         m = cls.__new__(cls)
         if raw.dim() != 2 or raw.shape[1] != 12 or features.shape != (raw.shape[0], 48):
             raise ValueError("from_tensors: raw must be [N,12] and features [N,48]")
+        m._features_owner = None
         m.raw, m.features = raw.contiguous(), features.contiguous()
         m.spatial_order, m.permutation = bool(spatial_order), permutation
         m.n_active_features, m.max_n_features = int(sh_degree), 3
@@ -68,6 +70,20 @@
     @property
     def num_gaussians(self):
         return self.raw.shape[0]
+
+    @property
+    def features(self):
+        owner = getattr(self, "_features_owner", None)
+        if owner is not None:
+            owner.sync_deferred_sh()
+        return self._features
+
+    @features.setter
+    def features(self, value):
+        owner = getattr(self, "_features_owner", None)
+        if owner is not None:
+            owner.sync_deferred_sh()
+        self._features = value
 
     @property
     def positions(self):
@@ -101,7 +117,7 @@
                  betas=(0.9, 0.999), eps=1e-15, fused_sh_adam=True, rank=0, fused_loss=True, lambda_l1=0.8, lambda_ssim=0.2,
                  dp_chunks=4, dp_chunk_min_rows=1 << 20, fuse_epilogue=True, schedule=None,
                  overlap_optimizer=None, dp_exchange="sparse", dp_side_stream=True, lazy_moments=True, lambda_opacity=0.0,
-                 lambda_scale=0.0):
+                 lambda_scale=0.0, defer_sh=False):
         self.model = model
         self.tracer = tracer
         self.raster: SplatRaster = tracer.tracer_wrapper
@@ -134,6 +150,13 @@
         self.wave_step = None
         self._lazy_overrun = torch.zeros(1, dtype=torch.int32, device=dev)
         self._step_id = 0
+        self.defer_sh = bool(defer_sh) and self.lazy_moments and world_size <= 1
+        self.sh_step = None
+        self._sh_ring = torch.zeros((self.LAZY_TABLE, 64), dtype=torch.float32, device=dev) if self.defer_sh else None
+        self._sh_maybe_deferred = False
+        self.sync_interval = self.LAZY_TABLE // 2
+        if self.defer_sh:
+            model._features_owner = self
         self.fused_loss = bool(fused_loss)
         self.fuse_epilogue = bool(fuse_epilogue)
         self.overlap_optimizer = (bool(getattr(model, "spatial_order", False)) and model.num_gaussians >= self.OVERLAP_MIN_GAUSSIANS) \
@@ -178,6 +201,9 @@
         self._act_key = None
         if getattr(self, "lazy_moments", False):
             self.wave_step = torch.full(((n + 63) // 64,), int(getattr(self, "step_id", 0)), dtype=torch.int32, device=dev)
+        if getattr(self, "defer_sh", False):
+            self.sh_step = torch.full(((n + 63) // 64,), int(getattr(self, "step_id", 0)), dtype=torch.int32, device=dev)
+            self._sh_maybe_deferred = False
         self.act = torch.empty((n, 12), dtype=torch.float32, device=dev)
         self.g12 = torch.empty((n, 12), dtype=torch.float32, device=dev)
         self._reg_partials = torch.empty((max(1, (n + 63) // 64), 2), dtype=torch.float32, device=dev)
@@ -231,6 +257,30 @@
         return _capi.GutLazyMoments(self.wave_step.data_ptr(), self._pow1.data_ptr(), self._pow2.data_ptr(), self.LAZY_TABLE,
                                     self._lazy_overrun.data_ptr())
 
+    def _deferred(self):
+        if not self.defer_sh or self.sh_step is None or self.wave_step is None:
+            return None
+        lz = self._lazy()
+        if lz is None:
+            return None
+        return _capi.GutDeferredSh(self.sh_step.data_ptr(), self._sh_ring.data_ptr(), self.LAZY_TABLE, int(self._step_id),
+                                   self.m48.data_ptr(), self.v48.data_ptr(), lz)
+
+    def sync_deferred_sh(self):
+        if not self._sh_maybe_deferred:
+            return
+        self._sh_maybe_deferred = False
+        m = self.model
+        df = self._deferred()
+        if df is None or m.num_gaussians == 0:
+            return
+        st = torch.cuda.current_stream(m.raw.device).cuda_stream
+        with torch.cuda.device(m.raw.device):
+            rc = self._lib.gut_sync_deferred_sh(C.c_void_p(st), m.num_gaussians, m._features.data_ptr(), self.m48.data_ptr(),
+                                                self.v48.data_ptr(), C.byref(df.lazy), C.byref(df), int(self._step_id))
+        if rc:
+            raise RuntimeError(f"[3dgut] sync_deferred_sh failed ({rc})")
+
     @property
     def step_id(self):
         return self._step_id
@@ -248,6 +298,8 @@
             self._step_id = step
             if self.wave_step is not None:
                 self.wave_step.fill_(step)
+            if self.sh_step is not None:
+                self.sh_step.fill_(step)
 
     def state_dict(self):
         self.sync_moments()
@@ -256,6 +308,7 @@
 
     def load_state_dict(self, state):
         n = self.model.num_gaussians
+        self.sync_deferred_sh()
         for key, dst in (("exp_avg_raw", self.m12), ("exp_avg_sq_raw", self.v12), ("exp_avg_features", self.m48), ("exp_avg_sq_features", self.v48)):
             src = state[key]
             if tuple(src.shape) != tuple(dst.shape):
@@ -266,8 +319,11 @@
         self._step_id = int(state["step"])
         if self.wave_step is not None:
             self.wave_step.fill_(self._step_id)
+        if self.sh_step is not None:
+            self.sh_step.fill_(self._step_id)
 
     def sync_moments(self):
+        self.sync_deferred_sh()
         lz = self._lazy()
         if lz is None or self.model.num_gaussians == 0 or not self.model.raw.is_cuda:
             return
@@ -384,11 +440,15 @@
         if rc:
             raise RuntimeError(f"[3dgut] adam_step failed ({rc})")
 
-    def forward(self, batch, train=True):
+    def forward(self, batch, train=True, _deferred=None):
         m = self.model
         act = self.activate()
         sensor, poses = Tracer.create_camera_parameters(batch)
-        rgba, dist_, hits, vis = self.raster.trace(self.step_id, m.n_active_features, act, m.features, batch.rays_ori.contiguous(),
+        feats = m.features if _deferred is None else m._features
+        if _deferred is not None:
+            self.raster.set_deferred_sh(_deferred)
+            self._defer_set = True
+        rgba, dist_, hits, vis = self.raster.trace(self.step_id, m.n_active_features, act, feats, batch.rays_ori.contiguous(),
                                                   batch.rays_dir.contiguous(), None, sensor, poses.timestamps_us[0],
                                                   poses.timestamps_us[1], poses.T_world_sensors[0], poses.T_world_sensors[1])
         self._ctx = (batch, sensor, poses, rgba, dist_)
@@ -441,6 +501,9 @@
             if getattr(self, "_reg_set", False):
                 self._reg_set = False
                 self.raster.set_regularisation(None)
+            if getattr(self, "_defer_set", False) and not getattr(self, "_early_queued", False):
+                self._defer_set = False
+                self.raster.set_deferred_sh(None)
             if getattr(self, "_early_queued", False):
                 self._early_queued = False
                 try:
@@ -450,6 +513,7 @@
                                        f"{type(err).__name__}: {err}; the trainer's state is not usable: {finish_err}") from err
                 self._act_key = None
                 self._probe_evs = None
+                self._defer_set = False
                 self._end_of_step(None)
             raise
 
@@ -483,12 +547,17 @@
                     self.overlap_optimizer = use_overlap = t_on <= t_off
         early = one_pass and use_overlap and not self.selective
         self._probe_evs = probe_evs
-        rgba, dist_, hits, vis = self.forward(batch)
+        deferred = self._deferred() if (one_pass and not self.selective and reg is None) else None
+        feats = m.features if deferred is None else m._features
+        self._step_deferred = deferred is not None
+        if deferred is not None:
+            self._sh_maybe_deferred = True
+        rgba, dist_, hits, vis = self.forward(batch, _deferred=deferred)
         if one_pass and reg is not None:
             self.raster.set_regularisation(reg)
             self._reg_set = True
         if early:
-            self.raster.optimize_rows_without_gradient(m.raw, self.m12, self.v12, m.features, self.m48, self.v48, self.lr12,
+            self.raster.optimize_rows_without_gradient(m.raw, self.m12, self.v12, feats, self.m48, self.v48, self.lr12,
                                                        self.lr48, self.betas, self.eps, self.step_id + 1, self.act, lazy=self._lazy())
             self._early_queued = True
         self._mark(evs)
@@ -521,7 +590,7 @@
             rgba_grad = rgba_leaf.grad
         self._mark(evs)
         _, sensor, poses, _, _ = self._ctx
-        bwd_args = (self.step_id, m.n_active_features, self.act, m.features, batch.rays_ori.contiguous(),
+        bwd_args = (self.step_id, m.n_active_features, self.act, feats, batch.rays_ori.contiguous(),
                     batch.rays_dir.contiguous(), None, sensor, poses.timestamps_us[0], poses.timestamps_us[1],
                     poses.T_world_sensors[0], poses.T_world_sensors[1], rgba, rgba_grad, dist_, None)
         vmask = None
@@ -535,10 +604,11 @@
                 stats = self.fused_statistics() if self.fused_statistics is not None else None
                 if stats is not None:
                     self.raster.set_position_gradient_statistics(*stats)
-                self.raster.optimize_after_bwd(m.n_active_features, None, m.raw, self.m12, self.v12, m.features,
+                self.raster.optimize_after_bwd(m.n_active_features, None, m.raw, self.m12, self.v12, feats,
                                                self.m48, self.v48, self.lr12, self.lr48, self.betas, self.eps,
                                                0 if self.selective else self.step_id + 1, vmask, self.act, lazy=self._lazy())
                 self._reg_set = False
+                self._defer_set = False
                 self._act_key = (m.raw.data_ptr(), m.raw._version, m.raw.shape[0])
                 return self._finish_step(evs, loss, pred_rgb, vis, hits, reg)
             if self.dp_exchange == "sparse":
@@ -711,7 +781,10 @@
             self.lr12[0:3] = lr
             self.model.n_active_features = deg
         self._step_id += 1
-        if self.lazy_moments and self._step_id % (self.LAZY_TABLE // 2) == 0:
+        if self.sh_step is not None and not getattr(self, "_step_deferred", False):
+            self.sh_step.fill_(self._step_id)
+        self._step_deferred = False
+        if self.lazy_moments and self._step_id % max(1, min(int(self.sync_interval), self.LAZY_TABLE - 1)) == 0:
             self.sync_moments()
 
     def render(self, batch, train=False):
diff --git a/3dgrut_amd/tracer.py b/3dgrut_amd/tracer.py
--- a/3dgrut_amd/tracer.py
+++ b/3dgrut_amd/tracer.py
@@ -389,6 +389,9 @@
 
     def set_regularisation(self, reg):
         _capi.check(self._lib.gut_set_regularisation(self._handle, None if reg is None else C.byref(reg)), "set_regularisation")
+
+    def set_deferred_sh(self, defer):
+        _capi.check(self._lib.gut_set_deferred_sh(self._handle, None if defer is None else C.byref(defer)), "set_deferred_sh")
 
     def optimize_after_bwd(self, num_active_features, camera_position, raw12, raw_m, raw_v, sh48, sh_m, sh_v, lr12, lr48, betas, eps,
                            step, visibility=None, act_out=None, lazy=None):
diff --git a/include/gut_hip.h b/include/gut_hip.h
--- a/include/gut_hip.h
+++ b/include/gut_hip.h
@@ -263,6 +263,20 @@
 int gut_regularisation_loss(void* stream, uint32_t num_particles, const float* d_partials, float lambda_opacity, float lambda_scale,
                             float* d_opacity_loss, float* d_scale_loss, float* d_loss);
 
+typedef struct GutDeferredSh {
+    uint32_t* d_sh_step;
+    float* d_step_ring;
+    uint32_t ring_len;
+    uint32_t steps_applied;
+    const float* d_sh_m;
+    const float* d_sh_v;
+    GutLazyMoments lazy;
+} GutDeferredSh;
+int gut_set_deferred_sh(gut_handle h, const GutDeferredSh* defer);
+int gut_sync_deferred_sh(void* stream, uint32_t num_particles, float* d_sh48, const float* d_sh_m, const float* d_sh_v,
+                         const GutLazyMoments* lazy, const GutDeferredSh* defer ,
+                         uint32_t step );
+
 int gut_position_gradient_statistics(void* stream, uint32_t num_particles, const float* d_position_grad, uint32_t grad_stride,
                                      const float* d_positions, uint32_t position_stride, const float* d_sensor_position,
                                      float* d_norm_accum, int32_t* d_norm_denom);
```

New measurement: 455.1 images/s. 1.9% lower.
